# spthm/grace-devel

Hardware: AMD Instinct MI355X
Metric: Mrays/s SPH column-density trace, 10^7 particles (higher is better)
Workload: dtype f32

## Files before the change

### grace-devel_amd/csrc/trace.hip

```cpp
#include "kernel_tables.hpp"
#include "trace_kernel.hpp"
#include "trace_plan.hpp"

#include <cmath>

using namespace grace_hip;

namespace grace_hip {

static_assert(GRACE_SPH_KERNEL_TABLE_ROWS == GRACE_SPH_KERNEL_WENDLAND_C6 + 1, "one table per built-in kernel");
__device__ double g_sph_kernel_tables[GRACE_SPH_KERNEL_TABLE_ROWS][N_TABLE] = GRACE_SPH_KERNEL_TABLES_INIT;
static const double k_sph_kernel_tables[GRACE_SPH_KERNEL_TABLE_ROWS][N_TABLE] = GRACE_SPH_KERNEL_TABLES_INIT;

static grace_status trace_state_destroy(Context& c)
{
    if (!c.trace) return GRACE_OK;
    TraceState& ts = *c.trace;
    GRACE_TRY(plan_release(ts));
    GRACE_TRY(scene_release(ts));
    GRACE_TRY(rays_release(ts));
    if (ts.hits.chunk_counts) GRACE_TRY_HIP(hipFree(ts.hits.chunk_counts));
    if (ts.custom_table) GRACE_TRY_HIP(hipFree(ts.custom_table));
    if (ts.status) GRACE_TRY_HIP(hipFree(ts.status));
    if (ts.ev0) GRACE_TRY_HIP(hipEventDestroy(ts.ev0));
    if (ts.ev1) GRACE_TRY_HIP(hipEventDestroy(ts.ev1));
    delete c.trace;
    c.trace = nullptr;
    return GRACE_OK;
}

grace_status trace_state(TraceState** out)
{
    Context* c = nullptr;
    GRACE_TRY(current_context(&c));
    if (!c->trace) {
        void* tables = nullptr;
        GRACE_TRY_HIP(hipGetSymbolAddress(&tables, HIP_SYMBOL(g_sph_kernel_tables)));
        c->trace = new TraceState();
        c->trace->builtin_tables = static_cast<const double*>(tables);
        c->trace->kernel_table = c->trace->builtin_tables + GRACE_SPH_KERNEL_CUBIC * N_TABLE;
        g_trace_state_destroy = trace_state_destroy;
    }
    *out = c->trace;
    return GRACE_OK;
}

}

namespace {

struct LaunchPlan {
    int width = 64, n_packets = 0;
    int split = 1;
    bool dev_split = false;
    int hit_chunk_shift = GRANULE_SHIFT, hit_chunks = 0, hit_split = 1;
    size_t hit_packets = 0;
    bool hits_split = false;
    bool keep_chunks = false;
    bool reorder = false;
    bool lattice = false;
    int lat_split = 0;
    bool fast_b = false;
    int treelet = 0, treelet_axis = 0;
};

template <int MODE>
LaunchPlan plan_launch(const TraceState& ts, const bool keep_requested, const size_t n_rays, const size_t n_prims)
{
    LaunchPlan p;
    while ((((n_prims - 1) >> p.hit_chunk_shift) + 1) > size_t(MAX_HIT_CHUNKS)) ++p.hit_chunk_shift;
    p.hit_chunks = int(((n_prims - 1) >> p.hit_chunk_shift) + 1);
    p.hit_packets = ceil_div(n_rays, size_t(64));
    const bool split_hits = ts.width <= 0 && p.hit_packets < 4096 && p.hit_chunks >= 8 && ts.split != 1;
    p.hits_split = MODE == MODE_HITS && split_hits;
    p.keep_chunks = MODE == MODE_COUNT && keep_requested && split_hits;
    if (p.hits_split) {
        if (ts.split > 0) p.hit_split = ts.split;
        else while (p.hit_split < 8 && p.hit_packets * p.hit_split < 16384) p.hit_split *= 2;
    }
    if (ts.width > 0) p.width = ts.width;
    else if (ordered(MODE) && !p.hits_split)
        while (p.width > 16 && ceil_div(n_rays, size_t(p.width)) < 4096) p.width /= 2;
    else if (class_split(MODE) && ts.split <= 0)
        while (p.width > 16 && ceil_div(n_rays, size_t(p.width)) * SUM_CLASSES < 4096) p.width /= 2;
    p.n_packets = ceil_div(n_rays, size_t(p.width));
    p.reorder = ts.ray_reorder && n_rays > 64;
    if (class_split(MODE)) {
        const size_t wave_budget = f4_sums(MODE) ? 16385 : 16384;
        if (ts.split > 0) p.split = ts.split;
        else {
            while (p.split < SUM_CLASSES && size_t(p.n_packets) * p.split < wave_budget) p.split *= 2;
            if (f4_sums(MODE) && p.split > 1 && p.split < ts.lat_split && p.reorder && p.width == 64)
                p.split = ts.lat_split;
        }
    }
    if (p.hits_split) p.split = p.hit_split;
    p.dev_split = f4_class_split(MODE) && p.split > 1 && ts.split <= 0;
    p.lattice = has_lattice(MODE) && p.reorder;
    if (f4_class_split(MODE) && p.split == 1 && p.lattice && p.width == 64
        && ts.lat_split > 0 && ts.split <= 0)
        p.lat_split = ts.lat_split;
    p.fast_b = f4_sums(MODE) && !ts.exact_integrals;
    const int auto_treelet = (MODE == MODE_TRI) ? 512 : 8192, auto_treelet_axis = 32768;
#ifdef GRACE_PACKET_STATS
    p.treelet = ts.treelet < 0 ? auto_treelet : ts.treelet;
    p.treelet_axis = ts.treelet < 0 ? auto_treelet_axis : ts.treelet;
#else
    p.treelet = (MODE == MODE_STATS) ? 0 : (ts.treelet < 0 ? auto_treelet : ts.treelet);
    p.treelet_axis = (MODE == MODE_STATS) ? 0 : (ts.treelet < 0 ? auto_treelet_axis : ts.treelet);
#endif
    return p;
}

struct Nested { bool on = false; size_t* measure = nullptr; };

struct TraceBuffers {
    unsigned long long* sig = nullptr;
    float4* A = nullptr; float2* B = nullptr; double* T64 = nullptr; int2* node_prims = nullptr; float4* C = nullptr;
    float* partial = nullptr; double* partial_d = nullptr;
    int *chunk_counts = nullptr, *chunk_off = nullptr, *scratch_counts = nullptr;
    int4* wave_map = nullptr; int *n_wave_map = nullptr, *pk_first = nullptr, *pk_parts = nullptr;
    uint32_t *pk_prefix = nullptr, *pk_total = nullptr;
    uint32_t* ext = nullptr; uint32_t* keys = nullptr; uint32_t* perm = nullptr;
    bool plan_eligible = false;
    PlanKey plan_key;
};

template <int MODE>
grace_status use_records(TraceState& ts, TraceArgs& a, TraceBuffers& b, FrameGuard& frame, const LaunchPlan& p,
                         const size_t n_rays, const size_t n_prims, const size_t n_nodes, hipStream_t stream,
                         const Nested nested = Nested())
{
    enum CacheUse { USE_NONE, USE_FILL, USE_CHECK, USE_TRUST };
    auto decide = [&](const bool have, const bool pinned, const bool repeat) {
        if (have) return ts.cache_validation ? USE_CHECK : USE_TRUST;
        return (ts.cache_auto && repeat && !pinned) ? USE_FILL : USE_NONE;
    };
    CacheUse scene_use = USE_NONE, rays_use = USE_NONE;
    const SceneKey skey{primitive(MODE), a.spheres, a.nodes, a.leaves, n_prims, n_nodes};
    if (!fp64(MODE) && MODE != MODE_STATS && !nested.measure) {
        scene_use = decide(ts.scene.valid && ts.scene.key == skey, ts.scene.valid && ts.scene.pinned,
                           ts.scene.seen == skey);
        ts.scene.seen = skey;
        if (scene_use == USE_FILL && scene_cache_alloc(ts, skey) != GRACE_OK) scene_use = USE_NONE;
    }
    const RayKey rkey{a.rays, n_rays};
    if (p.reorder && !nested.on) {
        rays_use = decide(ts.rays.valid && ts.rays.key == rkey, ts.rays.valid && ts.rays.pinned,
                          ts.rays.seen == rkey);
        ts.rays.seen = rkey;
        if (rays_use == USE_FILL && rays_cache_alloc(ts, rkey) != GRACE_OK) rays_use = USE_NONE;
    }
    const bool scene_cached = scene_use != USE_NONE, rays_cached = rays_use != USE_NONE;
    auto held = [](const CacheUse u) { return u == USE_CHECK || u == USE_TRUST; };
    b.plan_eligible = ts.plan_on && f4_sums(MODE) && held(scene_use) && held(rays_use) && p.lat_split == 0;
    if (b.plan_eligible)
        b.plan_key = PlanKey{ PLAN_FORMAT, p.fast_b, group_shift(n_prims), p.width, p.reorder, n_rays, n_prims, ts.scene.gen, ts.rays.gen };
    PlanGate gate;
    const bool plan_steady = b.plan_eligible && ts.plan.valid && ts.plan.key == b.plan_key;
    if (plan_steady) {
        gate.ctl = ts.plan.ctl; gate.scene = ts.scene.ctl; gate.rays = ts.rays.ctl;
    }
    const bool scene_sig = scene_use == USE_FILL || scene_use == USE_CHECK;
    const bool rays_sig = rays_use == USE_FILL || rays_use == USE_CHECK, sig = scene_sig || rays_sig;
    auto carve = [&](char* const base) {
        size_t used = 0;
        auto take = [&](auto*& ptr, const size_t count) {
            using T = std::remove_reference_t<decltype(*ptr)>;
            ptr = base ? reinterpret_cast<T*>(base + used) : nullptr;
            used += Workspace::aligned(count * sizeof(T));
        };
        if (sig) take(b.sig, sig_partial_words());
        if (!scene_cached) {
            take(b.A, n_prims + 4);
            if (f4_integrals(MODE)) take(b.B, n_prims + 4);
            if (MODE == MODE_TRI) take(b.T64, 9 * (n_prims + 4));
            take(b.node_prims, n_nodes); take(b.C, cluster_record_count(n_prims));
        }
        if (f4_sums(MODE)) take(b.partial, n_rays * SUM_CLASSES * channels(MODE));
        if (double_sums(MODE)) take(b.partial_d, n_rays * SUM_CLASSES);
        if (p.hits_split) {
            take(b.chunk_counts, n_rays * size_t(p.hit_chunks)); take(b.chunk_off, n_rays * size_t(p.hit_chunks));
            take(b.scratch_counts, n_rays); take(b.wave_map, p.hit_packets * p.hit_split); take(b.n_wave_map, 16);
            take(b.pk_prefix, p.hit_packets * size_t(p.hit_chunks));
            take(b.pk_total, p.hit_packets + 16); take(b.pk_first, p.hit_packets + 16); take(b.pk_parts, p.hit_packets + 16);
        }
        if (p.reorder) { take(b.ext, 20); take(b.keys, n_rays); take(b.perm, n_rays); }
        return used;
    };
    const size_t own = carve(nullptr);
    const size_t need = own + (p.reorder ? sort_ws_bytes(n_rays, 4, 0) : 0);
    if (nested.measure) {
        *nested.measure = need + Workspace::aligned(sig_partial_words() * sizeof(*b.sig));
        return GRACE_OK;
    }
    if (nested.on) GRACE_REQUIRE(Workspace::room() >= need, "trace: the caller's frame is too small for a nested trace");
    else GRACE_TRY(frame.begin(need, stream));
    carve(Workspace::take<char>(own));
    if (sig) {
        SigRequest rq;
        if (scene_sig) {
            rq.prims = a.spheres; rq.prims_bytes = n_prims * (MODE == MODE_TRI ? 36 : 16);
            rq.nodes = a.nodes; rq.nodes_bytes = n_nodes * 64;
            rq.leaves = a.leaves; rq.leaves_bytes = (n_nodes + 1) * 16;
            rq.scene_ctl = ts.scene.ctl; rq.scene_force = scene_use == USE_FILL;
        }
        if (rays_sig) {
            rq.rays = a.rays; rq.rays_bytes = n_rays * 28;
            rq.rays_ctl = ts.rays.ctl; rq.rays_force = rays_use == USE_FILL; rq.rays_ext = ts.rays.ext;
        }
        GRACE_TRY(launch_signatures(rq, b.sig, stream));
    }
    if (scene_cached) {
        Scene& sc = ts.scene;
        if (scene_use != USE_TRUST) {
            GRACE_TRY(scene_fill(skey.kind, a.spheres, n_prims, a.nodes, n_nodes, a.leaves, sc.A, sc.B1, sc.B50,
                                 sc.T64, sc.node_prims, sc.C, stream, &sc.ctl->stale));
            sc.valid = true;
        }
        a.A = sc.A; a.T64 = sc.T64; a.node_prims = sc.node_prims; a.C = sc.C;
        a.B = f4_integrals(MODE) ? (p.fast_b ? sc.B50 : sc.B1) : nullptr;
    } else {
        GRACE_TRY(scene_fill(skey.kind, primitive(MODE) == PRIM_D4 ? static_cast<const void*>(a.spheres_d) : a.spheres,
                             n_prims, a.nodes, n_nodes, a.leaves, b.A, p.fast_b ? nullptr : b.B, p.fast_b ? b.B : nullptr,
                             b.T64, b.node_prims, b.C, stream));
        a.A = b.A; a.B = b.B; a.T64 = b.T64; a.node_prims = b.node_prims; a.C = b.C;
    }
    if (p.reorder) {
        const float4* scene_min = a.C + 2 * ((n_prims + 63) / 64);
        uint32_t* lat_flag = p.lattice ? b.ext + 13 : nullptr;
        int* split_dev = p.dev_split ? reinterpret_cast<int*>(b.ext + 12) : nullptr;
        const int split_flags = f4_sums(MODE) ? SPLIT_WIDE_BUDGET : 0;
        if (rays_cached) {
            RayOrder& ro = ts.rays;
            if (rays_use != USE_TRUST) {
                GRACE_TRY(ray_order(a.rays, n_rays, ro.ext, b.keys, ro.perm, nullptr, nullptr, 0, 0, nullptr,
                                    stream, &ro.ctl->stale));
                ro.valid = true;
            }
            int* plan_split_dev = b.plan_eligible && split_dev && !weighted(MODE)
                ? reinterpret_cast<int*>(b.ext + 16) : nullptr;
            if (lat_flag || split_dev || plan_steady)
                GRACE_TRY(launch_choose_variants(ro.ext, int(n_rays), scene_min, lat_flag, p.n_packets,
                                                 p.split | split_flags, split_dev, stream, plan_steady ? &gate : nullptr,
                                                 plan_split_dev));
            a.perm = ro.perm; a.plan_split_dev = plan_split_dev;
        } else {
            GRACE_TRY(ray_order(a.rays, n_rays, b.ext, b.keys, b.perm, scene_min, lat_flag, p.n_packets,
                                p.split | split_flags, split_dev, stream));
            a.perm = b.perm;
        }
        a.lat_dev = reinterpret_cast<const int*>(lat_flag); a.split_dev = split_dev;
    }
    return GRACE_OK;
}

template <int MODE, bool SPLIT, bool ALT = false>
void launch_walk(const int grid, const TraceArgs& args, hipStream_t stream)
{
    trace_kernel<MODE, SPLIT, ALT, false><<<grid, TRACE_BLOCK, 0, stream>>>(args);
    if constexpr (has_lattice(MODE))
        if (args.lat_dev) trace_kernel<MODE, SPLIT, ALT, true><<<grid, TRACE_BLOCK, 0, stream>>>(args);
}

template <int MODE>
grace_status dispatch(const TraceState& ts, const TraceArgs& a, const TraceBuffers& b, const LaunchPlan& p,
                      const int* kept, const size_t n_rays, hipStream_t stream)
{
    const int grid = ceil_div(size_t(p.n_packets) * p.split, TRACE_BLOCK / 64);
    const int* const plan_k_dev = a.plan_usable ? a.plan_split_dev : nullptr;
    auto combine = [&](const int k, const int* k_dev, const int* run_if) -> grace_status {
        const int g = ceil_div(n_rays * channels(MODE), 256);
        if constexpr (double_sums(MODE))
            combine_classes_kernel<double><<<g, 256, 0, stream>>>(a.partial_d, int(n_rays), k, k_dev, a.out_sums_d, run_if);
        else if constexpr (weighted(MODE))
            combine_channel_classes_kernel<<<g, 256, 0, stream>>>(a.partial, int(n_rays), channels(MODE), k, k_dev,
                                                                  a.out_sums, a.out_stride, run_if,
                                                                  a.plan_usable, plan_k_dev);
        else if constexpr (f4_sums(MODE))
            combine_classes_kernel<float><<<g, 256, 0, stream>>>(a.partial, int(n_rays), k, k_dev, a.out_sums, run_if,
                                                                 a.plan_usable, plan_k_dev);
        else return GRACE_OK;
        GRACE_CHECK_LAUNCH();
        return GRACE_OK;
    };
    if constexpr (class_split(MODE)) {
        auto walk = [&](auto alt_tag) -> grace_status {
            constexpr bool ALT = decltype(alt_tag)::value;
            if constexpr (has_lattice(MODE)) if (p.lat_split) {
                if (output(MODE) == OUT_COUNTS)
                    GRACE_TRY_HIP(hipMemsetAsync(a.out_counts, 0, n_rays * sizeof(int), stream));
                trace_kernel<MODE, false, ALT, false><<<grid, TRACE_BLOCK, 0, stream>>>(a);
                GRACE_CHECK_LAUNCH();
                TraceArgs a_lat = a;
                a_lat.split = p.lat_split; a_lat.split_dev = nullptr;
                trace_kernel<MODE, true, ALT, true><<<ceil_div(size_t(p.n_packets) * p.lat_split, TRACE_BLOCK / 64),
                                                      TRACE_BLOCK, 0, stream>>>(a_lat);
                GRACE_CHECK_LAUNCH();
                return combine(p.lat_split, nullptr, a.lat_dev);
            }
            if constexpr (f4_sums(MODE)) if (a.plan_usable) {
                GRACE_TRY(plan_record(ts, a, stream));
                const int grid_planned = a.plan_split_dev
                    ? ceil_div(size_t(p.n_packets) * planned_split(p.n_packets), TRACE_BLOCK / 64) : grid;
                GRACE_TRY(launch_planned(MODE, ALT, grid_planned, a, stream));
                if (p.split == 1) GRACE_TRY(combine(1, nullptr, reinterpret_cast<const int*>(a.plan_usable)));
            }
            if (p.split > 1) launch_walk<MODE, true, ALT>(grid, a, stream);
            else launch_walk<MODE, false, ALT>(grid, a, stream);
            return GRACE_OK;
        };
        if constexpr (f4_sums(MODE)) GRACE_TRY(p.fast_b ? walk(std::true_type()) : walk(std::false_type()));
        else GRACE_TRY(walk(std::false_type()));
    } else if constexpr (MODE == MODE_HITS) {
        if (p.hits_split) {
            const int* counts = kept;
            if (!kept) {
                TraceArgs c = a;
                c.chunk_counts = b.chunk_counts; c.out_counts = b.scratch_counts;
                GRACE_TRY_HIP(hipMemsetAsync(b.chunk_counts, 0, n_rays * size_t(p.hit_chunks) * 4, stream));
                GRACE_TRY_HIP(hipMemsetAsync(b.scratch_counts, 0, n_rays * 4, stream));
                launch_walk<MODE_COUNT, true>(grid, c, stream);
                GRACE_CHECK_LAUNCH();
                counts = b.chunk_counts;
            }
            hits_offsets_kernel<<<ceil_div(n_rays, 4), 256, 0, stream>>>(counts, a.offsets, int(n_rays),
                                                                         p.hit_chunks, b.chunk_off);
            GRACE_CHECK_LAUNCH();
            hits_plan_kernel<<<p.n_packets, MAX_HIT_CHUNKS, 0, stream>>>(counts, a.perm, int(n_rays),
                                                                         p.hit_chunks, b.pk_prefix, b.pk_total);
            GRACE_CHECK_LAUNCH();
            hits_assign_kernel<<<1, 1024, 0, stream>>>(b.pk_total, p.n_packets, p.n_packets * p.split, p.hit_chunks,
                                                       b.pk_first, b.pk_parts, b.n_wave_map,
                                                       ts.hits_stage_split ? 200000ull : 0ull);
            GRACE_CHECK_LAUNCH();
            hits_bounds_kernel<<<p.n_packets, 64, 0, stream>>>(b.pk_prefix, b.pk_total, b.pk_first, b.pk_parts,
                                                               p.hit_chunks, b.wave_map);
            GRACE_CHECK_LAUNCH();
            TraceArgs staged = a, direct = a;
            staged.stage_dev = direct.stage_dev = b.n_wave_map + 4;
            staged.stage_want = 1; direct.stage_want = 0;
            launch_walk<MODE, true, true>(grid, staged, stream);
            GRACE_CHECK_LAUNCH();
            launch_walk<MODE, true, false>(grid, direct, stream);
        } else if (p.n_packets >= 4096) {
            launch_walk<MODE, false, true>(grid, a, stream);
        } else {
            launch_walk<MODE, false, false>(grid, a, stream);
        }
    } else {
        launch_walk<MODE, false>(grid, a, stream);
    }
    GRACE_CHECK_LAUNCH();
    GRACE_TRY(stamps_report(MODE));
    if (p.split > 1) GRACE_TRY(combine(p.split, a.split_dev, nullptr));
    return GRACE_OK;
}

template <int MODE>
grace_status launch_trace(TraceArgs a, size_t n_rays, size_t n_spheres, size_t n_nodes,
                          hipStream_t stream, const Nested nested = Nested())
{
    GRACE_REQUIRE(a.rays && a.spheres && a.nodes && a.leaves && a.root, "trace: null pointer");
    GRACE_REQUIRE(n_rays < (size_t(1) << 31), "trace: bad ray count");
    GRACE_REQUIRE(n_nodes >= 1 && n_nodes < (size_t(1) << 30), "trace: bad node count");
    GRACE_REQUIRE(n_spheres > 0 && n_spheres < (size_t(1) << 31), "trace: bad primitive count");
    TraceState* ts_ptr = nullptr;
    GRACE_TRY(trace_state(&ts_ptr));
    TraceState& ts = *ts_ptr;
    GRACE_TRY(ensure_status(ts, stream));
    a.kernel_table = ts.kernel_table;
    const LaunchPlan p = plan_launch<MODE>(ts, a.keep_chunks, n_rays, n_spheres);
    const bool reuse_chunks = p.hits_split && ts.hits.valid && ts.hits.rays == a.rays
        && ts.hits.n_rays == n_rays && ts.hits.prims == static_cast<const void*>(a.spheres)
        && ts.hits.n_prims == n_spheres && ts.hits.n_chunks == p.hit_chunks;
    if (chunked(MODE)) ts.hits.valid = false;
    const size_t need = n_rays * size_t(p.hit_chunks);
    if (p.keep_chunks && ts.hits.capacity < need) {
        if (ts.hits.chunk_counts) { GRACE_TRY_HIP(hipDeviceSynchronize()); GRACE_TRY_HIP(hipFree(ts.hits.chunk_counts)); }
        ts.hits.chunk_counts = nullptr; ts.hits.capacity = 0;
        hipError_t e = hipMalloc(reinterpret_cast<void**>(&ts.hits.chunk_counts), need * sizeof(int));
        if (e != hipSuccess) return set_error(GRACE_OUT_OF_MEMORY, __FILE__, __LINE__, hipGetErrorString(e));
        ts.hits.capacity = need;
    }
    FrameGuard frame;
    TraceBuffers b;
    GRACE_TRY(use_records<MODE>(ts, a, b, frame, p, n_rays, n_spheres, n_nodes, stream, nested));
    if (nested.measure) return GRACE_OK;
    a.width = p.width; a.split = p.split; a.treelet = p.treelet; a.treelet_axis = p.treelet_axis;
    a.n_rays = int(n_rays); a.n_nodes = int(n_nodes); a.n_prims = int(n_spheres); a.status = ts.status;
    a.group_shift = group_shift(n_spheres); a.chunk_shift = p.hit_chunk_shift; a.n_chunks = p.hit_chunks;
    a.partial = b.partial; a.partial_d = b.partial_d;
    a.chunk_off = b.chunk_off; a.wave_map = b.wave_map; a.n_wave_map = b.n_wave_map;
    if (p.split > 1 && output(MODE) == OUT_COUNTS)
        GRACE_TRY_HIP(hipMemsetAsync(a.out_counts, 0, n_rays * sizeof(int), stream));
    if (p.keep_chunks && p.split > 1) {
        a.chunk_counts = ts.hits.chunk_counts;
        GRACE_TRY_HIP(hipMemsetAsync(ts.hits.chunk_counts, 0, n_rays * size_t(p.hit_chunks) * 4, stream));
        ts.hits.valid = true; ts.hits.rays = a.rays; ts.hits.n_rays = n_rays;
        ts.hits.prims = a.spheres; ts.hits.n_prims = n_spheres; ts.hits.n_chunks = p.hit_chunks;
    }
    ts.last_lat_dev = a.lat_dev; ts.last_lat_stream = stream;
    if constexpr (f4_sums(MODE)) {
        PacketPlan& pp = ts.plan;
        if (b.plan_eligible && !(pp.key == b.plan_key && (pp.valid || pp.dead)))
            GRACE_TRY(plan_fill(ts, b.plan_key, a, stream));
        ts.last_plan_ctl = nullptr;
        if (b.plan_eligible && pp.valid && pp.key == b.plan_key) {
            a.plan_entries = pp.entries; a.plan_spans = pp.spans; a.plan_counts = pp.counts;
            a.plan_usable = &pp.ctl->usable;
            ts.last_plan_ctl = pp.ctl; ts.last_plan_stream = stream;
        }
    }
    return timed(ts, stream, [&] {
        return dispatch<MODE>(ts, a, b, p, reuse_chunks ? ts.hits.chunk_counts : nullptr, n_rays, stream);
    });
}

TraceArgs trace_args(const void* d_rays, const void* d_prims, const int* d_nodes, const int* d_leaves,
                     const int* d_root)
{
    TraceArgs a = {};
    a.rays = static_cast<const float*>(d_rays);
    a.spheres = static_cast<const float4*>(d_prims);
    a.nodes = reinterpret_cast<const float4*>(d_nodes);
    a.leaves = reinterpret_cast<const int4*>(d_leaves);
    a.root = d_root;
    return a;
}

}

namespace grace_hip {
grace_status rays_invalidate_if_written(const void* d_written)
{
    Context* c = nullptr;
    GRACE_TRY(current_context(&c));
    if (!c->trace) return GRACE_OK;
    TraceState& ts = *c->trace;
    if (ts.cache_validation) return GRACE_OK;
    if (ts.rays.valid && d_written && d_written == static_cast<const void*>(ts.rays.key.rays)) return rays_release(ts);
    return GRACE_OK;
}

grace_status scene_invalidate_if_written(const void* d_written)
{
    Context* c = nullptr;
    GRACE_TRY(current_context(&c));
    if (!c->trace) return GRACE_OK;
    TraceState& ts = *c->trace;
    if (ts.cache_validation) return GRACE_OK;
    if (ts.scene.valid && d_written
        && (d_written == ts.scene.key.prims || d_written == ts.scene.key.nodes || d_written == ts.scene.key.leaves))
        return scene_release(ts);
    return GRACE_OK;
}

grace_status trace_nested_bytes(size_t n_rays, size_t n_spheres, size_t n_nodes, size_t* bytes)
{
    TraceArgs a = trace_args(bytes, bytes, reinterpret_cast<const int*>(bytes), reinterpret_cast<const int*>(bytes),
                             reinterpret_cast<const int*>(bytes));
    size_t counts = 0, hits = 0;
    GRACE_TRY(launch_trace<MODE_COUNT>(a, n_rays, n_spheres, n_nodes, nullptr, Nested{true, &counts}));
    GRACE_TRY(launch_trace<MODE_HITS>(a, n_rays, n_spheres, n_nodes, nullptr, Nested{true, &hits}));
    *bytes = counts > hits ? counts : hits;
    return GRACE_OK;
}

grace_status trace_hitcounts_nested(const void* d_rays, size_t n_rays, const float* d_spheres, size_t n_spheres,
                                    const int* d_nodes, size_t n_nodes, const int* d_leaves, const int* d_root,
                                    int* d_hit_counts, hipStream_t stream)
{
    TraceArgs a = trace_args(d_rays, d_spheres, d_nodes, d_leaves, d_root);
    a.out_counts = d_hit_counts;
    return launch_trace<MODE_COUNT>(a, n_rays, n_spheres, n_nodes, stream, Nested{true, nullptr});
}

grace_status trace_hits_nested(const void* d_rays, size_t n_rays, const float* d_spheres, size_t n_spheres,
                               const int* d_nodes, size_t n_nodes, const int* d_leaves, const int* d_root,
                               const int* d_ray_offsets, int* d_hit_indices, float* d_hit_integrals,
                               float* d_hit_distances, hipStream_t stream)
{
    TraceArgs a = trace_args(d_rays, d_spheres, d_nodes, d_leaves, d_root);
    a.offsets = d_ray_offsets;
    a.hit_idx = d_hit_indices;
    a.hit_integral = d_hit_integrals;
    a.hit_dist = d_hit_distances;
    return launch_trace<MODE_HITS>(a, n_rays, n_spheres, n_nodes, stream, Nested{true, nullptr});
}
}

extern "C" {

grace_status grace_trace_hitcounts_f4(const void* d_rays, size_t n_rays, const float* d_spheres,
                                      size_t n_spheres, const int* d_nodes, size_t n_nodes,
                                      const int* d_leaves, const int* d_root,
                                      int* d_hit_counts, grace_stream stream)
{
    if (n_rays == 0) return GRACE_OK;
    GRACE_REQUIRE(d_hit_counts, "trace_hitcounts: null output");
    TraceArgs a = trace_args(d_rays, d_spheres, d_nodes, d_leaves, d_root);
    a.out_counts = d_hit_counts;
    return launch_trace<MODE_COUNT>(a, n_rays, n_spheres, n_nodes, as_stream(stream));
}

grace_status grace_trace_hitcounts_keep_f4(const void* d_rays, size_t n_rays, const float* d_spheres,
                                           size_t n_spheres, const int* d_nodes, size_t n_nodes,
                                           const int* d_leaves, const int* d_root,
                                           int* d_hit_counts, grace_stream stream)
{
    if (n_rays == 0) return GRACE_OK;
    GRACE_REQUIRE(d_hit_counts, "trace_hitcounts: null output");
    TraceArgs a = trace_args(d_rays, d_spheres, d_nodes, d_leaves, d_root);
    a.out_counts = d_hit_counts;
    a.keep_chunks = true;
    return launch_trace<MODE_COUNT>(a, n_rays, n_spheres, n_nodes, as_stream(stream));
}

grace_status grace_trace_cumulative_f4(const void* d_rays, size_t n_rays, const float* d_spheres,
                                       size_t n_spheres, const int* d_nodes, size_t n_nodes,
                                       const int* d_leaves, const int* d_root,
                                       float* d_cumulated, grace_stream stream)
{
    if (n_rays == 0) return GRACE_OK;
    GRACE_REQUIRE(d_cumulated, "trace_cumulative: null output");
    TraceArgs a = trace_args(d_rays, d_spheres, d_nodes, d_leaves, d_root);
    a.out_sums = d_cumulated;
    return launch_trace<MODE_CUMULATIVE>(a, n_rays, n_spheres, n_nodes, as_stream(stream));
}

grace_status grace_trace_cumulative_weighted_f4(const void* d_rays, size_t n_rays, const float* d_spheres,
                                                size_t n_spheres, const int* d_nodes, size_t n_nodes,
                                                const int* d_leaves, const int* d_root,
                                                const float* d_weights, int n_channels, float* d_out,
                                                grace_stream stream)
{
    GRACE_REQUIRE(n_channels >= 1 && n_channels <= 64, "trace_cumulative_weighted: channels must be 1..64");
    if (n_rays == 0) return GRACE_OK;
    GRACE_REQUIRE(d_weights || n_spheres == 0, "trace_cumulative_weighted: null weights");
    GRACE_REQUIRE(d_out, "trace_cumulative_weighted: null output");
    GRACE_REQUIRE(n_rays * size_t(n_channels) < (size_t(1) << 31), "trace_cumulative_weighted: too many outputs");
    for (int g = 0; g < n_channels; g += MAX_LAUNCH_CHANNELS) {
        TraceArgs a = trace_args(d_rays, d_spheres, d_nodes, d_leaves, d_root);
        a.weights = d_weights + g;
        a.w_stride = n_channels;
        a.out_sums = d_out + g;
        a.out_stride = n_channels;
        const hipStream_t s = as_stream(stream);
        switch (n_channels - g < MAX_LAUNCH_CHANNELS ? n_channels - g : MAX_LAUNCH_CHANNELS) {
        case 1: GRACE_TRY(launch_trace<MODE_WCUM1>(a, n_rays, n_spheres, n_nodes, s)); break;
        case 2: GRACE_TRY(launch_trace<MODE_WCUM2>(a, n_rays, n_spheres, n_nodes, s)); break;
        case 3: GRACE_TRY(launch_trace<MODE_WCUM3>(a, n_rays, n_spheres, n_nodes, s)); break;
        default: GRACE_TRY(launch_trace<MODE_WCUM4>(a, n_rays, n_spheres, n_nodes, s)); break;
        }
    }
    return GRACE_OK;
}

grace_status grace_trace_hits_f4(const void* d_rays, size_t n_rays, const float* d_spheres,
                                 size_t n_spheres, const int* d_nodes, size_t n_nodes,
                                 const int* d_leaves, const int* d_root,
                                 const int* d_ray_offsets, int* d_hit_indices,
                                 float* d_hit_integrals, float* d_hit_distances,
                                 grace_stream stream)
{
    if (n_rays == 0) return GRACE_OK;
    GRACE_REQUIRE(d_ray_offsets && d_hit_indices && d_hit_integrals && d_hit_distances,
                  "trace_hits: null output");
    TraceArgs a = trace_args(d_rays, d_spheres, d_nodes, d_leaves, d_root);
// ... 71 lines not shown
    GRACE_REQUIRE(d_hit_counts, "trace_hitcounts (float4, double): null output");
    TraceArgs a = trace_args(d_rays, d_spheres, d_nodes, d_leaves, d_root);
    a.out_counts = d_hit_counts;
    return launch_trace<MODE_COUNT_F4D>(a, n_rays, n_spheres, n_nodes, as_stream(stream));
}

grace_status grace_trace_cumulative_f4_f64(const void* d_rays, size_t n_rays, const float* d_spheres,
                                           size_t n_spheres, const int* d_nodes, size_t n_nodes,
                                           const int* d_leaves, const int* d_root, double* d_sums,
                                           grace_stream stream)
{
    if (n_rays == 0) return GRACE_OK;
    GRACE_REQUIRE(d_sums, "trace_cumulative (float4, double): null output");
    TraceArgs a = trace_args(d_rays, d_spheres, d_nodes, d_leaves, d_root);
    a.out_sums_d = d_sums;
    return launch_trace<MODE_CUM_F4D>(a, n_rays, n_spheres, n_nodes, as_stream(stream));
}

grace_status grace_trace_hits_f4_f64(const void* d_rays, size_t n_rays, const float* d_spheres,
                                     size_t n_spheres, const int* d_nodes, size_t n_nodes,
                                     const int* d_leaves, const int* d_root, const int* d_ray_offsets,
                                     int* d_hit_indices, double* d_hit_integrals,
                                     double* d_hit_distances, grace_stream stream)
{
    if (n_rays == 0) return GRACE_OK;
    GRACE_REQUIRE(d_ray_offsets && d_hit_indices && d_hit_integrals && d_hit_distances,
                  "trace_hits (float4, double): null output");
    TraceArgs a = trace_args(d_rays, d_spheres, d_nodes, d_leaves, d_root);
    a.offsets = d_ray_offsets;
    a.hit_idx = d_hit_indices;
    a.hit_integral_d = d_hit_integrals;
    a.hit_dist_d = d_hit_distances;
    return launch_trace<MODE_HITS_F4D>(a, n_rays, n_spheres, n_nodes, as_stream(stream));
}

grace_status grace_trace_stats_f4(const void* d_rays, size_t n_rays, const float* d_spheres,
                                  size_t n_spheres, const int* d_nodes, size_t n_nodes,
                                  const int* d_leaves, const int* d_root,
                                  uint32_t* d_stats4, grace_stream stream)
{
    if (n_rays == 0) return GRACE_OK;
    GRACE_REQUIRE(d_stats4, "trace_stats: null output");
    TraceArgs a = trace_args(d_rays, d_spheres, d_nodes, d_leaves, d_root);
    a.stats = d_stats4;
    return launch_trace<MODE_STATS>(a, n_rays, n_spheres, n_nodes, as_stream(stream));
}

grace_status grace_hit_integrals_f32(const float* d_b2, const float* d_h, size_t n, float* d_out,
                                     grace_stream stream)
{
    GRACE_REQUIRE(n == 0 || (d_b2 && d_h && d_out), "hit_integrals: null pointer");
    if (n == 0) return GRACE_OK;
    TraceState* ts = nullptr;
    GRACE_TRY(trace_state(&ts));
    hit_integrals_kernel<<<stream_grid(n, 256), 256, 0, as_stream(stream)>>>(d_b2, d_h, n, d_out,
                                                                             ts->kernel_table);
    GRACE_CHECK_LAUNCH();
    return GRACE_OK;
}

grace_status grace_sph_kernel_table(int kind, double* h_out51)
{
    GRACE_REQUIRE(kind >= GRACE_SPH_KERNEL_CUBIC && kind <= GRACE_SPH_KERNEL_WENDLAND_C6,
                  "sph_kernel_table: kind must be a built-in GRACE_SPH_KERNEL_* (0..5)");
    GRACE_REQUIRE(h_out51, "sph_kernel_table: null output");
    for (int i = 0; i < N_TABLE; ++i) h_out51[i] = k_sph_kernel_tables[kind][i];
    return GRACE_OK;
}

#define GRACE_TRACE_STATE()                                                                      \
    TraceState* ts_ptr_ = nullptr;                                                               \
    GRACE_TRY(trace_state(&ts_ptr_));                                                            \
    TraceState& ts = *ts_ptr_

grace_status grace_trace_prepare_f4(const float* d_spheres, size_t n_spheres, const int* d_nodes,
                                    size_t n_nodes, const int* d_leaves, grace_stream stream)
{
    GRACE_TRACE_STATE();
    return scene_prepare(ts, PRIM_F4, d_spheres, n_spheres, d_nodes, n_nodes, d_leaves, as_stream(stream));
}

grace_status grace_trace_prepare_tri(const float* d_tris, size_t n_tris, const int* d_nodes,
                                     size_t n_nodes, const int* d_leaves, grace_stream stream)
{
    GRACE_TRACE_STATE();
    return scene_prepare(ts, PRIM_TRI, d_tris, n_tris, d_nodes, n_nodes, d_leaves, as_stream(stream));
}

grace_status grace_trace_prepare_rays(const void* d_rays, size_t n_rays, grace_stream stream)
{
    GRACE_TRACE_STATE();
    return rays_prepare(ts, static_cast<const float*>(d_rays), n_rays, as_stream(stream));
}

grace_status grace_trace_release_rays(void)
{
    GRACE_TRACE_STATE();
    GRACE_TRY(plan_release(ts));
    return rays_release(ts);
}

grace_status grace_trace_release(void)
{
    GRACE_TRACE_STATE();
    if (ts.hits.chunk_counts) {
        GRACE_TRY_HIP(hipDeviceSynchronize());
        GRACE_TRY_HIP(hipFree(ts.hits.chunk_counts));
    }
    ts.hits = HitsCache();
    GRACE_TRY(plan_release(ts));
    return scene_release(ts);
}

grace_status grace_trace_enable_timing(int enabled)
{
    GRACE_TRACE_STATE();
    ts.timing = enabled != 0;
    ts.ev_valid = false;
    return GRACE_OK;
}

grace_status grace_trace_last_kernel_ms(float* h_ms)
{
    GRACE_REQUIRE(h_ms, "null output");
    GRACE_TRACE_STATE();
    GRACE_REQUIRE(ts.timing && ts.ev_valid, "no timed traversal launch recorded");
    GRACE_TRY_HIP(hipEventSynchronize(ts.ev1));
    GRACE_TRY_HIP(hipEventElapsedTime(h_ms, ts.ev0, ts.ev1));
    return GRACE_OK;
}

grace_status grace_trace_last_lattice(int* h_lattice)
{
    GRACE_REQUIRE(h_lattice, "null output");
    *h_lattice = 0;
    GRACE_TRACE_STATE();
    if (ts.last_lat_dev) {
        GRACE_TRY_HIP(hipStreamSynchronize(ts.last_lat_stream));
        GRACE_TRY_HIP(hipMemcpy(h_lattice, ts.last_lat_dev, sizeof(int), hipMemcpyDeviceToHost));
    }
    return GRACE_OK;
}

grace_status grace_trace_last_plan_used(int* h_used)
{
    GRACE_REQUIRE(h_used, "null output");
    *h_used = 0;
    GRACE_TRACE_STATE();
    if (ts.last_plan_ctl) {
        PlanCtl h = {};
        GRACE_TRY_HIP(hipStreamSynchronize(ts.last_plan_stream));
        GRACE_TRY_HIP(hipMemcpy(&h, ts.last_plan_ctl, sizeof(h), hipMemcpyDeviceToHost));
        *h_used = h.usable != 0u ? 1 : 0;
    }
    return GRACE_OK;
}

grace_status grace_trace_plan_stats(unsigned long long* h_stats)
{
    GRACE_REQUIRE(h_stats, "null output");
    for (int k = 0; k < 7; ++k) h_stats[k] = 0;
    GRACE_TRACE_STATE();
    if (ts.last_plan_ctl) {
        PlanCtl h = {};
        GRACE_TRY_HIP(hipStreamSynchronize(ts.last_plan_stream));
        GRACE_TRY_HIP(hipMemcpy(&h, ts.last_plan_ctl, sizeof(h), hipMemcpyDeviceToHost));
        if (h.usable != 0u) {
            for (int k = 0; k < 6; ++k) h_stats[k] = h.stats[k];
            h_stats[6] = h.largest_round;
        }
    }
    return GRACE_OK;
}

grace_status grace_trace_set_plan(int on)
{
    GRACE_TRACE_STATE();
    ts.plan_on = on != 0;
    if (!ts.plan_on) GRACE_TRY(plan_release(ts));
    return GRACE_OK;
}

grace_status grace_trace_set_plan_budget(size_t bytes)
{
    GRACE_TRACE_STATE();
    ts.plan_budget = bytes;
    GRACE_TRY(plan_release(ts));
    return GRACE_OK;
}

grace_status grace_trace_plan_bytes(size_t* h_bytes)
{
    GRACE_REQUIRE(h_bytes, "null output");
    GRACE_TRACE_STATE();
    const PacketPlan& pp = ts.plan;
    *h_bytes = pp.valid ? (pp.n_entries + 4) * sizeof(uint4) + pp.n_lists * (sizeof(int) + sizeof(int2)) + sizeof(PlanCtl) : 0;
    return GRACE_OK;
}

grace_status grace_trace_set_packet_split(int waves_per_packet)
{
    GRACE_REQUIRE(waves_per_packet == -1 || waves_per_packet == 1 || waves_per_packet == 2
                      || waves_per_packet == 4 || waves_per_packet == 8,
                  "packet split must be 1, 2, 4, 8 or -1 (automatic)");
    GRACE_TRACE_STATE();
    ts.split = waves_per_packet;
    return GRACE_OK;
}

grace_status grace_trace_set_packet_width(int rays_per_packet)
{
    GRACE_REQUIRE(rays_per_packet == -1 || rays_per_packet == 16 || rays_per_packet == 32
                      || rays_per_packet == 64,
                  "packet width must be 16, 32, 64 or -1 (automatic)");
    GRACE_TRACE_STATE();
    ts.width = rays_per_packet;
    return GRACE_OK;
}

grace_status grace_trace_set_exact_integrals(int enabled)
{
    GRACE_TRACE_STATE();
    ts.exact_integrals = enabled != 0;
    return GRACE_OK;
}

grace_status grace_trace_set_sph_kernel(int kind)
{
    GRACE_REQUIRE(kind >= GRACE_SPH_KERNEL_CUBIC && kind <= GRACE_SPH_KERNEL_WENDLAND_C6,
                  "set_sph_kernel: kind must be a built-in GRACE_SPH_KERNEL_* (0..5); a custom table is "
                  "set with grace_trace_set_sph_kernel_table");
    GRACE_TRACE_STATE();
    ts.sph_kernel = kind;
    ts.kernel_table = ts.builtin_tables + kind * N_TABLE;
    return GRACE_OK;
}

grace_status grace_trace_set_sph_kernel_table(const double* h_table, int n)
{
    GRACE_REQUIRE(h_table && n == N_TABLE, "set_sph_kernel_table: the table must hold 51 values");
    for (int i = 0; i < N_TABLE; ++i)
        GRACE_REQUIRE(std::isfinite(h_table[i]) && h_table[i] >= 0.0,
                      "set_sph_kernel_table: every value must be finite and >= 0");
    GRACE_REQUIRE(h_table[N_TABLE - 1] == 0.0, "set_sph_kernel_table: the last value (b = H) must be 0");
    GRACE_TRACE_STATE();
    GRACE_TRY_HIP(hipDeviceSynchronize());
    if (!ts.custom_table)
        GRACE_TRY_HIP(hipMalloc(reinterpret_cast<void**>(&ts.custom_table), N_TABLE * sizeof(double)));
    GRACE_TRY_HIP(hipMemcpy(ts.custom_table, h_table, N_TABLE * sizeof(double), hipMemcpyHostToDevice));
    for (int i = 0; i < N_TABLE; ++i) ts.custom_host[i] = h_table[i];
    ts.sph_kernel = GRACE_SPH_KERNEL_CUSTOM;
    ts.kernel_table = ts.custom_table;
    return GRACE_OK;
}

grace_status grace_trace_get_sph_kernel(int* h_kind, double* h_table51)
{
    GRACE_TRACE_STATE();
    if (h_kind) *h_kind = ts.sph_kernel;
    if (h_table51) {
        const double* t = ts.sph_kernel == GRACE_SPH_KERNEL_CUSTOM ? ts.custom_host
                                                                   : k_sph_kernel_tables[ts.sph_kernel];
        for (int i = 0; i < N_TABLE; ++i) h_table51[i] = t[i];
    }
    return GRACE_OK;
}

grace_status grace_trace_set_treelet_size(int max_primitives)
{
    GRACE_REQUIRE(max_primitives >= -1, "treelet size must be >= 0 (or -1 for automatic)");
    GRACE_TRACE_STATE();
    ts.treelet = max_primitives;
    return GRACE_OK;
}

grace_status grace_trace_set_ray_reorder(int enabled)
{
    GRACE_TRACE_STATE();
    ts.ray_reorder = enabled != 0;
    return GRACE_OK;
}

grace_status grace_trace_set_cache_validation(int enabled)
{
    GRACE_TRACE_STATE();
    ts.cache_validation = enabled != 0;
    return GRACE_OK;
}

grace_status grace_trace_set_cache_auto(int enabled)
{
    GRACE_TRACE_STATE();
    ts.cache_auto = enabled != 0;
    if (!ts.cache_auto) {
        if ((ts.scene.valid && !ts.scene.pinned) || (ts.rays.valid && !ts.rays.pinned)) GRACE_TRY(plan_release(ts));
        if (ts.scene.valid && !ts.scene.pinned) GRACE_TRY(scene_release(ts));
        if (ts.rays.valid && !ts.rays.pinned) GRACE_TRY(rays_release(ts));
        ts.scene.seen = SceneKey();
        ts.rays.seen = RayKey();
    }
    return GRACE_OK;
}

grace_status grace_trace_set_lattice_split(int waves_per_packet)
{
    GRACE_REQUIRE(waves_per_packet == 0 || waves_per_packet == 2 || waves_per_packet == 4
                      || waves_per_packet == 8,
                  "lattice split must be 0 (one wave per packet), 2, 4 or 8");
    GRACE_TRACE_STATE();
    ts.lat_split = waves_per_packet;
    return GRACE_OK;
}

grace_status grace_trace_set_hits_staging(int enabled)
{
    GRACE_TRACE_STATE();
    ts.hits_stage_split = enabled != 0;
    return GRACE_OK;
}

grace_status grace_trace_status(grace_stream stream)
{
    GRACE_TRACE_STATE();
    if (!ts.status) return GRACE_OK;
// ... 17 lines not shown
```

### grace-devel_amd/csrc/trace_cache.hip

```cpp
#include "trace_state.hpp"

#include <cstdint>

using namespace grace_hip;

namespace {

constexpr int SIG_BLOCK = 256;
constexpr int SIG_GRID = 1024;
constexpr int SIG_GROUPS = 2;

struct SigArgs {
    const uint32_t* base[4];
    size_t words[4];
    size_t chunk0[4];
    int group[4];
    int aligned[4];
    int n_arrays;
};

__device__ __forceinline__ unsigned long long mix64(unsigned long long v)
{
    v ^= v >> 32;
    v *= 0xD6E8FEB86659FD93ull;
    v ^= v >> 29;
    return v;
}

__global__ __launch_bounds__(SIG_BLOCK) void signature_kernel(const SigArgs a,
                                                              unsigned long long* __restrict__ partial)
{
    unsigned long long sx[SIG_GROUPS] = { 0ull, 0ull }, sy[SIG_GROUPS] = { 0ull, 0ull };
    const size_t t0 = blockIdx.x * size_t(blockDim.x) + threadIdx.x, stride = size_t(gridDim.x) * blockDim.x;
    for (int k = 0; k < a.n_arrays; ++k) {
        const size_t n_chunks = (a.words[k] + 3) / 4;
        const uint32_t* w = a.base[k];
        unsigned long long ax = 0ull, ay = 0ull;
        for (size_t c = t0; c < n_chunks; c += stride) {
            uint4 q;
            if (a.aligned[k] && 4 * c + 4 <= a.words[k]) {
                q = reinterpret_cast<const uint4*>(w)[c];
            } else {
                q.x = 4 * c + 0 < a.words[k] ? w[4 * c + 0] : 0u;
                q.y = 4 * c + 1 < a.words[k] ? w[4 * c + 1] : 0u;
                q.z = 4 * c + 2 < a.words[k] ? w[4 * c + 2] : 0u;
                q.w = 4 * c + 3 < a.words[k] ? w[4 * c + 3] : 0u;
            }
            const unsigned long long i = a.chunk0[k] + c;
            const unsigned long long lo = (unsigned long long)q.x | ((unsigned long long)q.y << 32);
            const unsigned long long hi = (unsigned long long)q.z | ((unsigned long long)q.w << 32);
            const unsigned long long x = mix64(lo ^ (i * 0x9E3779B97F4A7C15ull));
            const unsigned long long y = mix64((hi + ((x << 31) | (x >> 33))) ^ (i * 0xC2B2AE3D27D4EB4Full));
            ax += x;
            ay += y;
        }
        sx[a.group[k]] += ax;
        sy[a.group[k]] += ay;
    }
    __shared__ unsigned long long s_red[SIG_BLOCK / 64][2 * SIG_GROUPS];
    const int lane = threadIdx.x & 63, wave = threadIdx.x >> 6;
#pragma unroll
    for (int g = 0; g < SIG_GROUPS; ++g) {
#pragma unroll
        for (int off = 32; off > 0; off >>= 1) {
            sx[g] += __shfl_xor(sx[g], off);
            sy[g] += __shfl_xor(sy[g], off);
        }
        if (lane == 0) { s_red[wave][2 * g] = sx[g]; s_red[wave][2 * g + 1] = sy[g]; }
    }
    __syncthreads();
    if (threadIdx.x < 2 * SIG_GROUPS) {
        unsigned long long v = 0ull;
        for (int w = 0; w < SIG_BLOCK / 64; ++w) v += s_red[w][threadIdx.x];
        partial[size_t(blockIdx.x) * 2 * SIG_GROUPS + threadIdx.x] = v;
    }
}

struct CheckArgs {
    CacheCtl* ctl[SIG_GROUPS];
    int force[SIG_GROUPS];
    unsigned long long salt[SIG_GROUPS];
    uint32_t* rays_ext;
};

__global__ __launch_bounds__(SIG_BLOCK) void signature_check_kernel(const unsigned long long* __restrict__ partial,
                                                                    const CheckArgs a)
{
    __shared__ unsigned long long s_red[SIG_BLOCK / 64][2 * SIG_GROUPS];
    unsigned long long v[2 * SIG_GROUPS] = { 0ull, 0ull, 0ull, 0ull };
    for (int b = threadIdx.x; b < SIG_GRID; b += blockDim.x)
#pragma unroll
        for (int k = 0; k < 2 * SIG_GROUPS; ++k) v[k] += partial[size_t(b) * 2 * SIG_GROUPS + k];
    const int lane = threadIdx.x & 63, wave = threadIdx.x >> 6;
#pragma unroll
    for (int k = 0; k < 2 * SIG_GROUPS; ++k) {
#pragma unroll
        for (int off = 32; off > 0; off >>= 1) v[k] += __shfl_xor(v[k], off);
        if (lane == 0) s_red[wave][k] = v[k];
    }
    __syncthreads();
    if (threadIdx.x < SIG_GROUPS) {
        const int g = threadIdx.x;
        CacheCtl* ctl = a.ctl[g];
        if (ctl) {
            unsigned long long x = a.salt[g], y = ~a.salt[g];
            for (int w = 0; w < SIG_BLOCK / 64; ++w) { x += s_red[w][2 * g]; y += s_red[w][2 * g + 1]; }
            const bool stale = a.force[g] || ctl->sig[0] != x || ctl->sig[1] != y;
            ctl->sig[0] = x;
            ctl->sig[1] = y;
            ctl->stale = stale ? 1u : 0u;
            if (g == 1 && stale && a.rays_ext) {
                for (int k = 0; k < 16; ++k) a.rays_ext[k] = k < 6 ? 0xFFFFFFFFu : 0u;
            }
        }
    }
}

}

namespace grace_hip {

size_t sig_partial_words() { return size_t(SIG_GRID) * 2 * SIG_GROUPS; }

grace_status launch_signatures(const SigRequest& rq, unsigned long long* partial, hipStream_t stream)
{
    SigArgs a = {};
    CheckArgs c = {};
    size_t next_chunk[SIG_GROUPS] = { 0, 0 };
    auto add = [&](const void* p, size_t bytes, int group) {
        if (!p || bytes == 0) return;
        const int k = a.n_arrays++;
        a.base[k] = static_cast<const uint32_t*>(p);
        a.words[k] = bytes / 4;
        a.group[k] = group;
        a.aligned[k] = (reinterpret_cast<uintptr_t>(p) & 15u) == 0 ? 1 : 0;
        a.chunk0[k] = next_chunk[group];
        next_chunk[group] += (a.words[k] + 3) / 4;
        c.salt[group] = c.salt[group] * 0x100000001B3ull + bytes;
    };
    if (rq.scene_ctl) {
        add(rq.prims, rq.prims_bytes, 0);
        add(rq.nodes, rq.nodes_bytes, 0);
        add(rq.leaves, rq.leaves_bytes, 0);
        c.ctl[0] = rq.scene_ctl;
        c.force[0] = rq.scene_force ? 1 : 0;
    }
    if (rq.rays_ctl) {
        add(rq.rays, rq.rays_bytes, 1);
        c.ctl[1] = rq.rays_ctl;
        c.force[1] = rq.rays_force ? 1 : 0;
        c.rays_ext = rq.rays_ext;
    }
    if (!c.ctl[0] && !c.ctl[1]) return GRACE_OK;
    signature_kernel<<<SIG_GRID, SIG_BLOCK, 0, stream>>>(a, partial);
    GRACE_CHECK_LAUNCH();
    signature_check_kernel<<<1, SIG_BLOCK, 0, stream>>>(partial, c);
    GRACE_CHECK_LAUNCH();
    return GRACE_OK;
}

}
```

### grace-devel_amd/csrc/trace_coherence.hip

```cpp
#include "trace_state.hpp"

using namespace grace_hip;

namespace {

__device__ __forceinline__ uint32_t f2ord_u(float f)
{
    const uint32_t u = __float_as_uint(f);
    return (u & 0x80000000u) ? ~u : (u | 0x80000000u);
}

__device__ __forceinline__ float ord2f_u(uint32_t u)
{
    return __uint_as_float((u & 0x80000000u) ? (u & 0x7fffffffu) : ~u);
}

__global__ void ray_ext_init_kernel(uint32_t* __restrict__ ext16)
{
    if (threadIdx.x < 16) ext16[threadIdx.x] = threadIdx.x < 6 ? 0xFFFFFFFFu : 0u;
}

__global__ __launch_bounds__(1024) void ray_extents_kernel(const float* __restrict__ rays, int n,
                                                          uint32_t* __restrict__ ext12,
                                                          const uint32_t* __restrict__ run_if)
// ... 3 lines not shown
    float len_hi = -INFINITY;
#pragma unroll
    for (int k = 0; k < 6; ++k) { lo[k] = INFINITY; hi[k] = -INFINITY; }
    for (int i = blockIdx.x * blockDim.x + threadIdx.x; i < n; i += gridDim.x * blockDim.x) {
        const float* r = rays + 7 * size_t(i);
#pragma unroll
        for (int k = 0; k < 6; ++k) {
            const float v = r[k];
            lo[k] = fminf(lo[k], v);
            hi[k] = fmaxf(hi[k], v);
        }
        len_hi = fmaxf(len_hi, r[6]);
    }
#pragma unroll
    for (int off = 32; off > 0; off >>= 1) len_hi = fmaxf(len_hi, __shfl_xor(len_hi, off));
#pragma unroll
    for (int k = 0; k < 6; ++k) {
#pragma unroll
        for (int off = 32; off > 0; off >>= 1) {
            lo[k] = fminf(lo[k], __shfl_xor(lo[k], off));
            hi[k] = fmaxf(hi[k], __shfl_xor(hi[k], off));
        }
    }
    __shared__ float s_lo[16][6], s_hi[16][6], s_len[16];
    const int wave = threadIdx.x >> 6;
    if ((threadIdx.x & 63) == 0) {
#pragma unroll
        for (int k = 0; k < 6; ++k) { s_lo[wave][k] = lo[k]; s_hi[wave][k] = hi[k]; }
        s_len[wave] = len_hi;
    }
    __syncthreads();
    const int n_waves = int(blockDim.x >> 6);
    if (threadIdx.x < 6) {
        const int k = threadIdx.x;
        float l = s_lo[0][k], h = s_hi[0][k];
        for (int w = 1; w < n_waves; ++w) { l = fminf(l, s_lo[w][k]); h = fmaxf(h, s_hi[w][k]); }
        atomicMin(&ext12[k], f2ord_u(l));
        atomicMax(&ext12[6 + k], f2ord_u(h));
    } else if (threadIdx.x == 6) {
        float l = s_len[0];
        for (int w = 1; w < n_waves; ++w) l = fmaxf(l, s_len[w]);
        if (l > -INFINITY) atomicMax(&ext12[15], f2ord_u(l));
    }
}

__device__ int choose_split(const uint32_t* __restrict__ ext12, int n_packets, int launched_arg, bool lattice)
{
    const bool one_direction = ext12[0] == ext12[6] && ext12[1] == ext12[7] && ext12[2] == ext12[8];
    const int launched = launched_arg & 0xFF;
    const int budget = (launched_arg & SPLIT_WIDE_BUDGET) ? 32768 : 16384;
    int k = launched;
    if (one_direction && !lattice) {
        k = 1;
        while (k < launched && n_packets * k < 8192) k *= 2;
        if (k < launched && n_packets >= 6144 && n_packets * k * 2 <= budget) k *= 2;
    } else if (!lattice) {
        k = 1;
        while (k < launched && n_packets * k < 16384) k *= 2;
    }
    return k;
}

__device__ __forceinline__ uint32_t hilbert2d_15(uint32_t x, uint32_t y)
{
    uint32_t d = 0;
    for (uint32_t s = 1u << 14; s > 0; s >>= 1) {
        const uint32_t rx = (x & s) ? 1u : 0u, ry = (y & s) ? 1u : 0u;
        d = (d << 2) | ((3u * rx) ^ ry);
        if (ry == 0) {
            if (rx) { x = 32767u - x; y = 32767u - y; }
            const uint32_t t = x; x = y; y = t;
        }
    }
    return d;
}

__global__ __launch_bounds__(256) void ray_lattice_kernel(const float* __restrict__ rays, int n,
                                                          const uint32_t* __restrict__ ext12,
                                                          uint32_t* __restrict__ flag,
                                                          const uint32_t* __restrict__ run_if)
{
    if (run_if && *run_if == 0u) return;
    int dims[2] = { 0, 0 }, nvar = 0;
    float lo[2] = { 0.f, 0.f }, span[2] = { 0.f, 0.f };
    for (int k = 5; k >= 0; --k) {
        const float l = ord2f_u(ext12[k]), sp = ord2f_u(ext12[6 + k]) - l;
        if (sp > 0.f && sp < INFINITY) {
            if (nvar < 2) { dims[nvar] = k; lo[nvar] = l; span[nvar] = sp; }
            ++nvar;
        }
    }
    bool fit = nvar == 2 && n >= 64 && (n & (n - 1)) == 0;
    float m1 = 0.f, m2 = 0.f;
    if (fit) {
        int log_n = 0;
        while ((1 << log_n) < n) ++log_n;
        fit = false;
        const float ratio = span[0] / span[1];
        for (int a = 3; a <= log_n - 3; ++a) {
            const float c1 = float((1 << a) - 1), c2 = float((1 << (log_n - a)) - 1);
            if (fabsf(c1 / c2 - ratio) <= 1e-3f * ratio) { fit = true; m1 = c1; m2 = c2; break; }
        }
    }
    if (!fit) {
        if (blockIdx.x == 0 && threadIdx.x == 0) atomicOr(flag, 1u);
        return;
    }
    const float s1 = m1 / span[0], s2 = m2 / span[1];
    bool off = false;
    for (int i = blockIdx.x * blockDim.x + threadIdx.x; i < n; i += gridDim.x * blockDim.x) {
        const float* r = rays + 7 * size_t(i);
        const float u1 = (r[dims[0]] - lo[0]) * s1, u2 = (r[dims[1]] - lo[1]) * s2;
        off = off || !(fabsf(u1 - rintf(u1)) <= 0.01f) || !(fabsf(u2 - rintf(u2)) <= 0.01f);
    }
    if (__builtin_amdgcn_ballot_w64(off) != 0ull && (threadIdx.x & 63) == 0) atomicOr(flag, 1u);
}

__device__ void choose_variants(const uint32_t* __restrict__ ext12, int n, const float4* __restrict__ scene_min,
                                uint32_t* __restrict__ lat_flag, int split_packets, int split_launched,
                                int* __restrict__ split_dev)
{
    if (lat_flag) {
        int n_dir = 0;
        bool one_dir = true;
        float e1 = 0.f, e2 = 0.f;
        for (int k = 0; k < 3; ++k) {
            const float dl = ord2f_u(ext12[k]), dh = ord2f_u(ext12[6 + k]);
            one_dir = one_dir && dl == dh;
            n_dir += dl != 0.f ? 1 : 0;
            const float e = ord2f_u(ext12[9 + k]) - ord2f_u(ext12[3 + k]);
            if (e > e1) { e2 = e1; e1 = e; } else if (e > e2) e2 = e;
        }
        const float spacing2 = e1 * e2 / float(n);
        const float r2_min = scene_min->x;
        bool lat = one_dir && n_dir == 1 && spacing2 > 0.f && r2_min < 2.0f * spacing2;
        if (!lat && e1 == 0.f && ext12[15] != 0u) {
            const float len = ord2f_u(ext12[15]);
            if (len > 0.f && len < INFINITY) lat = r2_min < 2.0f * (12.566371f * len * len / float(n));
        }
        *lat_flag = lat ? 1u : 0u;
    }
    if (split_dev)
        *split_dev = choose_split(ext12, split_packets, split_launched, lat_flag ? *lat_flag != 0u : false);
}

__global__ void choose_variants_kernel(const uint32_t* __restrict__ ext12, int n, const float4* __restrict__ scene_min,
                                       uint32_t* __restrict__ lat_flag, int split_packets, int split_launched,
                                       int* __restrict__ split_dev, const PlanGate gate,
                                       int* __restrict__ plan_split_dev)
{
    if (lat_flag || split_dev)
        choose_variants(ext12, n, scene_min, lat_flag, split_packets, split_launched, split_dev);
    if (plan_split_dev) *plan_split_dev = planned_split(split_packets);
    if (gate.ctl) {
        PlanCtl& pc = *gate.ctl;
        const bool stale = pc.sig[0] != gate.scene->sig[0] || pc.sig[1] != gate.scene->sig[1]
            || pc.sig[2] != gate.rays->sig[0] || pc.sig[3] != gate.rays->sig[1];
        pc.record = stale ? 1u : 0u;
        if (stale) {
            pc.unusable = 0u; pc.usable = 1u;
            pc.sig[0] = gate.scene->sig[0]; pc.sig[1] = gate.scene->sig[1];
            pc.sig[2] = gate.rays->sig[0]; pc.sig[3] = gate.rays->sig[1];
            for (int k = 0; k < 6; ++k) pc.stats[k] = 0ull;
            pc.largest_round = 0u;
        }
    }
}

__global__ __launch_bounds__(256) void ray_keys_kernel(const float* __restrict__ rays, int n,
                                                       const uint32_t* __restrict__ ext12,
                                                       uint32_t* __restrict__ keys,
                                                       const float4* __restrict__ scene_min,
                                                       uint32_t* __restrict__ lat_flag,
                                                       int split_packets, int split_launched,
                                                       int* __restrict__ split_dev,
                                                       const uint32_t* __restrict__ not_grid,
                                                       const uint32_t* __restrict__ run_if)
{
    if (run_if && *run_if == 0u) return;
    const bool z_order_2d = not_grid && *not_grid == 0u;
    if (blockIdx.x == 0 && threadIdx.x == 0)
        choose_variants(ext12, n, scene_min, lat_flag, split_packets, split_launched, split_dev);
    float lo[6], scale[6], span[6];
    int nvar = 0;
    float span_d = 0.f, span_o = 0.f;
#pragma unroll
    for (int k = 0; k < 6; ++k) {
        lo[k] = ord2f_u(ext12[k]);
        span[k] = ord2f_u(ext12[6 + k]) - lo[k];
        const bool varies = span[k] > 0.f && span[k] < INFINITY;
        if (varies) { if (k < 3) span_d = fmaxf(span_d, span[k]); else span_o = fmaxf(span_o, span[k]); }
    }
#pragma unroll
    for (int k = 0; k < 6; ++k) {
        const bool varies = span[k] > 0.f && span[k] < INFINITY;
        scale[k] = varies ? 1.0f / (k < 3 ? span_d : span_o) : 0.f;
        nvar += varies ? 1 : 0;
    }
    const int bits = nvar ? min(15, 30 / nvar) : 0;
    const float qmax = float((1 << bits) - 1);
    const bool pencil = scale[3] == 0.f && scale[4] == 0.f && scale[5] == 0.f && nvar > 0;
    for (int i = blockIdx.x * blockDim.x + threadIdx.x; i < n; i += gridDim.x * blockDim.x) {
        const float* r = rays + 7 * size_t(i);
        if (pencil) {
            const float l1 = fabsf(r[0]) + fabsf(r[1]) + fabsf(r[2]);
            float u = r[0] / l1, v = r[1] / l1;
            if (r[2] < 0.f) {
                const float fu = (1.f - fabsf(v)) * (u >= 0.f ? 1.f : -1.f);
                const float fv = (1.f - fabsf(u)) * (v >= 0.f ? 1.f : -1.f);
                u = fu; v = fv;
            }
            const uint32_t qu = uint32_t(fminf(32767.f, fmaxf(0.f, (u * 0.5f + 0.5f) * 32767.f + 0.5f)));
            const uint32_t qv = uint32_t(fminf(32767.f, fmaxf(0.f, (v * 0.5f + 0.5f) * 32767.f + 0.5f)));
            keys[i] = hilbert2d_15(qu, qv);
            continue;
        }
        uint32_t q[6];
#pragma unroll
        for (int k = 0; k < 6; ++k) q[k] = uint32_t(fminf(qmax, (r[k] - lo[k]) * scale[k] * qmax + 0.5f));
#ifndef GRACE_MORTON2D
        if (nvar == 2 && !z_order_2d) {
            uint32_t xy[2] = {0, 0};
            int m = 0;
#pragma unroll
            for (int k = 5; k >= 0; --k)
                if (scale[k] > 0.f) { if (m < 2) xy[m] = q[k]; ++m; }
            keys[i] = hilbert2d_15(xy[1], xy[0]);
            continue;
        }
#endif
        uint32_t key = 0;
        for (int b = bits - 1; b >= 0; --b) {
#pragma unroll
            for (int k = 5; k >= 0; --k)
                if (scale[k] > 0.f) key = (key << 1) | ((q[k] >> b) & 1u);
        }
        keys[i] = key << (30 - bits * nvar);
    }
}

}

namespace grace_hip {

grace_status launch_choose_variants(const uint32_t* ext12, int n, const float4* scene_min, uint32_t* lat_flag,
                                    int split_packets, int split_launched, int* split_dev, hipStream_t stream,
                                    const PlanGate* gate, int* plan_split_dev)
{
    choose_variants_kernel<<<1, 1, 0, stream>>>(ext12, n, scene_min, lat_flag, split_packets, split_launched,
                                                split_dev, gate ? *gate : PlanGate(), plan_split_dev);
    GRACE_CHECK_LAUNCH();
    return GRACE_OK;
}

static grace_status rays_free_buffers(RayOrder& ro)
{
    if (ro.perm || ro.ext || ro.ctl) GRACE_TRY_HIP(hipDeviceSynchronize());
    if (ro.perm) GRACE_TRY_HIP(hipFree(ro.perm));
    if (ro.ext) GRACE_TRY_HIP(hipFree(ro.ext));
    if (ro.ctl) GRACE_TRY_HIP(hipFree(ro.ctl));
    ro.perm = nullptr; ro.ext = nullptr; ro.ctl = nullptr;
    ro.valid = false;
    ro.pinned = false;
    return GRACE_OK;
}

grace_status rays_release(TraceState& ts)
{
    GRACE_TRY(rays_free_buffers(ts.rays));
    ts.rays = RayOrder();
    return GRACE_OK;
}

grace_status rays_cache_alloc(TraceState& ts, const RayKey& key)
{
    RayOrder& ro = ts.rays;
    GRACE_TRY(rays_free_buffers(ro));
    if (hipMalloc(reinterpret_cast<void**>(&ro.perm), key.n * 4) != hipSuccess
        || hipMalloc(reinterpret_cast<void**>(&ro.ext), 64) != hipSuccess
        || hipMalloc(reinterpret_cast<void**>(&ro.ctl), sizeof(CacheCtl)) != hipSuccess) {
        (void)hipGetLastError();
        (void)rays_free_buffers(ro);
        return set_error(GRACE_OUT_OF_MEMORY, __FILE__, __LINE__, "ray order cache: out of device memory");
    }
    ro.key = key;
    ro.gen = ++ts.cache_gen;
    return GRACE_OK;
}

grace_status ray_order(const float* d_rays, size_t n_rays, uint32_t* ext, uint32_t* keys, uint32_t* perm,
                       const float4* scene_min, uint32_t* lat_flag, int n_packets, int split, int* split_dev,
                       hipStream_t stream, const uint32_t* run_if)
{
    if (!run_if) {
        ray_ext_init_kernel<<<1, 64, 0, stream>>>(ext);
        GRACE_CHECK_LAUNCH();
    }
    const int grid_small = stream_grid(n_rays, 256, 4) < 1024 ? stream_grid(n_rays, 256, 4) : 1024;
    const int grid_ext = stream_grid(n_rays, 1024, 4) < 128 ? stream_grid(n_rays, 1024, 4) : 128;
    ray_extents_kernel<<<grid_ext, 1024, 0, stream>>>(d_rays, int(n_rays), ext, run_if);
    GRACE_CHECK_LAUNCH();
    ray_lattice_kernel<<<grid_small, 256, 0, stream>>>(d_rays, int(n_rays), ext, ext + 14, run_if);
    GRACE_CHECK_LAUNCH();
    ray_keys_kernel<<<stream_grid(n_rays, 256), 256, 0, stream>>>(d_rays, int(n_rays), ext, keys, scene_min,
                                                                 lat_flag, n_packets, split, split_dev, ext + 14,
                                                                 run_if);
    GRACE_CHECK_LAUNCH();
// ... 41 lines not shown
```

### grace-devel_amd/csrc/trace_kernel.hpp

```cpp
#pragma once

#include "trace_diag.hpp"
#include "trace_packet.hpp"
#include "trace_state.hpp"

#include <type_traits>

namespace {

using namespace grace_hip;

__device__ __forceinline__ bool any_lane(bool p) { return __builtin_amdgcn_ballot_w64(p) != 0ull; }

__device__ __forceinline__ int imin(int a, int b) { return a < b ? a : b; }
__device__ __forceinline__ int imax(int a, int b) { return a > b ? a : b; }

__device__ __forceinline__ void aabbs_hit(const float ix, const float iy, const float iz,
                                          const float ox, const float oy, const float oz,
                                          const float len, const float4 L, const float4 R,
                                          const float4 Z, bool& hit_l, bool& hit_r)
{
    const float bx_L = (L.x - ox) * ix, tx_L = (L.y - ox) * ix;
    const float by_L = (L.z - oy) * iy, ty_L = (L.w - oy) * iy;
    const float bz_L = (Z.x - oz) * iz, tz_L = (Z.y - oz) * iz;
    const float bx_R = (R.x - ox) * ix, tx_R = (R.y - ox) * ix;
    const float by_R = (R.z - oy) * iy, ty_R = (R.w - oy) * iy;
    const float bz_R = (Z.z - oz) * iz, tz_R = (Z.w - oz) * iz;

    auto entry = [](const float t) { return t != t ? -INFINITY : t; };
    auto exit_ = [](const float t) { return t != t ? INFINITY : t; };
    const int zero = __float_as_int(0.0f), ilen = __float_as_int(len);
    const int tmin_L = imax(imax(__float_as_int(fminf(entry(bx_L), entry(tx_L))), __float_as_int(fminf(entry(by_L), entry(ty_L)))),
                            imax(imin(__float_as_int(entry(bz_L)), __float_as_int(entry(tz_L))), zero));
    const int tmax_L = imin(imin(__float_as_int(fmaxf(exit_(bx_L), exit_(tx_L))), __float_as_int(fmaxf(exit_(by_L), exit_(ty_L)))),
                            imin(imax(__float_as_int(exit_(bz_L)), __float_as_int(exit_(tz_L))), ilen));
    const int tmin_R = imax(imax(__float_as_int(fminf(entry(bx_R), entry(tx_R))), __float_as_int(fminf(entry(by_R), entry(ty_R)))),
                            imax(imin(__float_as_int(entry(bz_R)), __float_as_int(entry(tz_R))), zero));
    const int tmax_R = imin(imin(__float_as_int(fmaxf(exit_(bx_R), exit_(tx_R))), __float_as_int(fmaxf(exit_(by_R), exit_(ty_R)))),
                            imin(imax(__float_as_int(exit_(bz_R)), __float_as_int(exit_(tz_R))), ilen));
    hit_r = __int_as_float(tmax_R) >= __int_as_float(tmin_R);
    hit_l = __int_as_float(tmax_L) >= __int_as_float(tmin_L);
}

__device__ __forceinline__ float sqrt_rn_normal(const float x)
{
    const float y = __builtin_amdgcn_sqrtf(x);
    const float ym = __int_as_float(__float_as_int(y) - 1);
    const float yp = __int_as_float(__float_as_int(y) + 1);
    const float rm = __builtin_fmaf(-ym, y, x);
    const float rp = __builtin_fmaf(-yp, y, x);
    float r = (0.0f >= rm) ? ym : y;
    r = (0.0f < rp) ? yp : r;
    return r;
}

__device__ __forceinline__ float hit_integral(const float b2, const float ir, const float ir2,
                                              const double2* lut)
{
    const bool tiny = b2 < 1.2621774e-29f && b2 > 0.0f;
    const float root = __builtin_amdgcn_ballot_w64(tiny) ? __builtin_sqrtf(b2) : sqrt_rn_normal(b2);
    const float b = (N_TABLE - 1) * (root * ir);
    int x_idx = static_cast<int>(b);
    float t32 = b - static_cast<float>(x_idx);
    if (__builtin_amdgcn_ballot_w64(x_idx >= N_TABLE - 1)) {
        t32 = x_idx >= N_TABLE - 1 ? 1.0f : t32;
        x_idx = x_idx >= N_TABLE - 1 ? N_TABLE - 2 : x_idx;
    }
    const double2 y = lut[x_idx];
    float integral = static_cast<float>(__builtin_fma(static_cast<double>(t32), y.y, y.x));
    integral *= ir2;
    return integral;
}

__device__ __forceinline__ float hit_integral_fast(const float b2, const float ir50,
                                                   const float2* lutf)
{
    const float b = __builtin_amdgcn_sqrtf(b2) * ir50;
    const float2 y = lutf[static_cast<int>(b)];
    return __builtin_fmaf(y.y, b, y.x);
}

__device__ __forceinline__ bool tri_intersect(const double ddx, const double ddy, const double ddz,
                                              const float ox, const float oy, const float oz,
                                              const double* __restrict__ tri, float* t_out)
{
    const double vx = tri[0], vy = tri[1], vz = tri[2];
    const double e1x = tri[3], e1y = tri[4], e1z = tri[5];
    const double e2x = tri[6], e2y = tri[7], e2z = tri[8];
    const float Px = float(ddy * e2z - ddz * e2y);
    const float Py = float(ddz * e2x - ddx * e2z);
    const float Pz = float(ddx * e2y - ddy * e2x);
    const float det = float((e1x * double(Px) + e1y * double(Py)) + e1z * double(Pz));
    bool reject = det < 1E-14f;
    const float inv_det = 1.0f / det;
    const float OVx = ox - float(vx), OVy = oy - float(vy), OVz = oz - float(vz);
    const double dOVx = OVx, dOVy = OVy, dOVz = OVz;
    const float u = float(((dOVx * double(Px) + dOVy * double(Py)) + dOVz * double(Pz)) * double(inv_det));
    reject = reject || (u < 0.f || u > 1.f);
    const float Qx = float(dOVy * e1z - dOVz * e1y);
    const float Qy = float(dOVz * e1x - dOVx * e1z);
    const float Qz = float(dOVx * e1y - dOVy * e1x);
    const float v = float(((ddx * double(Qx) + ddy * double(Qy)) + ddz * double(Qz)) * double(inv_det));
    reject = reject || (v < 0.f || u + v > 1.f);
    *t_out = float(((e2x * double(Qx) + e2y * double(Qy)) + e2z * double(Qz)) * double(inv_det));
    return !reject;
}

__global__ __launch_bounds__(256) void hit_integrals_kernel(const float* __restrict__ b2,
                                                            const float* __restrict__ h, size_t n,
                                                            float* __restrict__ out,
                                                            const double* __restrict__ table)
{
    __shared__ double2 s_lut[N_TABLE];
    if (threadIdx.x < N_TABLE) {
        const double y0 = table[threadIdx.x];
        const double y1 = threadIdx.x + 1 < N_TABLE ? table[threadIdx.x + 1] : y0;
        s_lut[threadIdx.x] = make_double2(y0, y1 - y0);
    }
    __syncthreads();
    for (size_t i = blockIdx.x * size_t(blockDim.x) + threadIdx.x; i < n;
         i += size_t(gridDim.x) * blockDim.x) {
        const float ir = 1.f / h[i];
        out[i] = hit_integral(b2[i], ir, ir * ir, s_lut);
    }
}

__device__ __forceinline__ bool beam_may_hit(const float4 s, const Beam& bm,
                                             const float margin = 3.814697265625e-06f )
{
    float p2_lo = 0.f, p2_hi = 0.f, t_lo = 0.f, t_hi = 0.f;
    const float c[3] = { s.x, s.y, s.z };
#pragma unroll
    for (int k = 0; k < 3; ++k) {
        const float plo = c[k] - bm.ohi[k], phi = c[k] - bm.olo[k];
        const float a2 = plo * plo, b2 = phi * phi;
        p2_hi += fmaxf(a2, b2);
        p2_lo += (plo <= 0.f && phi >= 0.f) ? 0.f : fminf(a2, b2);
        const float q0 = plo * bm.dlo[k], q1 = plo * bm.dhi[k];
        const float q2 = phi * bm.dlo[k], q3 = phi * bm.dhi[k];
        t_lo += fminf(fminf(q0, q1), fminf(q2, q3));
        t_hi += fmaxf(fmaxf(q0, q1), fmaxf(q2, q3));
    }
    const float t2_hi = fmaxf(t_lo * t_lo, t_hi * t_hi);
    const float b2_lo = p2_lo - t2_hi - margin * p2_hi;
    return !(b2_lo >= s.w);
}

struct Pencil {
    float ox, oy, oz;
    float ax, ay, az;
    float sin_t, cos_t;
    float nx[4], ny[4], nz[4];
};

__device__ __forceinline__ bool pencil_may_hit(const float4 s, const Pencil& pc)
{
    const float vx = s.x - pc.ox, vy = s.y - pc.oy, vz = s.z - pc.oz;
    const float d2 = __builtin_fmaf(vx, vx, __builtin_fmaf(vy, vy, vz * vz));
    const float va = __builtin_fmaf(vx, pc.ax, __builtin_fmaf(vy, pc.ay, vz * pc.az));
    const float inv = __builtin_amdgcn_rsqf(d2);
    const float sin_a = fminf(1.0f, __builtin_amdgcn_sqrtf(s.w) * inv * 1.00001f);
    const float cos_a = __builtin_amdgcn_sqrtf(fmaxf(0.0f, __builtin_fmaf(-sin_a, sin_a, 1.0f)));
    const float cos_limit = __builtin_fmaf(pc.cos_t, cos_a, -pc.sin_t * sin_a) - 1e-5f;
    const float h = __builtin_amdgcn_sqrtf(s.w) * 1.00001f + 1e-6f * __builtin_amdgcn_sqrtf(d2);
    float out = -1.0f;
#pragma unroll
    for (int k = 0; k < 4; ++k)
        out = fmaxf(out, __builtin_fmaf(vx, pc.nx[k], __builtin_fmaf(vy, pc.ny[k], vz * pc.nz[k])) - h);
    return !(d2 > s.w * 1.00001f) || (!(va * inv < cos_limit) && !(out > 0.0f));
}

template <int AX, bool FUSED = false>
__device__ __forceinline__ bool axis_beam_may_hit(const float4 s, const Beam& bm)
{
    constexpr int D1 = AX == 0 ? 1 : 0, D2 = AX == 2 ? 1 : 2;
    const float s1 = AX == 0 ? s.y : s.x;
    const float s2 = AX == 2 ? s.y : s.z;
    const float q1 = s1 - __builtin_amdgcn_fmed3f(s1, bm.olo[D1], bm.ohi[D1]);
    const float q2 = s2 - __builtin_amdgcn_fmed3f(s2, bm.olo[D2], bm.ohi[D2]);
    const float b2_lo = FUSED ? __builtin_fmaf(q1, q1, q2 * q2) : q1 * q1 + q2 * q2;
    return !(b2_lo >= s.w);
}

__device__ __forceinline__ float4 cluster_sphere(const float4 blo, const float4 bhi)
{
    const float cx = 0.5f * (blo.x + bhi.x), cy = 0.5f * (blo.y + bhi.y), cz = 0.5f * (blo.z + bhi.z);
    const float ex = bhi.x - cx, ey = bhi.y - cy, ez = bhi.z - cz;
    const float fx = cx - blo.x, fy = cy - blo.y, fz = cz - blo.z;
    const float rx = fmaxf(ex, fx), ry = fmaxf(ey, fy), rz = fmaxf(ez, fz);
    return make_float4(cx, cy, cz, (rx * rx + ry * ry + rz * rz) * 1.001f);
}

template <int AX>
__device__ __forceinline__ bool cluster_may_hit(const float4 blo, const float4 bhi, const Beam& bm,
                                                const Pencil* pc)
{
    if constexpr (AX >= 0) {
        constexpr int D1 = AX == 0 ? 1 : 0, D2 = AX == 2 ? 1 : 2;
        const float lo1 = AX == 0 ? blo.y : blo.x, hi1 = AX == 0 ? bhi.y : bhi.x;
        const float lo2 = AX == 2 ? blo.y : blo.z, hi2 = AX == 2 ? bhi.y : bhi.z;
        return !(lo1 > bm.ohi[D1]) && !(hi1 < bm.olo[D1]) && !(lo2 > bm.ohi[D2]) && !(hi2 < bm.olo[D2]);
    } else if constexpr (AX == -2) {
        const float lx = blo.x - pc->ox, ly = blo.y - pc->oy, lz = blo.z - pc->oz;
        const float hx = bhi.x - pc->ox, hy = bhi.y - pc->oy, hz = bhi.z - pc->oz;
        const float scale = fmaxf(fmaxf(fmaxf(fabsf(lx), fabsf(hx)), fmaxf(fabsf(ly), fabsf(hy))),
                                  fmaxf(fabsf(lz), fabsf(hz)));
        const float slack = 1e-5f * scale;
        float worst = -1.0f;
#pragma unroll
        for (int k = 0; k < 4; ++k) {
            const float m = fminf(pc->nx[k] * lx, pc->nx[k] * hx) + fminf(pc->ny[k] * ly, pc->ny[k] * hy)
                + fminf(pc->nz[k] * lz, pc->nz[k] * hz);
            worst = fmaxf(worst, m);
        }
        const float front = fmaxf(pc->ax * lx, pc->ax * hx) + fmaxf(pc->ay * ly, pc->ay * hy)
            + fmaxf(pc->az * lz, pc->az * hz);
        return !(worst > slack) && !(front < -slack) && pencil_may_hit(cluster_sphere(blo, bhi), *pc);
    } else {
        return beam_may_hit(cluster_sphere(blo, bhi), bm, 1.52587890625e-05f );
    }
}

typedef uint32_t plan_u32x4 __attribute__((ext_vector_type(4)));
typedef int plan_i32x2 __attribute__((ext_vector_type(2)));
template <typename T>
__device__ __forceinline__ const __attribute__((address_space(4))) T* plan_const(const void* p)
{
    return (const __attribute__((address_space(4))) T*)(uintptr_t)p;
}

template <int N>
struct WeightedB {
    float x, y;
    float w[N + 1];
    __device__ WeightedB(const float2 b) : x(b.x), y(b.y), w{} {}
};

template <int MODE, bool SPLIT, bool ALT = false, bool LAT = false, bool PLANNED = false>
__global__ __launch_bounds__(TRACE_BLOCK, !f4_class_split(MODE) ? 1
                                          : weighted(MODE) ? (channels(MODE) == 1 ? 6 : 7 - channels(MODE))
                                          : (SPLIT ? 8 : 6))
void trace_kernel(const TraceArgs a)
{
    static_assert(!ALT || f4_integrals(MODE), "no alternative path for this mode");
    static_assert(!LAT || has_lattice(MODE), "no lattice cull for this mode");
    static_assert(!PLANNED || (SPLIT && !LAT && f4_sums(MODE)), "planned: class-split column densities only");
    if constexpr (PLANNED) {
        if (*plan_const<uint32_t>(a.plan_usable) == 0u) return;
    } else if (has_lattice(MODE)) {
        if (a.plan_usable && *a.plan_usable != 0u) return;
        if (a.lat_dev ? (*a.lat_dev != 0) != LAT : LAT) return;
        if (a.stage_dev && *a.stage_dev != a.stage_want) return;
    }
    constexpr bool FAST = ALT && f4_sums(MODE);
    constexpr bool WEIGHTED = weighted(MODE);
    constexpr int NW = channels(MODE), WP = WEIGHTED ? (NW + 1) / 2 : 0;
    using BRec = std::conditional_t<WEIGHTED, WeightedB<NW>, float2>;
    __shared__ double2 s_lut[FAST ? 1 : N_TABLE];
    constexpr int LUTF_N = 256;
    __shared__ float2 s_lutf[FAST ? LUTF_N : 1];
    constexpr bool D4 = primitive(MODE) == PRIM_D4, F4D = primitive(MODE) == PRIM_F4D;
    constexpr bool LDS_TILE = primitive(MODE) == PRIM_F4;
    __shared__ __align__(16) float2 s_tile[LDS_TILE ? TRACE_BLOCK / 64 : 1][LDS_TILE ? 3 + WP : 1][LDS_TILE ? 66 : 1];
    __shared__ double s_tile_d[D4 ? TRACE_BLOCK / 64 : 1][D4 ? 64 : 1][D4 ? 6 : 1];
    __shared__ float4 s_tile_f[F4D ? TRACE_BLOCK / 64 : 1][F4D ? 64 : 1][F4D ? 2 : 1];
    const int lane = threadIdx.x & 63;
    static_assert(!SPLIT || class_split(MODE) || MODE == MODE_HITS, "triangle and stats walks do not split");
    constexpr bool RANGE_SPLIT = SPLIT && MODE == MODE_HITS;
    const int split_ordinary = !SPLIT ? 1 : (!RANGE_SPLIT && a.split_dev) ? *a.split_dev : a.split;
    int split_planned = 0;
    if constexpr (PLANNED)
        if (a.plan_split_dev) split_planned = *plan_const<int>(a.plan_split_dev);
    const int split = PLANNED && split_planned > 0 ? split_planned : split_ordinary;
    const int n_packets = (a.n_rays + a.width - 1) / a.width;
    const int nb = (n_packets * split + TRACE_BLOCK / 64 - 1) / (TRACE_BLOCK / 64);
    const int q = nb >> 3, r8 = nb & 7, xcd = blockIdx.x & 7, slot = blockIdx.x >> 3;
    if (slot >= q + (xcd < r8 ? 1 : 0)) return;
    const int vblock = (xcd < r8 ? xcd * (q + 1) : r8 * (q + 1) + (xcd - r8) * q) + slot;
    const int wave_id = __builtin_amdgcn_readfirstlane(vblock * (TRACE_BLOCK / 64)
                                                       + (threadIdx.x >> 6));
    if (integrates(MODE)) {
        if (FAST) {
            static_assert(TRACE_BLOCK >= 256, "one table entry per thread");
            float2 e = make_float2(0.f, 0.f);
            if (threadIdx.x < N_TABLE - 1) {
                const double y0 = a.kernel_table[threadIdx.x], dy = a.kernel_table[threadIdx.x + 1] - y0;
                e = make_float2(float(y0 - double(threadIdx.x) * dy), float(dy));
            }
            if (threadIdx.x < LUTF_N) s_lutf[threadIdx.x] = e;
        } else if (threadIdx.x < N_TABLE) {
            const int i0 = threadIdx.x;
            const double y0 = a.kernel_table[i0];
            const double y1 = i0 + 1 < N_TABLE ? a.kernel_table[i0 + 1] : y0;
            s_lut[threadIdx.x] = make_double2(y0, y1 - y0);
        }
        __syncthreads();
    }
    int packet = wave_id / split, part = wave_id - packet * split;
    int prim_lo = 0, prim_hi = 0x7fffffff;
    if (RANGE_SPLIT) {
        if (wave_id >= *a.n_wave_map) return;
        const int4 wm = a.wave_map[wave_id];
        packet = wm.x; part = 0;
        prim_lo = wm.y << a.chunk_shift;
        prim_hi = wm.z << a.chunk_shift;
        if (prim_lo >= prim_hi) return;
    }
    const int first_ray = packet * a.width;
    if (first_ray >= a.n_rays) return;
    const int classes_per_part = SUM_CLASSES / split;
    const int own_lo = part * classes_per_part, own_hi = own_lo + classes_per_part;
    auto owns_granule = [&](const int g) {
        if (RANGE_SPLIT) { const int p = g << GRANULE_SHIFT; return p >= prim_lo && p < prim_hi; }
        const int c = g & (SUM_CLASSES - 1);
        return c >= own_lo && c < own_hi;
    };
    auto foreign_range = [&](const int first, const int count) {
        if (RANGE_SPLIT) return first + count <= prim_lo || first >= prim_hi;
        const int g0 = first >> GRANULE_SHIFT, g1 = (first + count - 1) >> GRANULE_SHIFT;
        return g1 - g0 <= 1 && !owns_granule(g0) && !owns_granule(g1);
    };
    const PacketRay ray = load_packet_ray(a, first_ray, lane);
    const bool valid = ray.valid;
    const int ray_index = ray.index;
    const float dx = ray.dx, dy = ray.dy, dz = ray.dz;
    const float ox = ray.ox, oy = ray.oy, oz = ray.oz;
    const float len = ray.len;
    const float ix = 1.f / dx, iy = 1.f / dy, iz = 1.f / dz;
    const Beam beam = packet_beam(ray);
    int axis = -1;
    if (!ordered(MODE)) axis = packet_axis(dx, dy, dz);
    __shared__ Pencil s_pencil[TRACE_BLOCK / 64];
    Pencil pencil;
    bool is_pencil = false;
    if (!PLANNED && axis < 0 && MODE != MODE_STATS && beam.olo[0] == beam.ohi[0] && beam.olo[1] == beam.ohi[1]
        && beam.olo[2] == beam.ohi[2]) {
        float sx = dx, sy = dy, sz = dz;
#pragma unroll
        for (int off = 32; off > 0; off >>= 1) {
            sx += __shfl_xor(sx, off); sy += __shfl_xor(sy, off); sz += __shfl_xor(sz, off);
        }
        const float inv = 1.0f / sqrtf(sx * sx + sy * sy + sz * sz);
        const float ax = sx * inv, ay = sy * inv, az = sz * inv;
        const float cx = ay * dz - az * dy, cy = az * dx - ax * dz, cz = ax * dy - ay * dx;
        const float sin_t = wave_max(sqrtf(cx * cx + cy * cy + cz * cz)) + 2e-6f;
        const float cos_min = wave_min(ax * dx + ay * dy + az * dz);
        if (cos_min > 0.5f && sin_t < 0.8660254f) {
            is_pencil = true;
            pencil.ox = beam.olo[0]; pencil.oy = beam.olo[1]; pencil.oz = beam.olo[2];
            pencil.ax = ax; pencil.ay = ay; pencil.az = az;
            pencil.sin_t = sin_t;
            pencil.cos_t = sqrtf(1.0f - sin_t * sin_t);
            float ux, uy, uz;
            if (fabsf(ax) <= fabsf(ay) && fabsf(ax) <= fabsf(az)) { ux = 0.f; uy = -az; uz = ay; }
            else if (fabsf(ay) <= fabsf(az)) { ux = az; uy = 0.f; uz = -ax; }
            else { ux = -ay; uy = ax; uz = 0.f; }
            const float un = 1.0f / sqrtf(ux * ux + uy * uy + uz * uz);
            ux *= un; uy *= un; uz *= un;
            const float vx = ay * uz - az * uy, vy = az * ux - ax * uz, vz = ax * uy - ay * ux;
            const float da_ = ax * dx + ay * dy + az * dz;
            const float tu = (ux * dx + uy * dy + uz * dz) / da_, tv = (vx * dx + vy * dy + vz * dz) / da_;
            const float m = 4e-6f;
            const float tu_lo = wave_min(tu) - m, tu_hi = wave_max(tu) + m;
            const float tv_lo = wave_min(tv) - m, tv_hi = wave_max(tv) + m;
            auto plane = [&](int k, float cu, float cv, float ca) {
                float px = cu * ux + cv * vx + ca * ax, py = cu * uy + cv * vy + ca * ay,
                      pz = cu * uz + cv * vz + ca * az;
                const float pn = 1.0f / sqrtf(px * px + py * py + pz * pz);
                pencil.nx[k] = px * pn; pencil.ny[k] = py * pn; pencil.nz[k] = pz * pn;
            };
            plane(0, 1.f, 0.f, -tu_hi);
            plane(1, -1.f, 0.f, tu_lo);
            plane(2, 0.f, 1.f, -tv_hi);
            plane(3, 0.f, -1.f, tv_lo);
            if (lane == 0) s_pencil[threadIdx.x >> 6] = pencil;
        }
    }
    const AxisRay ar = axis_ray(axis, ray);
    const float oa = ar.oa, da = ar.da, noda = ar.noda, o1 = ar.o1, o2 = ar.o2;
    float noda_lo = 0.f, noda_hi = 0.f, len_lo = 0.f, da0 = 0.f;
    bool same_sense = false;
    if (axis >= 0) axis_extremes(ar, len, noda_lo, noda_hi, len_lo, da0, same_sense);
    const float fat_r2 = FAST && axis >= 0 ? fat_radius2(axis, beam) : INFINITY;
    const int treelet = axis >= 0 ? a.treelet_axis : a.treelet;
    constexpr bool LATTICE = LAT;
    __shared__ float s_lat[LATTICE ? TRACE_BLOCK / 64 : 1][2][8];
    __shared__ float s_lat_r2[LATTICE ? TRACE_BLOCK / 64 : 1];
    if (LATTICE && lane == 0) s_lat_r2[threadIdx.x >> 6] = 0.f;
    if (LATTICE && axis >= 0) {
        bool ok;
        float cell2;
        build_origin_lattice(o1, o2, lane, s_lat, ok, cell2);
        if (lane == 0) s_lat_r2[threadIdx.x >> 6] = ok ? cell2 : 0.f;
    }

    int count = 0;
    constexpr bool CHUNKED = SPLIT && chunked(MODE);
    int cur_chunk = -1;
    int count_at_chunk = 0;
    float sum = 0.f;
    float wsum[NW] = {};
    constexpr bool CLASSES_F = f4_sums(MODE), CLASSES_D = double_sums(MODE);
    constexpr bool CLASSES = output(MODE) == OUT_SUMS || WEIGHTED;
    __shared__ float s_class[CLASSES_F ? TRACE_BLOCK / 64 : 1][CLASSES_F ? SUM_CLASSES * NW : 1][CLASSES_F ? 64 : 1];
    __shared__ double s_class_d[CLASSES_D ? TRACE_BLOCK / 64 : 1][CLASSES_D ? SUM_CLASSES : 1][CLASSES_D ? 64 : 1];
    const int wv_acc = threadIdx.x >> 6;
    if (CLASSES_F) {
#pragma unroll
        for (int c = 0; c < SUM_CLASSES * NW; ++c) s_class[wv_acc][c][lane] = 0.f;
    }
    if (CLASSES_D) {
#pragma unroll
        for (int c = 0; c < SUM_CLASSES; ++c) s_class_d[wv_acc][c][lane] = 0.0;
    }
    double sum_d = 0.0;
    int cur_granule = -1;
    int cur_granule_end = 0;
    bool cur_owned = true;
    auto enter_granule = [&](const int prim) {
        if (cur_granule >= 0) {
            if constexpr (WEIGHTED) {
#pragma unroll
                for (int c = 0; c < NW; ++c) s_class[wv_acc][(cur_granule & (SUM_CLASSES - 1)) * NW + c][lane] = wsum[c];
            } else {
            if (CLASSES_D) s_class_d[wv_acc][cur_granule & (SUM_CLASSES - 1)][lane] = sum_d;
            else s_class[wv_acc][cur_granule & (SUM_CLASSES - 1)][lane] = sum;
            }
        }
        cur_granule = prim >> GRANULE_SHIFT;
// ... 861 lines not shown
```

### grace-devel_amd/csrc/trace_planned.hip

```cpp
#include "trace_kernel.hpp"

#include <vector>

using namespace grace_hip;

namespace {

struct PlanRef {
    uint4* entries;
    const int2* spans;
    int* counts;
    PlanCtl* ctl;
    int force;
};

template <bool FUSED>
__global__ __launch_bounds__(TRACE_BLOCK) void plan_record_kernel(const TraceArgs a, const PlanRef pl)
{
    __shared__ float s_lat[TRACE_BLOCK / 64][2][8];
    if (pl.spans && !pl.force && pl.ctl->record == 0u) return;
    const int lane = threadIdx.x & 63, wv = threadIdx.x >> 6;
    const int n_packets = (a.n_rays + a.width - 1) / a.width;
    const int packet = blockIdx.x * (TRACE_BLOCK / 64) + wv;
    if (packet >= n_packets) return;
// ... 33 lines not shown
            const bool g_may = box_may_hit(group_boxes[2 * size_t(gj)], group_boxes[2 * size_t(gj) + 1], true);
            const int n_g = min(64, n_groups - g0);
            unsigned long long gmask = __builtin_amdgcn_ballot_w64(g_may) & (n_g >= 64 ? ~0ull : ((1ull << n_g) - 1ull));
            while (gmask != 0ull) {
                const int g = g0 + __builtin_ctzll(gmask);
                gmask &= gmask - 1ull;
                const int r_lo = g << a.group_shift;
                const int r_hi = r_lo + min(1 << a.group_shift, covered - r_lo);
                const int c_first = r_lo >> 6, c_last = (r_hi - 1) >> 6;
                for (int cg = c_first; cg <= c_last; cg += 64) {
                    const int cj = min(cg + lane, c_last);
                    const bool c_may = box_may_hit(a.C[2 * size_t(cj)], a.C[2 * size_t(cj) + 1], false);
                    const int n_c = min(64, c_last - cg + 1);
                    unsigned long long cmask = __builtin_amdgcn_ballot_w64(c_may)
                        & (n_c >= 64 ? ~0ull : ((1ull << n_c) - 1ull));
                    while (cmask != 0ull) {
                        const int c = cg + __builtin_ctzll(cmask);
                        cmask &= cmask - 1ull;
                        const int pbase = c << 6;
                        const int pj = min(max(pbase + lane, r_lo), r_hi - 1);
                        const float4 mine = a.A[pj];
                        const int lo_bit = max(r_lo - pbase, 0), hi_bit = min(r_hi - pbase, 64);
                        const unsigned long long m_mask =
                            (hi_bit >= 64 ? ~0ull : ((1ull << hi_bit) - 1ull)) & (~0ull << lo_bit);
                        const float s1 = axis == 0 ? mine.y : mine.x;
                        const float s2 = axis == 2 ? mine.y : mine.z;
                        const float sa = axis == 0 ? mine.x : axis == 1 ? mine.y : mine.z;
                        const float q1 = s1 - __builtin_amdgcn_fmed3f(s1, lo1, hi1);
                        const float q2 = s2 - __builtin_amdgcn_fmed3f(s2, lo2, hi2);
                        const float b2_lo = FUSED ? __builtin_fmaf(q1, q1, q2 * q2) : q1 * q1 + q2 * q2;
                        bool keep = !(b2_lo >= mine.w);
                        unsigned long long rest = __builtin_amdgcn_ballot_w64(keep) & m_mask;
                        keep = __builtin_amdgcn_inverse_ballot_w64(rest);
                        if (rest != 0ull && __builtin_amdgcn_ballot_w64(keep && mine.w < lat_r2) != 0ull) {
                            float p1 = INFINITY, p2 = INFINITY;
                            for (int k = 0; k < 8; ++k) {
                                p1 = fminf(p1, fabsf(s1 - s_lat[wv][0][k]));
                                p2 = fminf(p2, fabsf(s2 - s_lat[wv][1][k]));
                            }
                            const float nan_if_nan = (s1 + s2) * 0.0f;
                            const float l2 = (FUSED ? __builtin_fmaf(p1, p1, p2 * p2) : p1 * p1 + p2 * p2) + nan_if_nan;
                            keep = keep && !(l2 >= mine.w);
                            rest = __builtin_amdgcn_ballot_w64(keep);
                        }
                        if (rest == 0ull) continue;
                        const unsigned long long inside =
                            __builtin_amdgcn_ballot_w64(__builtin_fmaf(sa, da0, noda_lo) >= 0.0f)
                            & __builtin_amdgcn_ballot_w64(__builtin_fmaf(sa, da0, noda_hi) < len_lo);
                        const bool lean = same_sense && (rest & ~inside) == 0ull;
                        const bool fat = FUSED && (rest & ~__builtin_amdgcn_ballot_w64(mine.w >= fat_r2)) == 0ull;
                        const int cls = (c >> (GRANULE_SHIFT - 6)) & (SUM_CLASSES - 1);
                        const int n = __builtin_amdgcn_readlane(cnt, cls);
                        const int bits = (lean ? 1 : 0) | (fat ? 2 : 0);
                        const int n_surv = __builtin_popcountll(rest);
                        const int open_n = __builtin_amdgcn_readlane(round_n, cls);
                        const int open_bits = __builtin_amdgcn_readlane(round_bits, cls);
                        const bool close_cap = n > 0 && open_n + n_surv > 64;
                        const bool close_flag = n > 0 && !close_cap && open_bits != bits;
                        const bool close = close_cap || close_flag;
                        if (pl.spans) {
                            const int2 span = pl.spans[packet * SUM_CLASSES + cls];
                            if (n < span.y) {
                                if (lane == 0) {
                                    if (close) pl.entries[size_t(span.x) + n - 1].w = uint32_t(open_bits) | PLAN_ROUND_END;
                                    pl.entries[size_t(span.x) + n] =
                                        make_uint4(uint32_t(c), uint32_t(rest), uint32_t(rest >> 32), uint32_t(bits));
                                }
                            } else {
                                failed = true;
                            }
                        }
                        if (lane == cls) {
                            if (close) {
                                t_rounds += 1; t_full += open_n == 64 ? 1 : 0;
                                t_cap += close_cap ? 1 : 0; t_flag += close_flag ? 1 : 0;
                                t_max = max(t_max, open_n);
                                round_n = 0;
                            }
                            round_n += n_surv; round_bits = bits;
                            t_surv += n_surv;
                            cnt += 1;
                        }
                    }
                }
            }
        }
    }
    if (failed) {
        cnt = 0;
        if (lane == 0) { pl.ctl->unusable = 1u; pl.ctl->usable = 0u; }
    }
    if (lane < SUM_CLASSES) pl.counts[packet * SUM_CLASSES + lane] = cnt;
    if (pl.spans && !failed) {
        for (int cls = 0; cls < SUM_CLASSES; ++cls) {
            const int n = __builtin_amdgcn_readlane(cnt, cls);
            const int open_bits = __builtin_amdgcn_readlane(round_bits, cls);
            if (n > 0 && lane == 0)
                pl.entries[size_t(pl.spans[packet * SUM_CLASSES + cls].x) + n - 1].w = uint32_t(open_bits) | PLAN_ROUND_END;
        }
        if (lane < SUM_CLASSES && cnt > 0) {
            t_rounds += 1; t_full += round_n == 64 ? 1 : 0;
            t_max = max(t_max, round_n);
        }
        if (lane >= SUM_CLASSES) cnt = 0;
        int tally[6] = { cnt, t_surv, t_rounds, t_full, t_cap, t_flag };
#pragma unroll
        for (int off = 1; off < SUM_CLASSES; off <<= 1) {
#pragma unroll
            for (int k = 0; k < 6; ++k) tally[k] += __shfl_xor(tally[k], off);
            t_max = max(t_max, __shfl_xor(t_max, off));
        }
        if (lane == 0) {
#pragma unroll
            for (int k = 0; k < 6; ++k)
                if (tally[k]) atomicAdd(&pl.ctl->stats[k], (unsigned long long)tally[k]);
            atomicMax(&pl.ctl->largest_round, uint32_t(t_max));
        }
    }
}

grace_status launch_record(const bool fast, const TraceArgs& a, const PlanRef& pl, hipStream_t stream)
{
    const int n_packets = (a.n_rays + a.width - 1) / a.width;
    const int grid = ceil_div(size_t(n_packets), size_t(TRACE_BLOCK / 64));
    if (fast) plan_record_kernel<true><<<grid, TRACE_BLOCK, 0, stream>>>(a, pl);
    else plan_record_kernel<false><<<grid, TRACE_BLOCK, 0, stream>>>(a, pl);
    GRACE_CHECK_LAUNCH();
    return GRACE_OK;
}

grace_status plan_free_buffers(PacketPlan& pp)
{
    void* bufs[] = { pp.entries, pp.spans, pp.counts, pp.ctl };
    bool any = false;
    for (void* b : bufs) any = any || b;
    if (any) GRACE_TRY_HIP(hipDeviceSynchronize());
    for (void* b : bufs)
        if (b) GRACE_TRY_HIP(hipFree(b));
    pp.entries = nullptr; pp.spans = nullptr; pp.counts = nullptr; pp.ctl = nullptr;
    pp.valid = false;
    pp.n_lists = pp.n_entries = pp.recorded = 0;
    return GRACE_OK;
}

}

namespace grace_hip {

grace_status plan_release(TraceState& ts)
{
    GRACE_TRY(plan_free_buffers(ts.plan));
    ts.plan = PacketPlan();
    ts.last_plan_ctl = nullptr;
    return GRACE_OK;
}

grace_status plan_fill(TraceState& ts, const PlanKey& key, const TraceArgs& a, hipStream_t stream)
{
    PacketPlan& pp = ts.plan;
    GRACE_TRY(plan_free_buffers(pp));
    ts.last_plan_ctl = nullptr;
    pp.key = key;
    pp.dead = true;
    const int n_packets = (a.n_rays + a.width - 1) / a.width;
    const size_t n_lists = size_t(n_packets) * SUM_CLASSES;
    auto alloc = [&](auto*& ptr, const size_t bytes) {
        if (hipMalloc(reinterpret_cast<void**>(&ptr), bytes) == hipSuccess) return true;
        (void)hipGetLastError();
        ptr = nullptr;
        return false;
    };
    if (n_lists * (sizeof(int) + sizeof(int2)) > ts.plan_budget) return GRACE_OK;
    if (!alloc(pp.counts, n_lists * sizeof(int)) || !alloc(pp.spans, n_lists * sizeof(int2))
        || !alloc(pp.ctl, sizeof(PlanCtl)))
        return plan_free_buffers(pp);
    GRACE_TRY_HIP(hipMemsetAsync(pp.ctl, 0, sizeof(PlanCtl), stream));
    GRACE_TRY(launch_record(key.fast, a, PlanRef{ nullptr, nullptr, pp.counts, pp.ctl, 1 }, stream));
    std::vector<int> counts(n_lists);
    PlanCtl seen = {};
    GRACE_TRY_HIP(hipMemcpyAsync(counts.data(), pp.counts, n_lists * sizeof(int), hipMemcpyDeviceToHost, stream));
    GRACE_TRY_HIP(hipMemcpyAsync(&seen, pp.ctl, sizeof(seen), hipMemcpyDeviceToHost, stream));
    GRACE_TRY_HIP(hipStreamSynchronize(stream));
    if (seen.unusable) return plan_free_buffers(pp);
    std::vector<int2> spans(n_lists);
    size_t total = 0, used = 0;
    for (size_t l = 0; l < n_lists; ++l) {
        const size_t room = size_t(counts[l]) + size_t(counts[l]) / 8 + 2;
        spans[l] = make_int2(int(total), int(room));
        total += room;
        used += size_t(counts[l]);
        if (total >= (size_t(1) << 31)) return plan_free_buffers(pp);
    }
    const size_t bytes = (total + 4) * sizeof(uint4) + n_lists * (sizeof(int) + sizeof(int2));
    if (bytes > ts.plan_budget || !alloc(pp.entries, (total + 4) * sizeof(uint4))) return plan_free_buffers(pp);
    GRACE_TRY_HIP(hipMemcpy(pp.spans, spans.data(), n_lists * sizeof(int2), hipMemcpyHostToDevice));
    GRACE_TRY_HIP(hipMemsetAsync(pp.entries + total, 0, 4 * sizeof(uint4), stream));
    pp.n_lists = n_lists; pp.n_entries = total; pp.recorded = used;
    GRACE_TRY_HIP(hipMemsetD32Async(reinterpret_cast<hipDeviceptr_t>(&pp.ctl->usable), 1, 1, stream));
    GRACE_TRY_HIP(hipMemcpyAsync(&pp.ctl->sig[0], ts.scene.ctl->sig, 16, hipMemcpyDeviceToDevice, stream));
    GRACE_TRY_HIP(hipMemcpyAsync(&pp.ctl->sig[2], ts.rays.ctl->sig, 16, hipMemcpyDeviceToDevice, stream));
    GRACE_TRY(launch_record(key.fast, a, PlanRef{ pp.entries, pp.spans, pp.counts, pp.ctl, 1 }, stream));
    pp.valid = true;
    pp.dead = false;
    return GRACE_OK;
}

grace_status plan_record(const TraceState& ts, const TraceArgs& a, hipStream_t stream)
{
    const PacketPlan& pp = ts.plan;
    return launch_record(pp.key.fast, a, PlanRef{ pp.entries, pp.spans, pp.counts, pp.ctl, 0 }, stream);
}

grace_status launch_planned(const int mode, const bool fast, const int grid, const TraceArgs& a, hipStream_t stream)
{
    auto go = [&](auto mode_tag) {
        constexpr int MODE = decltype(mode_tag)::value;
        if (fast) trace_kernel<MODE, true, true, false, true><<<grid, TRACE_BLOCK, 0, stream>>>(a);
        else trace_kernel<MODE, true, false, false, true><<<grid, TRACE_BLOCK, 0, stream>>>(a);
    };
    switch (mode) {
    case MODE_CUMULATIVE: go(std::integral_constant<int, MODE_CUMULATIVE>()); break;
    case MODE_WCUM1: go(std::integral_constant<int, MODE_WCUM1>()); break;
    case MODE_WCUM2: go(std::integral_constant<int, MODE_WCUM2>()); break;
    case MODE_WCUM3: go(std::integral_constant<int, MODE_WCUM3>()); break;
    case MODE_WCUM4: go(std::integral_constant<int, MODE_WCUM4>()); break;
    default: return set_error(GRACE_INVALID_ARGUMENT, __FILE__, __LINE__, "no planned kernel for this mode");
    }
    GRACE_CHECK_LAUNCH();
    return GRACE_OK;
}

}
```

### grace-devel_amd/csrc/trace_state.hpp

```cpp
#pragma once

#include "common.hpp"

namespace grace_hip {

constexpr int TRACE_BLOCK = 256;
constexpr int N_TABLE = 51;
constexpr int SPLIT_WIDE_BUDGET = 0x100;

inline int group_shift(size_t n_prims)
{
    int s = 12;
    while (((n_prims + (size_t(1) << s) - 1) >> s) > 4096) ++s;
    return s;
}
inline size_t group_count(size_t n_prims)
{
    const int s = group_shift(n_prims);
    return (n_prims + (size_t(1) << s) - 1) >> s;
}
inline size_t cluster_record_count(size_t n_prims)
{
    return 2 * ((n_prims + 63) / 64) + 1 + 2 * group_count(n_prims);
}
constexpr int MAX_HIT_CHUNKS = 256;
constexpr int SUM_CLASSES = 8;
constexpr int GRANULE_SHIFT = 10;


enum { MODE_COUNT = 0, MODE_CUMULATIVE = 1, MODE_HITS = 2, MODE_STATS = 3, MODE_TRI = 4,
       MODE_COUNT_D4 = 5, MODE_CUM_D4 = 6, MODE_HITS_D4 = 7,
       MODE_COUNT_F4D = 8, MODE_CUM_F4D = 9, MODE_HITS_F4D = 10,
       MODE_WCUM1 = 11, MODE_WCUM2 = 12, MODE_WCUM3 = 13, MODE_WCUM4 = 14 };

enum Primitive { PRIM_F4 = 0,
                 PRIM_TRI = 1,
                 PRIM_D4 = 2,
                 PRIM_F4D = 3 };
enum Output { OUT_COUNTS, OUT_SUMS, OUT_HITS, OUT_STATS, OUT_CLOSEST,
              OUT_WSUMS };

struct ModeParts { Primitive prim; Output out; int channels = 1; };
constexpr ModeParts mode_parts(const int mode)
{
    switch (mode) {
    case MODE_COUNT:      return { PRIM_F4, OUT_COUNTS };
    case MODE_CUMULATIVE: return { PRIM_F4, OUT_SUMS };
    case MODE_HITS:       return { PRIM_F4, OUT_HITS };
    case MODE_STATS:      return { PRIM_F4, OUT_STATS };
    case MODE_TRI:        return { PRIM_TRI, OUT_CLOSEST };
    case MODE_COUNT_D4:   return { PRIM_D4, OUT_COUNTS };
    case MODE_CUM_D4:     return { PRIM_D4, OUT_SUMS };
    case MODE_HITS_D4:    return { PRIM_D4, OUT_HITS };
    case MODE_COUNT_F4D:  return { PRIM_F4D, OUT_COUNTS };
    case MODE_CUM_F4D:    return { PRIM_F4D, OUT_SUMS };
    case MODE_HITS_F4D:   return { PRIM_F4D, OUT_HITS };
    case MODE_WCUM1:      return { PRIM_F4, OUT_WSUMS, 1 };
    case MODE_WCUM2:      return { PRIM_F4, OUT_WSUMS, 2 };
    case MODE_WCUM3:      return { PRIM_F4, OUT_WSUMS, 3 };
    case MODE_WCUM4:      return { PRIM_F4, OUT_WSUMS, 4 };
    }
    __builtin_unreachable();
}
constexpr Primitive primitive(const int mode) { return mode_parts(mode).prim; }
constexpr Output output(const int mode) { return mode_parts(mode).out; }
constexpr int channels(const int mode) { return mode_parts(mode).channels; }
constexpr int MAX_LAUNCH_CHANNELS = 4;
constexpr bool weighted(const int mode) { return output(mode) == OUT_WSUMS; }

constexpr bool fp64(const int mode) { return primitive(mode) == PRIM_D4 || primitive(mode) == PRIM_F4D; }
constexpr bool class_split(const int mode)
{
    return output(mode) == OUT_COUNTS || output(mode) == OUT_SUMS || output(mode) == OUT_WSUMS;
}
constexpr bool f4_class_split(const int mode) { return class_split(mode) && primitive(mode) == PRIM_F4; }
constexpr bool f4_sums(const int mode)
{
    return primitive(mode) == PRIM_F4 && (output(mode) == OUT_SUMS || output(mode) == OUT_WSUMS);
}
constexpr bool double_sums(const int mode) { return output(mode) == OUT_SUMS && fp64(mode); }
constexpr bool ordered(const int mode) { return output(mode) == OUT_HITS || output(mode) == OUT_CLOSEST; }
constexpr bool integrates(const int mode)
{
    return output(mode) == OUT_SUMS || output(mode) == OUT_WSUMS || output(mode) == OUT_HITS;
}
constexpr bool f4_integrals(const int mode) { return integrates(mode) && primitive(mode) == PRIM_F4; }
constexpr bool has_lattice(const int mode) { return primitive(mode) == PRIM_F4 && output(mode) != OUT_STATS; }
constexpr bool chunked(const int mode)
{
    return primitive(mode) == PRIM_F4 && (output(mode) == OUT_COUNTS || output(mode) == OUT_HITS);
}

struct TraceArgs {
    const float* rays;
    const uint32_t* perm;
    int n_rays;
    const float4* spheres;
    const int2* node_prims;
    int treelet;
    int treelet_axis;
    const float4* A;
    const float2* B;
    int group_shift;
    const float4* C;
    const double* T64;
    const double* spheres_d;
    double* out_sums_d;
    double* hit_integral_d;
    double* hit_dist_d;
    int split;
    int n_prims;
    float* partial;
    double* partial_d;
    const int* split_dev;
    const int* lat_dev;
    const int* stage_dev;
    int stage_want;
    int* chunk_counts;
    const int* chunk_off;
    const int4* wave_map;
    const int* n_wave_map;
    bool keep_chunks;
    int chunk_shift, n_chunks;
    int width;
    const float4* nodes;
    int n_nodes;
    const int4* leaves;
    const int* root;
    int* out_counts;
    float* out_sums;
    const int* offsets;
    int* hit_idx;
    float* hit_integral;
    float* hit_dist;
    uint32_t* stats;
    int* status;
    const float* weights;
    int w_stride;
    int out_stride;
    const double* kernel_table;
    const uint4* plan_entries;
    const int2* plan_spans;
    const int* plan_counts;
    const uint32_t* plan_usable;
    const int* plan_split_dev;
};


struct CacheCtl {
    unsigned long long sig[2];
    uint32_t stale;
    uint32_t pad;
};

struct SceneKey {
    Primitive kind = PRIM_F4;
    const void* prims = nullptr; const void* nodes = nullptr; const void* leaves = nullptr;
    size_t n_prims = 0, n_nodes = 0;
    bool operator==(const SceneKey& o) const
    {
        return kind == o.kind && prims == o.prims && nodes == o.nodes && leaves == o.leaves
            && n_prims == o.n_prims && n_nodes == o.n_nodes;
    }
};

struct Scene {
    bool valid = false;
    SceneKey key;
    SceneKey seen;
    float4* A = nullptr; float2* B1 = nullptr; float2* B50 = nullptr; double* T64 = nullptr;
    int2* node_prims = nullptr; float4* C = nullptr;
    CacheCtl* ctl = nullptr;
    bool pinned = false;
    unsigned long long gen = 0;
};

struct RayKey {
    const float* rays = nullptr;
    size_t n = 0;
    bool operator==(const RayKey& o) const { return rays == o.rays && n == o.n; }
};

struct RayOrder {
    bool valid = false;
    RayKey key, seen;
    uint32_t* perm = nullptr;
    uint32_t* ext = nullptr;
    CacheCtl* ctl = nullptr;
    bool pinned = false;
    unsigned long long gen = 0;
};

struct PlanCtl {
    uint32_t record;
    uint32_t unusable;
    uint32_t usable;
    uint32_t largest_round;
    unsigned long long sig[4];
    unsigned long long stats[6];
};
constexpr uint32_t PLAN_ROUND_END = 4u;
constexpr int PLAN_FORMAT = 2;

struct PlanKey {
    int format = PLAN_FORMAT;
    bool fast = false;
    int group_shift = 0, width = 0;
    bool reorder = false;
    size_t n_rays = 0, n_prims = 0;
    unsigned long long scene_gen = 0, rays_gen = 0;
    bool operator==(const PlanKey& o) const
    {
        return format == o.format && fast == o.fast && group_shift == o.group_shift && width == o.width && reorder == o.reorder
            && n_rays == o.n_rays && n_prims == o.n_prims && scene_gen == o.scene_gen && rays_gen == o.rays_gen;
    }
};

struct PacketPlan {
    bool valid = false;
    bool dead = false;
    PlanKey key;
    uint4* entries = nullptr;
    int2* spans = nullptr;
    int* counts = nullptr;
    PlanCtl* ctl = nullptr;
    size_t n_lists = 0, n_entries = 0;
    size_t recorded = 0;
};

struct PlanGate {
    const CacheCtl* scene = nullptr;
    const CacheCtl* rays = nullptr;
    PlanCtl* ctl = nullptr;
};

__host__ __device__ inline int planned_split(const int n_packets)
{
    return n_packets <= 8192 ? SUM_CLASSES : SUM_CLASSES / 2;
}

struct HitsCache {
    int* chunk_counts = nullptr;
    size_t capacity = 0;
    bool valid = false;
    const void* rays = nullptr; const void* prims = nullptr;
    size_t n_rays = 0, n_prims = 0;
    int n_chunks = 0;
};

struct TraceState {
    int* status = nullptr;
    const int* last_lat_dev = nullptr;
    hipStream_t last_lat_stream = nullptr;
    bool timing = false;
    hipEvent_t ev0 = nullptr, ev1 = nullptr;
    bool ev_valid = false;
    bool ray_reorder = true;
    int treelet = -1;
    int split = -1;
    int lat_split = 4;
    int width = -1;
    bool exact_integrals = false;
    bool hits_stage_split = true;
    bool cache_validation = true;
    bool cache_auto = true;
    int sph_kernel = 0;
    const double* builtin_tables = nullptr;
    const double* kernel_table = nullptr;
    double* custom_table = nullptr;
    double custom_host[N_TABLE] = {};
    bool plan_on = true;
    size_t plan_budget = size_t(512) << 20;
    Scene scene;
    RayOrder rays;
    HitsCache hits;
    unsigned long long cache_gen = 0;
    PacketPlan plan;
    const PlanCtl* last_plan_ctl = nullptr;
    hipStream_t last_plan_stream = nullptr;
};

grace_status trace_state(TraceState** out);

inline grace_status ensure_status(TraceState& ts, hipStream_t stream)
{
    if (!ts.status) {
        GRACE_TRY_HIP(hipMalloc(reinterpret_cast<void**>(&ts.status), sizeof(int)));
        GRACE_TRY_HIP(hipMemsetAsync(ts.status, 0, sizeof(int), stream));
    }
    return GRACE_OK;
}

template <typename Launches>
grace_status timed(TraceState& ts, hipStream_t stream, Launches launches)
{
    if (ts.timing) {
        if (!ts.ev0) { GRACE_TRY_HIP(hipEventCreate(&ts.ev0)); GRACE_TRY_HIP(hipEventCreate(&ts.ev1)); }
        GRACE_TRY_HIP(hipEventRecord(ts.ev0, stream));
    }
    GRACE_TRY(launches());
    if (ts.timing) {
        GRACE_TRY_HIP(hipEventRecord(ts.ev1, stream));
        ts.ev_valid = true;
    }
    return GRACE_OK;
}

size_t sig_partial_words();
struct SigRequest {
    const void* prims = nullptr; size_t prims_bytes = 0;
    const void* nodes = nullptr; size_t nodes_bytes = 0;
    const void* leaves = nullptr; size_t leaves_bytes = 0;
    CacheCtl* scene_ctl = nullptr; bool scene_force = false;
    const void* rays = nullptr; size_t rays_bytes = 0;
    CacheCtl* rays_ctl = nullptr; bool rays_force = false;
    uint32_t* rays_ext = nullptr;
};
grace_status launch_signatures(const SigRequest& rq, unsigned long long* partial, hipStream_t stream);

grace_status scene_release(TraceState& ts);
grace_status scene_cache_alloc(TraceState& ts, const SceneKey& key);
grace_status scene_fill(Primitive kind, const void* prims, size_t n_prims, const float4* nodes,
                        size_t n_nodes, const int4* leaves, float4* A, float2* B1, float2* B50,
                        double* T64, int2* node_prims, float4* C, hipStream_t stream,
                        const uint32_t* run_if = nullptr);
grace_status scene_prepare(TraceState& ts, Primitive kind, const void* prims, size_t n_prims,
                           const int* d_nodes, size_t n_nodes, const int* d_leaves, hipStream_t stream);

grace_status rays_release(TraceState& ts);
grace_status rays_cache_alloc(TraceState& ts, const RayKey& key);
grace_status ray_order(const float* d_rays, size_t n_rays, uint32_t* ext, uint32_t* keys, uint32_t* perm,
                       const float4* scene_min, uint32_t* lat_flag, int n_packets, int split, int* split_dev,
                       hipStream_t stream, const uint32_t* run_if = nullptr);
grace_status rays_prepare(TraceState& ts, const float* d_rays, size_t n_rays, hipStream_t stream);
grace_status launch_choose_variants(const uint32_t* ext12, int n, const float4* scene_min, uint32_t* lat_flag,
                                    int split_packets, int split_launched, int* split_dev, hipStream_t stream,
                                    const PlanGate* gate = nullptr, int* plan_split_dev = nullptr);

grace_status plan_release(TraceState& ts);
grace_status plan_fill(TraceState& ts, const PlanKey& key, const TraceArgs& a, hipStream_t stream);
grace_status plan_record(const TraceState& ts, const TraceArgs& a, hipStream_t stream);
grace_status launch_planned(int mode, bool fast, int grid, const TraceArgs& a, hipStream_t stream);

}
```

### grace-devel_amd/grace_hip/__init__.py

```python
import collections
import ctypes as C
import os

import numpy as np
import torch

_HERE = os.path.dirname(os.path.abspath(__file__))
LIB_PATH = os.path.join(os.path.dirname(_HERE), "lib", "libgrace_hip.so")

if not os.path.exists(LIB_PATH):
    raise ImportError(
        "libgrace_hip.so is not built (%s). Run __graft_entry__.build() or "
        "`make -C grace-devel_amd`. There is no CPU fallback." % LIB_PATH)

_lib = C.CDLL(LIB_PATH)
_lib.grace_last_error.restype = C.c_char_p
_lib.grace_version.restype = C.c_int

GRACE_OK = 0
GRACE_INVALID_ARGUMENT = 1
GRACE_HIP_ERROR = 2
GRACE_OUT_OF_MEMORY = 3
GRACE_STACK_OVERFLOW = 4

# ... 165 lines not shown
def ALBVH_sph(spheres, deltas, tree):
    n = len(spheres)
    assert tree.leaves.shape[0] >= n and len(deltas) == n + 1
    n_leaves = C.c_size_t(0)
    fn = {torch.float32: _lib.grace_albvh_build_f4, torch.float64: _lib.grace_albvh_build_f4_f64,
          torch.int32: _lib.grace_albvh_build_f4_u32,
          torch.int64: _lib.grace_albvh_build_f4_u64}.get(deltas.dtype)
    if fn is None:
        raise ValueError("deltas must be float32/float64 or 32/64-bit XOR deltas")
    _check(fn(_ptr(_spheres(spheres)), C.c_size_t(n), _ptr(deltas), C.c_int(tree.max_per_leaf),
              _ptr(tree.nodes), _ptr(tree.leaves), _ptr(tree.root_index), C.byref(n_leaves),
              _stream()))
    tree.leaves = tree.leaves[: n_leaves.value]
    tree.nodes = tree.nodes[: n_leaves.value - 1]
    return tree


PRIM_SPHERE_F4, PRIM_TRIANGLE, PRIM_SPHERE_D4, PRIM_BOX = 0, 1, 2, 3
COMP_LESS, COMP_GREATER = 0, 1
_DELTA_CODES = {torch.float32: 0, torch.float64: 1, torch.int32: 2, torch.int64: 3}


def build_ALBVH(tree, prims, deltas, prim_kind=PRIM_SPHERE_F4, delta_comp=COMP_LESS):
    n = len(prims)
    assert tree.leaves.shape[0] >= n and len(deltas) == n + 1
    if deltas.dtype not in _DELTA_CODES:
        raise ValueError("deltas must be float32/float64 or 32/64-bit XOR deltas")
    n_leaves = C.c_size_t(0)
    _check(_lib.grace_albvh_build_ex(C.c_int(prim_kind), _ptr(prims), C.c_size_t(n),
                                     C.c_int(_DELTA_CODES[deltas.dtype]), _ptr(deltas), C.c_int(delta_comp),
                                     C.c_int(tree.max_per_leaf), _ptr(tree.nodes), _ptr(tree.leaves),
                                     _ptr(tree.root_index), C.byref(n_leaves), _stream()))
    tree.leaves = tree.leaves[: n_leaves.value]
    tree.nodes = tree.nodes[: n_leaves.value - 1]
    return tree


def min_max_components(data, n_comp, first=0):
    code = {torch.float32: 0, torch.float64: 1, torch.int32: 2}[data.dtype]
    assert data.dim() == 2 and data.is_contiguous() and first + n_comp <= data.shape[1]
    npdt = {0: np.float32, 1: np.float64, 2: np.int32}[code]
    lo = np.zeros(n_comp, npdt); hi = np.zeros(n_comp, npdt)
    elem = data.element_size()
    _check(_lib.grace_minmax_components(C.c_void_p(data.data_ptr() + first * elem), C.c_size_t(len(data)),
                                        C.c_int(code), C.c_int(n_comp), C.c_size_t(data.shape[1] * elem),
                                        lo.ctypes.data_as(C.c_void_p), hi.ctypes.data_as(C.c_void_p), _stream()))
    return lo, hi


def build_tree(spheres, tree, low=None, high=None, want_perm=False):
    deltas = torch.empty(len(spheres) + 1, dtype=torch.float32, device=spheres.device)
    keys = torch.empty(len(spheres), dtype=torch.int32, device=spheres.device)
    morton_keys_sph(spheres, keys, low, high)
    perm = sort_by_key(keys, spheres, 0, 30, want_perm=want_perm)
    euclidean_deltas_sph(spheres, deltas)
    ALBVH_sph(spheres, deltas, tree)
    return (tree, perm) if want_perm else tree


def _check_rays(rays):
    _rays(rays)
    if len(rays) % 32 != 0:
        raise ValueError("Number of rays must be a multiple of the warp size (32).")


def _trace_args(rays, spheres, tree):
    return (_ptr(rays), C.c_size_t(len(rays)), _ptr(_spheres(spheres)), C.c_size_t(len(spheres)),
            _ptr(tree.nodes), C.c_size_t(tree.n_nodes), _ptr(tree.leaves), _ptr(tree.root_index))


def hit_integrals(b2, h):
    out = torch.empty_like(b2)
    _check(_lib.grace_hit_integrals_f32(_ptr(b2), _ptr(h), C.c_size_t(len(b2)), _ptr(out), _stream()))
    return out


def enable_kernel_timing(enabled=True):
    _check(_lib.grace_trace_enable_timing(C.c_int(1 if enabled else 0)))


def last_kernel_ms():
    ms = C.c_float(0)
    _check(_lib.grace_trace_last_kernel_ms(C.byref(ms)))
    return ms.value


def last_lattice():
    v = C.c_int(0)
    _check(_lib.grace_trace_last_lattice(C.byref(v)))
    return v.value


def set_packet_split(k):
    _check(_lib.grace_trace_set_packet_split(C.c_int(int(k))))


def set_packet_width(w):
    _check(_lib.grace_trace_set_packet_width(C.c_int(int(w))))


def set_exact_integrals(enabled):
    _check(_lib.grace_trace_set_exact_integrals(C.c_int(1 if enabled else 0)))


SPH_KERNELS = ("cubic", "quartic", "quintic", "wendland_c2", "wendland_c4", "wendland_c6")
SPH_KERNEL_CUSTOM = -1


def _kernel_kind(name):
    if name not in SPH_KERNELS:
        raise ValueError("unknown SPH kernel %r (one of %s)" % (name, ", ".join(SPH_KERNELS)))
    return SPH_KERNELS.index(name)


def sph_kernel_table(name):
    out = (C.c_double * N_TABLE)()
    _check(_lib.grace_sph_kernel_table(C.c_int(_kernel_kind(name)), out))
    return np.array(out, np.float64)


def set_sph_kernel(kernel):
    if isinstance(kernel, str):
        _check(_lib.grace_trace_set_sph_kernel(C.c_int(_kernel_kind(kernel))))
        return
    t = np.asarray(kernel)
    if t.dtype.kind not in "fiu" or t.ndim != 1:
        raise ValueError("an SPH kernel table must be a 1-D array of 51 numbers")
    t = np.ascontiguousarray(t, dtype=np.float64)
    _check(_lib.grace_trace_set_sph_kernel_table(t.ctypes.data_as(C.POINTER(C.c_double)), C.c_int(len(t))))


def sph_kernel():
    kind = C.c_int(0)
    out = (C.c_double * N_TABLE)()
    _check(_lib.grace_trace_get_sph_kernel(C.byref(kind), out))
    name = "custom" if kind.value == SPH_KERNEL_CUSTOM else SPH_KERNELS[kind.value]
    return name, np.array(out, np.float64)


def set_cache_validation(enabled):
    _check(_lib.grace_trace_set_cache_validation(C.c_int(1 if enabled else 0)))


def set_cache_auto(enabled):
    _check(_lib.grace_trace_set_cache_auto(C.c_int(1 if enabled else 0)))


def set_plan(enabled):
    _check(_lib.grace_trace_set_plan(C.c_int(1 if enabled else 0)))


def set_plan_budget(n_bytes):
    _check(_lib.grace_trace_set_plan_budget(C.c_size_t(int(n_bytes))))


def plan_bytes():
    v = C.c_size_t(0)
    _check(_lib.grace_trace_plan_bytes(C.byref(v)))
    return v.value


def last_plan_used():
    v = C.c_int(0)
    _check(_lib.grace_trace_last_plan_used(C.byref(v)))
    return v.value


PlanStats = collections.namedtuple(
    "PlanStats", "entries survivors rounds full_rounds closed_by_capacity closed_by_flags largest_round")


def plan_stats():
    v = (C.c_ulonglong * 7)()
    _check(_lib.grace_trace_plan_stats(v))
    return PlanStats(*[int(x) for x in v])


def set_lattice_split(k):
    _check(_lib.grace_trace_set_lattice_split(C.c_int(k)))


def set_hits_staging(enabled):
    _check(_lib.grace_trace_set_hits_staging(C.c_int(1 if enabled else 0)))


class Context:

    def __init__(self):
        self._h = C.c_void_p(0)
        _check(_lib.grace_context_create(C.byref(self._h)))

    def make_current(self):
        _check(_lib.grace_context_set_current(self._h))

    @staticmethod
    def reset_current():
        _check(_lib.grace_context_set_current(C.c_void_p(0)))

    def destroy(self):
        if self._h:
            _check(_lib.grace_context_destroy(self._h))
            self._h = C.c_void_p(0)

    def __enter__(self):
        self.make_current()
        return self

    def __exit__(self, *exc):
        Context.reset_current()
        self.destroy()
        return False


def set_treelet_size(n):
    _check(_lib.grace_trace_set_treelet_size(C.c_int(int(n))))


def set_ray_reorder(enabled):
    _check(_lib.grace_trace_set_ray_reorder(C.c_int(1 if enabled else 0)))


def trace_status():
    _check(_lib.grace_trace_status(_stream()))


_prepared = {}


def trace_prepare(spheres, tree):
    _check(_lib.grace_trace_prepare_f4(_ptr(_spheres(spheres)), C.c_size_t(len(spheres)),
                                       _ptr(tree.nodes), C.c_size_t(tree.n_nodes),
                                       _ptr(tree.leaves), _stream()))
    _prepared["scene"] = (spheres, tree.nodes, tree.leaves)


def trace_prepare_tri(tris, tree):
    _check(_lib.grace_trace_prepare_tri(_ptr(_tris(tris)), C.c_size_t(len(tris)),
                                        _ptr(tree.nodes), C.c_size_t(tree.n_nodes),
                                        _ptr(tree.leaves), _stream()))
    _prepared["scene"] = (tris, tree.nodes, tree.leaves)


def trace_prepare_rays(rays):
    _check(_lib.grace_trace_prepare_rays(_ptr(_rays(rays)), C.c_size_t(len(rays)), _stream()))
    _prepared["rays"] = rays


def trace_release_rays():
    _check(_lib.grace_trace_release_rays())
    _prepared.pop("rays", None)


def trace_release():
    _check(_lib.grace_trace_release())
    _prepared.pop("scene", None)


def _trace_hitcounts_keep(rays, spheres, tree, hit_counts, real=torch.float32):
    _check_rays(rays)
    fn = _lib.grace_trace_hitcounts_f4_f64 if real == torch.float64 else _lib.grace_trace_hitcounts_keep_f4
    _check(fn(*_trace_args(rays, spheres, tree), _ptr(hit_counts), _stream()))
    return hit_counts


def _real_of(real):
    assert real in (torch.float32, torch.float64), "real: torch.float32 or torch.float64"
    return real


def trace_hitcounts_f4_f64(rays, spheres, tree, hit_counts, check=False):
    _check_rays(rays)
    assert hit_counts.dtype == torch.int32 and len(hit_counts) == len(rays)
    _check(_lib.grace_trace_hitcounts_f4_f64(*_trace_args(rays, spheres, tree), _ptr(hit_counts), _stream()))
    if check:
        trace_status()
    return hit_counts


def trace_hitcounts_sph(rays, spheres, tree, hit_counts, check=False):
    _check_rays(rays)
    assert hit_counts.dtype == torch.int32 and len(hit_counts) == len(rays)
    _check(_lib.grace_trace_hitcounts_f4(*_trace_args(rays, spheres, tree), _ptr(hit_counts),
                                         _stream()))
    if check:
        trace_status()
    return hit_counts


def trace_cumulative_sph(rays, spheres, tree, cumulated, check=False):
    _check_rays(rays)
    assert cumulated.dtype in (torch.float32, torch.float64) and len(cumulated) == len(rays)
    fn = _lib.grace_trace_cumulative_f4_f64 if cumulated.dtype == torch.float64 else _lib.grace_trace_cumulative_f4
    _check(fn(*_trace_args(rays, spheres, tree), _ptr(cumulated), _stream()))
    if check:
        trace_status()
    return cumulated


def trace_cumulative_weighted_sph(rays, spheres, tree, weights, out=None, check=False):
    _check_rays(rays)
    if weights.dtype != torch.float32:
        raise ValueError("weights must be float32")
    if weights.dim() not in (1, 2) or weights.shape[0] != len(spheres):
        raise ValueError("weights must have shape [n_spheres] or [n_spheres, C]")
    n_ch = 1 if weights.dim() == 1 else weights.shape[1]
    if not 1 <= n_ch <= 64:
# ... 734 lines not shown
```

### include/grace_hip.h

```cpp
#ifndef GRACE_HIP_H
#define GRACE_HIP_H

#include <stddef.h>
#include <stdint.h>

#ifdef __cplusplus
extern "C" {
#endif

typedef enum grace_status {
    GRACE_OK = 0,
    GRACE_INVALID_ARGUMENT = 1,
    GRACE_HIP_ERROR = 2,
    GRACE_OUT_OF_MEMORY = 3,
    GRACE_STACK_OVERFLOW = 4
} grace_status;

typedef void* grace_stream;

int grace_version(void);
const char* grace_last_error(void);

grace_status grace_device_malloc(void** d_ptr, size_t bytes);
grace_status grace_device_free(void* d_ptr);
// ... 64 lines not shown
} grace_sort_stats;
grace_status grace_sort_last_stats(grace_sort_stats* h_stats);

grace_status grace_deltas_euclid_f4(const float* d_spheres, size_t n, float* d_deltas,
                                    grace_stream stream);
grace_status grace_deltas_area_f4(const float* d_spheres, size_t n, float* d_deltas,
                                  grace_stream stream);
grace_status grace_deltas_xor_u32(const uint32_t* d_keys, size_t n, uint32_t* d_deltas,
                                  grace_stream stream);
grace_status grace_deltas_xor_u64(const uint64_t* d_keys, size_t n, uint64_t* d_deltas,
                                  grace_stream stream);

grace_status grace_albvh_build_f4(const float* d_spheres, size_t n, const float* d_deltas,
                                  int max_per_leaf, int* d_nodes, int* d_leaves, int* d_root,
                                  size_t* h_n_leaves, grace_stream stream);
grace_status grace_albvh_build_f4_u32(const float* d_spheres, size_t n, const uint32_t* d_deltas,
                                      int max_per_leaf, int* d_nodes, int* d_leaves,
                                      int* d_root, size_t* h_n_leaves, grace_stream stream);

grace_status grace_centroid_bounds_tri(const float* d_tris, size_t n, float* h_bot, float* h_top,
                                       grace_stream stream);
grace_status grace_morton_keys30_tri(const float* d_tris, size_t n, const float* h_bot,
                                     const float* h_top, uint32_t* d_keys, grace_stream stream);
grace_status grace_albvh_build_tri_u32(const float* d_tris, size_t n, const uint32_t* d_deltas,
                                       int max_per_leaf, int* d_nodes, int* d_leaves, int* d_root,
                                       size_t* h_n_leaves, grace_stream stream);

enum { GRACE_PRIM_SPHERE_F4 = 0, GRACE_PRIM_TRIANGLE = 1, GRACE_PRIM_SPHERE_D4 = 2, GRACE_PRIM_BOX = 3 };
enum { GRACE_DELTA_F32 = 0, GRACE_DELTA_F64 = 1, GRACE_DELTA_U32 = 2, GRACE_DELTA_U64 = 3 };
enum { GRACE_COMP_LESS = 0, GRACE_COMP_GREATER = 1 };
grace_status grace_albvh_build_ex(int prim_kind, const void* d_prims, size_t n, int delta_type,
                                  const void* d_deltas, int delta_comp, int max_per_leaf,
                                  int* d_nodes, int* d_leaves, int* d_root, size_t* h_n_leaves,
                                  grace_stream stream);

grace_status grace_albvh_enable_timing(int enabled);
grace_status grace_albvh_last_phase_ms(float* h_leaves_ms, float* h_nodes_ms);
grace_status grace_trace_closest_tri(const void* d_rays, size_t n_rays, const float* d_tris,
                                     size_t n_tris, const int* d_nodes, size_t n_nodes,
                                     const int* d_leaves, const int* d_root, int* d_closest,
                                     grace_stream stream);

grace_status grace_trace_hitcounts_f4(const void* d_rays, size_t n_rays, const float* d_spheres,
                                      size_t n_spheres, const int* d_nodes, size_t n_nodes,
                                      const int* d_leaves, const int* d_root,
                                      int* d_hit_counts, grace_stream stream);
grace_status grace_trace_hitcounts_keep_f4(const void* d_rays, size_t n_rays, const float* d_spheres,
                                           size_t n_spheres, const int* d_nodes, size_t n_nodes,
                                           const int* d_leaves, const int* d_root,
                                           int* d_hit_counts, grace_stream stream);
grace_status grace_trace_cumulative_f4(const void* d_rays, size_t n_rays, const float* d_spheres,
                                       size_t n_spheres, const int* d_nodes, size_t n_nodes,
                                       const int* d_leaves, const int* d_root,
                                       float* d_cumulated, grace_stream stream);
grace_status grace_trace_cumulative_weighted_f4(const void* d_rays, size_t n_rays, const float* d_spheres,
                                                size_t n_spheres, const int* d_nodes, size_t n_nodes,
                                                const int* d_leaves, const int* d_root,
                                                const float* d_weights, int n_channels, float* d_out,
                                                grace_stream stream);
grace_status grace_trace_emission_absorption_f4(const void* d_rays, size_t n_rays, const float* d_spheres,
                                                size_t n_spheres, const int* d_nodes, size_t n_nodes,
                                                const int* d_leaves, const int* d_root,
                                                const float* d_emission, int n_channels,
                                                const float* d_absorption, float* d_out, float* d_tau,
                                                grace_stream stream);
grace_status grace_trace_absorption_deposit_f4(const void* d_rays, size_t n_rays, const float* d_spheres,
                                               size_t n_spheres, const int* d_nodes, size_t n_nodes,
                                               const int* d_leaves, const int* d_root,
                                               const float* d_luminosity, const float* d_absorption,
                                               int n_channels, double* d_deposit, float* d_transmitted,
                                               double* d_quantum, grace_stream stream);
typedef struct grace_spectrum_grid {
    double v0;
    double dv;
    int    n_bins;
    int    periodic;
    double hubble;
} grace_spectrum_grid;
grace_status grace_trace_spectra_f4(const void* d_rays, size_t n_rays, const float* d_spheres,
                                    size_t n_spheres, const int* d_nodes, size_t n_nodes,
                                    const int* d_leaves, const int* d_root,
                                    const float* d_amount, const float* d_width, const float* d_velocity,
                                    int n_channels, const grace_spectrum_grid* grid, float* d_tau,
                                    float* d_column, grace_stream stream);
grace_status grace_trace_set_ordered_budget(size_t bytes);
grace_status grace_trace_ordered_limits(int* wave_max_hits, int* block_max_hits);
typedef struct grace_ordered_stats {
    unsigned long long batches;
    unsigned long long total_hits;
    unsigned long long rays_wave, rays_block, rays_global;
    unsigned long long budget_bytes, frame_bytes;
    float ms_count, ms_trace, ms_composite;
} grace_ordered_stats;
grace_status grace_trace_ordered_enable_stats(int enabled);
grace_status grace_trace_ordered_last_stats(grace_ordered_stats* h_stats);
grace_status grace_trace_hits_f4(const void* d_rays, size_t n_rays, const float* d_spheres,
                                 size_t n_spheres, const int* d_nodes, size_t n_nodes,
                                 const int* d_leaves, const int* d_root,
                                 const int* d_ray_offsets, int* d_hit_indices,
                                 float* d_hit_integrals, float* d_hit_distances,
                                 grace_stream stream);
grace_status grace_trace_stats_f4(const void* d_rays, size_t n_rays, const float* d_spheres,
                                  size_t n_spheres, const int* d_nodes, size_t n_nodes,
                                  const int* d_leaves, const int* d_root,
                                  uint32_t* d_stats4, grace_stream stream);

grace_status grace_hit_integrals_f32(const float* d_b2, const float* d_h, size_t n, float* d_out,
                                     grace_stream stream);

grace_status grace_trace_set_ray_reorder(int enabled);

grace_status grace_trace_enable_timing(int enabled);
grace_status grace_trace_last_kernel_ms(float* h_ms);

grace_status grace_trace_last_lattice(int* h_lattice);

grace_status grace_trace_set_packet_split(int waves_per_packet);

grace_status grace_trace_set_packet_width(int rays_per_packet);

grace_status grace_trace_set_exact_integrals(int enabled);

#define GRACE_SPH_KERNEL_CUSTOM      (-1)
#define GRACE_SPH_KERNEL_CUBIC       0
#define GRACE_SPH_KERNEL_QUARTIC     1
#define GRACE_SPH_KERNEL_QUINTIC     2
#define GRACE_SPH_KERNEL_WENDLAND_C2 3
#define GRACE_SPH_KERNEL_WENDLAND_C4 4
#define GRACE_SPH_KERNEL_WENDLAND_C6 5
grace_status grace_trace_set_sph_kernel(int kind);
grace_status grace_trace_set_sph_kernel_table(const double* h_table, int n);
grace_status grace_trace_get_sph_kernel(int* h_kind, double* h_table51);
grace_status grace_sph_kernel_table(int kind, double* h_out51);

grace_status grace_trace_set_treelet_size(int max_primitives);

grace_status grace_trace_set_lattice_split(int waves_per_packet);
grace_status grace_trace_set_hits_staging(int enabled);

grace_status grace_trace_prepare_f4(const float* d_spheres, size_t n_spheres, const int* d_nodes,
                                    size_t n_nodes, const int* d_leaves, grace_stream stream);
grace_status grace_trace_prepare_tri(const float* d_tris, size_t n_tris, const int* d_nodes,
                                     size_t n_nodes, const int* d_leaves, grace_stream stream);
grace_status grace_trace_release(void);
grace_status grace_trace_prepare_rays(const void* d_rays, size_t n_rays, grace_stream stream);
grace_status grace_trace_release_rays(void);
grace_status grace_trace_set_cache_validation(int enabled);
grace_status grace_trace_set_cache_auto(int enabled);

grace_status grace_trace_set_plan(int on);
grace_status grace_trace_set_plan_budget(size_t bytes);
grace_status grace_trace_plan_bytes(size_t* h_bytes);
grace_status grace_trace_last_plan_used(int* h_used);
grace_status grace_trace_plan_stats(unsigned long long* h_stats );

grace_status grace_trace_status(grace_stream stream);

grace_status grace_scan_exclusive_i32(const int* d_in, size_t n, int* d_out, long long* h_total,
                                      grace_stream stream);
grace_status grace_segscan_exclusive_f32(const int* d_segment_offsets, size_t n_segments,
                                         const float* d_data, size_t n, float* d_results,
                                         grace_stream stream);
grace_status grace_segscan_exclusive_f64(const int* d_segment_offsets, size_t n_segments,
                                         const double* d_data, size_t n, double* d_results,
                                         grace_stream stream);
grace_status grace_add_iota_i32(int* d_values, size_t n, grace_stream stream);
grace_status grace_fill_u32(void* d_values, size_t n, uint32_t bits, grace_stream stream);
grace_status grace_multiply_by_weights_f32(const float* d_unweighted, size_t n,
                                           const float* d_weights, const uint32_t* d_weight_map,
                                           float* d_weighted, grace_stream stream);
grace_status grace_multiply_by_weights_f64(const double* d_unweighted, size_t n,
                                           const double* d_weights, const uint32_t* d_weight_map,
                                           double* d_weighted, grace_stream stream);

grace_status grace_sort_by_distance_f32(float* d_distances, const int* d_ray_offsets,
                                        size_t n_rays, size_t n_hits, int* d_hit_indices,
                                        float* d_hit_data, grace_stream stream);

grace_status grace_sort_by_distance_f64(double* d_distances, const int* d_ray_offsets,
                                        size_t n_rays, size_t n_hits, int* d_hit_indices,
                                        double* d_hit_data, grace_stream stream);

grace_status grace_rays_orthogonal_z(int n_side, const float* h_mins4, const float* h_maxs4,
                                     void* d_rays, float* h_area, grace_stream stream);
grace_status grace_rays_pinhole(int res_x, int res_y, const float* h_camera, const float* h_look_at,
                                const float* h_view_up, float fovy, float length, void* d_rays,
                                grace_stream stream);
grace_status grace_rays_healpix(int nside, float ox, float oy, float oz, float length,
                                void* d_rays, grace_stream stream);
grace_status grace_rays_isotropic(size_t n_rays, float ox, float oy, float oz, float length,
                                  uint64_t seed, void* d_rays, grace_stream stream);

grace_status grace_rays_isotropic_octant(size_t n_rays, float ox, float oy, float oz, float length,
                                         int octant, uint64_t seed, void* d_rays,
                                         grace_stream stream);
grace_status grace_rays_one_to_many(size_t n_rays, float ox, float oy, float oz,
                                    const void* d_points, int is_double, int elems_per_point,
                                    int sort_type, const float* h_bot, const float* h_top,
                                    void* d_rays, grace_stream stream);
grace_status grace_rays_plane_parallel_random(int width, int height, const float* h_base,
                                              const float* h_w, const float* h_h, float length,
                                              uint64_t seed, void* d_rays, grace_stream stream);
grace_status grace_rays_orthographic_projection(int res_x, int res_y, const float* h_camera,
                                                const float* h_look_at, const float* h_view_up,
                                                float vertical_extent, float length,
                                                void* d_rays, grace_stream stream);

grace_status grace_deltas_euclid_d4(const double* d_spheres, size_t n, float* d_deltas,
                                    grace_stream stream);
grace_status grace_deltas_euclid_d4_f64(const double* d_spheres, size_t n, double* d_deltas,
                                        grace_stream stream);
grace_status grace_deltas_area_d4(const double* d_spheres, size_t n, float* d_deltas,
                                  grace_stream stream);
grace_status grace_deltas_area_d4_f64(const double* d_spheres, size_t n, double* d_deltas,
                                      grace_stream stream);
grace_status grace_albvh_build_f4_u64(const float* d_spheres, size_t n, const uint64_t* d_deltas,
                                      int max_per_leaf, int* d_nodes, int* d_leaves, int* d_root,
                                      size_t* h_n_leaves, grace_stream stream);
grace_status grace_albvh_build_f4_f64(const float* d_spheres, size_t n, const double* d_deltas,
                                      int max_per_leaf, int* d_nodes, int* d_leaves, int* d_root,
                                      size_t* h_n_leaves, grace_stream stream);
grace_status grace_albvh_build_d4_f64(const double* d_spheres, size_t n, const double* d_deltas,
                                      int max_per_leaf, int* d_nodes, int* d_leaves, int* d_root,
                                      size_t* h_n_leaves, grace_stream stream);
grace_status grace_albvh_build_d4_u32(const double* d_spheres, size_t n, const uint32_t* d_deltas,
                                      int max_per_leaf, int* d_nodes, int* d_leaves, int* d_root,
                                      size_t* h_n_leaves, grace_stream stream);
grace_status grace_albvh_build_d4_u64(const double* d_spheres, size_t n, const uint64_t* d_deltas,
                                      int max_per_leaf, int* d_nodes, int* d_leaves, int* d_root,
                                      size_t* h_n_leaves, grace_stream stream);
grace_status grace_albvh_build_d4(const double* d_spheres, size_t n, const float* d_deltas,
                                  int max_per_leaf, int* d_nodes, int* d_leaves, int* d_root,
                                  size_t* h_n_leaves, grace_stream stream);
grace_status grace_trace_hitcounts_d4(const void* d_rays, size_t n_rays, const double* d_spheres,
                                      size_t n_spheres, const int* d_nodes, size_t n_nodes,
                                      const int* d_leaves, const int* d_root, int* d_hit_counts,
                                      grace_stream stream);
grace_status grace_trace_cumulative_d4(const void* d_rays, size_t n_rays, const double* d_spheres,
                                       size_t n_spheres, const int* d_nodes, size_t n_nodes,
                                       const int* d_leaves, const int* d_root, double* d_sums,
                                       grace_stream stream);
grace_status grace_trace_hits_d4(const void* d_rays, size_t n_rays, const double* d_spheres,
                                 size_t n_spheres, const int* d_nodes, size_t n_nodes,
                                 const int* d_leaves, const int* d_root, const int* d_ray_offsets,
                                 int* d_hit_indices, double* d_hit_integrals,
                                 double* d_hit_distances, grace_stream stream);
grace_status grace_trace_status_d4(grace_stream stream);

grace_status grace_trace_hitcounts_f4_f64(const void* d_rays, size_t n_rays, const float* d_spheres,
                                          size_t n_spheres, const int* d_nodes, size_t n_nodes,
                                          const int* d_leaves, const int* d_root, int* d_hit_counts,
                                          grace_stream stream);
grace_status grace_trace_cumulative_f4_f64(const void* d_rays, size_t n_rays, const float* d_spheres,
                                           size_t n_spheres, const int* d_nodes, size_t n_nodes,
                                           const int* d_leaves, const int* d_root, double* d_sums,
                                           grace_stream stream);
grace_status grace_trace_hits_f4_f64(const void* d_rays, size_t n_rays, const float* d_spheres,
                                     size_t n_spheres, const int* d_nodes, size_t n_nodes,
                                     const int* d_leaves, const int* d_root, const int* d_ray_offsets,
                                     int* d_hit_indices, double* d_hit_integrals,
                                     double* d_hit_distances, grace_stream stream);

grace_status grace_interpolate_points_f4(const float* d_points, size_t n_points, int elems_per_point,
                                         const float* d_spheres, size_t n_spheres, const int* d_nodes,
                                         size_t n_nodes, const int* d_leaves, const int* d_root,
                                         const float* d_weights, int n_channels,
                                         float* d_out, int* d_counts, grace_stream stream);
grace_status grace_interpolate_grid_f4(const float* h_origin3, const float* h_uvw9, const int* h_dims3,
                                       const float* d_spheres, size_t n_spheres, const int* d_nodes,
                                       size_t n_nodes, const int* d_leaves, const int* d_root,
                                       const float* d_weights, int n_channels,
                                       float* d_out, int* d_counts, grace_stream stream);
grace_status grace_interpolate_enable_stats(int enabled);
grace_status grace_interpolate_last_stats(unsigned long long* h_survivor_tests);

grace_status grace_nearest_neighbours_f4(const float* d_points, size_t n_points, int elems_per_point,
                                         const float* d_spheres, size_t n_spheres, const int* d_nodes,
                                         size_t n_nodes, const int* d_leaves, const int* d_root,
                                         int k, int* d_indices, float* d_d2, grace_stream stream);
grace_status grace_smoothing_lengths_f4(const float* d_spheres, size_t n_spheres, const int* d_nodes,
                                        size_t n_nodes, const int* d_leaves, const int* d_root,
                                        int k, float eta, float* d_h, grace_stream stream);
grace_status grace_neighbours_enable_stats(int enabled);
grace_status grace_neighbours_last_stats(unsigned long long* h_candidate_tests, unsigned long long* h_packets,
                                         unsigned long long* h_insertion_steps);

grace_status grace_range_counts_f4(const float* d_points, size_t n_points, int elems_per_point,
                                   const float* d_radii, float radius,
                                   const float* d_spheres, size_t n_spheres, const int* d_nodes,
                                   size_t n_nodes, const int* d_leaves, const int* d_root,
                                   const float* d_weights, int n_channels,
                                   int* d_counts, float* d_sums, grace_stream stream);
grace_status grace_range_neighbours_f4(const float* d_points, size_t n_points, int elems_per_point,
                                       const float* d_radii, float radius,
                                       const float* d_spheres, size_t n_spheres, const int* d_nodes,
                                       size_t n_nodes, const int* d_leaves, const int* d_root,
                                       const int* d_offsets, int* d_indices, float* d_d2,
                                       grace_stream stream);

grace_status grace_fof_labels_f4(const float* d_spheres, size_t n_spheres, const int* d_nodes,
                                 size_t n_nodes, const int* d_leaves, const int* d_root,
                                 float linking_length, int* d_labels, grace_stream stream);
grace_status grace_fof_groups(const int* d_labels, size_t n, int min_members, int* d_group_of,
                              int* d_sizes, int* d_n_groups, grace_stream stream);
grace_status grace_fof_members(const int* d_group_of, size_t n, const int* d_sizes, size_t n_groups,
                               int* d_offsets, int* d_members, grace_stream stream);
// ... 39 lines not shown
```

Baseline: 554.0.

## Fuse cache signature validation into the planned trace kernel speculatively

When the plan, scene and ray caches are all held and validated, the separate signature and check kernels are folded into extra workgroups of the planned trace launch. The last signature block uses a ticket atomic to run the check and set a flag. Trace and combine kernels then gate on that flag instead of the plan usable bit. This removes separate validation launches and their serialization on repeated calls, at the cost of added workgroups, cross-workgroup fences and a more intricate correctness path.

```diff
diff --git a/grace-devel_amd/csrc/trace.hip b/grace-devel_amd/csrc/trace.hip
--- a/grace-devel_amd/csrc/trace.hip
+++ b/grace-devel_amd/csrc/trace.hip
@@ -124,12 +124,14 @@
     uint32_t* ext = nullptr; uint32_t* keys = nullptr; uint32_t* perm = nullptr;
     bool plan_eligible = false;
     PlanKey plan_key;
+    bool speculative = false;
+    int spec_k = 0;
 };
 
-template <int MODE>
+template <int MODE, typename SpecLaunch>
 grace_status use_records(TraceState& ts, TraceArgs& a, TraceBuffers& b, FrameGuard& frame, const LaunchPlan& p,
                          const size_t n_rays, const size_t n_prims, const size_t n_nodes, hipStream_t stream,
-                         const Nested nested = Nested())
+                         const Nested nested, SpecLaunch spec_launch)
 {
     enum CacheUse { USE_NONE, USE_FILL, USE_CHECK, USE_TRUST };
     auto decide = [&](const bool have, const bool pinned, const bool repeat) {
@@ -160,6 +162,11 @@
     const bool plan_steady = b.plan_eligible && ts.plan.valid && ts.plan.key == b.plan_key;
     if (plan_steady) {
         gate.ctl = ts.plan.ctl; gate.scene = ts.scene.ctl; gate.rays = ts.rays.ctl;
+        const bool k_planned = p.dev_split && !weighted(MODE);
+        b.speculative = ts.spec_sig_blocks > 0 && scene_use == USE_CHECK && rays_use == USE_CHECK
+            && (k_planned || !p.dev_split);
+        b.spec_k = k_planned ? planned_split(p.n_packets) : p.split;
+        gate.decided = b.speculative;
     }
     const bool scene_sig = scene_use == USE_FILL || scene_use == USE_CHECK;
     const bool rays_sig = rays_use == USE_FILL || rays_use == USE_CHECK, sig = scene_sig || rays_sig;
@@ -185,7 +192,7 @@
             take(b.pk_prefix, p.hit_packets * size_t(p.hit_chunks));
             take(b.pk_total, p.hit_packets + 16); take(b.pk_first, p.hit_packets + 16); take(b.pk_parts, p.hit_packets + 16);
         }
-        if (p.reorder) { take(b.ext, 20); take(b.keys, n_rays); take(b.perm, n_rays); }
+        if (p.reorder) { take(b.ext, 24); take(b.keys, n_rays); take(b.perm, n_rays); }
         return used;
     };
     const size_t own = carve(nullptr);
@@ -197,6 +204,24 @@
     if (nested.on) GRACE_REQUIRE(Workspace::room() >= need, "trace: the caller's frame is too small for a nested trace");
     else GRACE_TRY(frame.begin(need, stream));
     carve(Workspace::take<char>(own));
+    if (scene_cached) {
+        Scene& sc = ts.scene;
+        a.A = sc.A; a.T64 = sc.T64; a.node_prims = sc.node_prims; a.C = sc.C;
+        a.B = f4_integrals(MODE) ? (p.fast_b ? sc.B50 : sc.B1) : nullptr;
+    } else {
+        a.A = b.A; a.B = b.B; a.T64 = b.T64; a.node_prims = b.node_prims; a.C = b.C;
+    }
+    uint32_t* lat_flag = nullptr;
+    int *split_dev = nullptr, *plan_split_dev = nullptr;
+    if (p.reorder) {
+        lat_flag = p.lattice ? b.ext + 13 : nullptr;
+        split_dev = p.dev_split ? reinterpret_cast<int*>(b.ext + 12) : nullptr;
+        if (rays_cached && b.plan_eligible && split_dev && !weighted(MODE))
+            plan_split_dev = reinterpret_cast<int*>(b.ext + 16);
+        a.perm = rays_cached ? ts.rays.perm : b.perm;
+        a.plan_split_dev = plan_split_dev;
+        a.lat_dev = reinterpret_cast<const int*>(lat_flag); a.split_dev = split_dev;
+    }
     if (sig) {
         SigRequest rq;
         if (scene_sig) {
@@ -209,7 +234,8 @@
             rq.rays = a.rays; rq.rays_bytes = n_rays * 28;
             rq.rays_ctl = ts.rays.ctl; rq.rays_force = rays_use == USE_FILL; rq.rays_ext = ts.rays.ext;
         }
-        GRACE_TRY(launch_signatures(rq, b.sig, stream));
+        if (b.speculative) GRACE_TRY(spec_launch(rq));
+        else GRACE_TRY(launch_signatures(rq, b.sig, stream));
     }
     if (scene_cached) {
         Scene& sc = ts.scene;
@@ -218,18 +244,13 @@
                                  sc.T64, sc.node_prims, sc.C, stream, &sc.ctl->stale));
             sc.valid = true;
         }
-        a.A = sc.A; a.T64 = sc.T64; a.node_prims = sc.node_prims; a.C = sc.C;
-        a.B = f4_integrals(MODE) ? (p.fast_b ? sc.B50 : sc.B1) : nullptr;
     } else {
         GRACE_TRY(scene_fill(skey.kind, primitive(MODE) == PRIM_D4 ? static_cast<const void*>(a.spheres_d) : a.spheres,
                              n_prims, a.nodes, n_nodes, a.leaves, b.A, p.fast_b ? nullptr : b.B, p.fast_b ? b.B : nullptr,
                              b.T64, b.node_prims, b.C, stream));
-        a.A = b.A; a.B = b.B; a.T64 = b.T64; a.node_prims = b.node_prims; a.C = b.C;
     }
     if (p.reorder) {
         const float4* scene_min = a.C + 2 * ((n_prims + 63) / 64);
-        uint32_t* lat_flag = p.lattice ? b.ext + 13 : nullptr;
-        int* split_dev = p.dev_split ? reinterpret_cast<int*>(b.ext + 12) : nullptr;
         const int split_flags = f4_sums(MODE) ? SPLIT_WIDE_BUDGET : 0;
         if (rays_cached) {
             RayOrder& ro = ts.rays;
@@ -238,19 +259,14 @@
                                     stream, &ro.ctl->stale));
                 ro.valid = true;
             }
-            int* plan_split_dev = b.plan_eligible && split_dev && !weighted(MODE)
-                ? reinterpret_cast<int*>(b.ext + 16) : nullptr;
             if (lat_flag || split_dev || plan_steady)
                 GRACE_TRY(launch_choose_variants(ro.ext, int(n_rays), scene_min, lat_flag, p.n_packets,
                                                  p.split | split_flags, split_dev, stream, plan_steady ? &gate : nullptr,
                                                  plan_split_dev));
-            a.perm = ro.perm; a.plan_split_dev = plan_split_dev;
         } else {
             GRACE_TRY(ray_order(a.rays, n_rays, b.ext, b.keys, b.perm, scene_min, lat_flag, p.n_packets,
                                 p.split | split_flags, split_dev, stream));
-            a.perm = b.perm;
-        }
-        a.lat_dev = reinterpret_cast<const int*>(lat_flag); a.split_dev = split_dev;
+        }
     }
     return GRACE_OK;
 }
@@ -268,6 +284,8 @@
                       const int* kept, const size_t n_rays, hipStream_t stream)
 {
     const int grid = ceil_div(size_t(p.n_packets) * p.split, TRACE_BLOCK / 64);
+    TraceArgs o = a;
+    if (b.speculative) o.plan_usable = a.spec.flags + 1;
     const int* const plan_k_dev = a.plan_usable ? a.plan_split_dev : nullptr;
     auto combine = [&](const int k, const int* k_dev, const int* run_if) -> grace_status {
         const int g = ceil_div(n_rays * channels(MODE), 256);
@@ -276,10 +294,10 @@
         else if constexpr (weighted(MODE))
             combine_channel_classes_kernel<<<g, 256, 0, stream>>>(a.partial, int(n_rays), channels(MODE), k, k_dev,
                                                                   a.out_sums, a.out_stride, run_if,
-                                                                  a.plan_usable, plan_k_dev);
+                                                                  o.plan_usable, plan_k_dev);
         else if constexpr (f4_sums(MODE))
             combine_classes_kernel<float><<<g, 256, 0, stream>>>(a.partial, int(n_rays), k, k_dev, a.out_sums, run_if,
-                                                                 a.plan_usable, plan_k_dev);
+                                                                 o.plan_usable, plan_k_dev);
         else return GRACE_OK;
         GRACE_CHECK_LAUNCH();
         return GRACE_OK;
@@ -303,11 +321,13 @@
                 GRACE_TRY(plan_record(ts, a, stream));
                 const int grid_planned = a.plan_split_dev
                     ? ceil_div(size_t(p.n_packets) * planned_split(p.n_packets), TRACE_BLOCK / 64) : grid;
-                GRACE_TRY(launch_planned(MODE, ALT, grid_planned, a, stream));
-                if (p.split == 1) GRACE_TRY(combine(1, nullptr, reinterpret_cast<const int*>(a.plan_usable)));
+                TraceArgs again = a;
+                again.spec.sig_blocks = 0;
+                GRACE_TRY(launch_planned(MODE, ALT, grid_planned, again, stream));
+                if (p.split == 1) GRACE_TRY(combine(1, nullptr, reinterpret_cast<const int*>(o.plan_usable)));
             }
-            if (p.split > 1) launch_walk<MODE, true, ALT>(grid, a, stream);
-            else launch_walk<MODE, false, ALT>(grid, a, stream);
+            if (p.split > 1) launch_walk<MODE, true, ALT>(grid, o, stream);
+            else launch_walk<MODE, false, ALT>(grid, o, stream);
             return GRACE_OK;
         };
         if constexpr (f4_sums(MODE)) GRACE_TRY(p.fast_b ? walk(std::true_type()) : walk(std::false_type()));
@@ -385,13 +405,35 @@
     }
     FrameGuard frame;
     TraceBuffers b;
-    GRACE_TRY(use_records<MODE>(ts, a, b, frame, p, n_rays, n_spheres, n_nodes, stream, nested));
+    auto set_sizes = [&] {
+        a.width = p.width; a.split = p.split; a.treelet = p.treelet; a.treelet_axis = p.treelet_axis;
+        a.n_rays = int(n_rays); a.n_nodes = int(n_nodes); a.n_prims = int(n_spheres); a.status = ts.status;
+        a.group_shift = group_shift(n_spheres); a.chunk_shift = p.hit_chunk_shift; a.n_chunks = p.hit_chunks;
+        a.partial = b.partial; a.partial_d = b.partial_d;
+        a.chunk_off = b.chunk_off; a.wave_map = b.wave_map; a.n_wave_map = b.n_wave_map;
+    };
+    auto use_plan = [&] {
+        const PacketPlan& pp = ts.plan;
+        a.plan_entries = pp.entries; a.plan_spans = pp.spans; a.plan_counts = pp.counts;
+        a.plan_usable = &pp.ctl->usable;
+    };
+    auto spec_launch = [&](const SigRequest& rq) -> grace_status {
+        if constexpr (f4_sums(MODE)) {
+            set_sizes();
+            use_plan();
+            SpecArgs& s = a.spec;
+            sig_build(rq, s.sig, s.check);
+            s.sig_blocks = ts.spec_sig_blocks; s.split = b.spec_k;
+            s.partial = b.sig; s.plan_ctl = ts.plan.ctl; s.flags = b.ext + 17;
+            GRACE_TRY(timed_begin(ts, stream));
+            const int grid = ceil_div(size_t(p.n_packets) * b.spec_k, TRACE_BLOCK / 64) + s.sig_blocks;
+            return launch_planned(MODE, p.fast_b, grid, a, stream);
+        }
+        return GRACE_OK;
+    };
+    GRACE_TRY(use_records<MODE>(ts, a, b, frame, p, n_rays, n_spheres, n_nodes, stream, nested, spec_launch));
     if (nested.measure) return GRACE_OK;
-    a.width = p.width; a.split = p.split; a.treelet = p.treelet; a.treelet_axis = p.treelet_axis;
-    a.n_rays = int(n_rays); a.n_nodes = int(n_nodes); a.n_prims = int(n_spheres); a.status = ts.status;
-    a.group_shift = group_shift(n_spheres); a.chunk_shift = p.hit_chunk_shift; a.n_chunks = p.hit_chunks;
-    a.partial = b.partial; a.partial_d = b.partial_d;
-    a.chunk_off = b.chunk_off; a.wave_map = b.wave_map; a.n_wave_map = b.n_wave_map;
+    set_sizes();
     if (p.split > 1 && output(MODE) == OUT_COUNTS)
         GRACE_TRY_HIP(hipMemsetAsync(a.out_counts, 0, n_rays * sizeof(int), stream));
     if (p.keep_chunks && p.split > 1) {
@@ -401,20 +443,22 @@
         ts.hits.prims = a.spheres; ts.hits.n_prims = n_spheres; ts.hits.n_chunks = p.hit_chunks;
     }
     ts.last_lat_dev = a.lat_dev; ts.last_lat_stream = stream;
+    ts.last_plan_flag = nullptr;
     if constexpr (f4_sums(MODE)) {
         PacketPlan& pp = ts.plan;
         if (b.plan_eligible && !(pp.key == b.plan_key && (pp.valid || pp.dead)))
             GRACE_TRY(plan_fill(ts, b.plan_key, a, stream));
         ts.last_plan_ctl = nullptr;
+        ts.last_plan_flag = nullptr;
         if (b.plan_eligible && pp.valid && pp.key == b.plan_key) {
-            a.plan_entries = pp.entries; a.plan_spans = pp.spans; a.plan_counts = pp.counts;
-            a.plan_usable = &pp.ctl->usable;
+            use_plan();
             ts.last_plan_ctl = pp.ctl; ts.last_plan_stream = stream;
-        }
-    }
-    return timed(ts, stream, [&] {
-        return dispatch<MODE>(ts, a, b, p, reuse_chunks ? ts.hits.chunk_counts : nullptr, n_rays, stream);
-    });
+            if (b.speculative) ts.last_plan_flag = a.spec.flags + 1;
+        }
+    }
+    if (!b.speculative) GRACE_TRY(timed_begin(ts, stream));
+    GRACE_TRY(dispatch<MODE>(ts, a, b, p, reuse_chunks ? ts.hits.chunk_counts : nullptr, n_rays, stream));
+    return timed_end(ts, stream);
 }
 
 TraceArgs trace_args(const void* d_rays, const void* d_prims, const int* d_nodes, const int* d_leaves,
@@ -792,6 +836,11 @@
         GRACE_TRY_HIP(hipStreamSynchronize(ts.last_plan_stream));
         GRACE_TRY_HIP(hipMemcpy(&h, ts.last_plan_ctl, sizeof(h), hipMemcpyDeviceToHost));
         *h_used = h.usable != 0u ? 1 : 0;
+        if (ts.last_plan_flag) {
+            uint32_t ran = 0u;
+            GRACE_TRY_HIP(hipMemcpy(&ran, ts.last_plan_flag, sizeof(ran), hipMemcpyDeviceToHost));
+            *h_used = ran != 0u ? 1 : 0;
+        }
     }
     return GRACE_OK;
 }
@@ -810,6 +859,15 @@
             h_stats[6] = h.largest_round;
         }
     }
+    return GRACE_OK;
+}
+
+grace_status grace_trace_set_signature_blocks(int blocks)
+{
+    GRACE_REQUIRE(blocks >= 0 && blocks <= SIG_GRID && blocks % 8 == 0,
+                  "trace_set_signature_blocks: 0 (off) or a multiple of 8 up to 1024");
+    GRACE_TRACE_STATE();
+    ts.spec_sig_blocks = blocks;
     return GRACE_OK;
 }
 
diff --git a/grace-devel_amd/csrc/trace_cache.hip b/grace-devel_amd/csrc/trace_cache.hip
--- a/grace-devel_amd/csrc/trace_cache.hip
+++ b/grace-devel_amd/csrc/trace_cache.hip
@@ -1,119 +1,21 @@
-#include "trace_state.hpp"
-
-#include <cstdint>
+#include "trace_signature.hpp"
 
 using namespace grace_hip;
 
 namespace {
 
-constexpr int SIG_BLOCK = 256;
-constexpr int SIG_GRID = 1024;
-constexpr int SIG_GROUPS = 2;
-
-struct SigArgs {
-    const uint32_t* base[4];
-    size_t words[4];
-    size_t chunk0[4];
-    int group[4];
-    int aligned[4];
-    int n_arrays;
-};
-
-__device__ __forceinline__ unsigned long long mix64(unsigned long long v)
-{
-    v ^= v >> 32;
-    v *= 0xD6E8FEB86659FD93ull;
-    v ^= v >> 29;
-    return v;
-}
-
 __global__ __launch_bounds__(SIG_BLOCK) void signature_kernel(const SigArgs a,
                                                               unsigned long long* __restrict__ partial)
 {
-    unsigned long long sx[SIG_GROUPS] = { 0ull, 0ull }, sy[SIG_GROUPS] = { 0ull, 0ull };
-    const size_t t0 = blockIdx.x * size_t(blockDim.x) + threadIdx.x, stride = size_t(gridDim.x) * blockDim.x;
-    for (int k = 0; k < a.n_arrays; ++k) {
-        const size_t n_chunks = (a.words[k] + 3) / 4;
-        const uint32_t* w = a.base[k];
-        unsigned long long ax = 0ull, ay = 0ull;
-        for (size_t c = t0; c < n_chunks; c += stride) {
-            uint4 q;
-            if (a.aligned[k] && 4 * c + 4 <= a.words[k]) {
-                q = reinterpret_cast<const uint4*>(w)[c];
-            } else {
-                q.x = 4 * c + 0 < a.words[k] ? w[4 * c + 0] : 0u;
-                q.y = 4 * c + 1 < a.words[k] ? w[4 * c + 1] : 0u;
-                q.z = 4 * c + 2 < a.words[k] ? w[4 * c + 2] : 0u;
-                q.w = 4 * c + 3 < a.words[k] ? w[4 * c + 3] : 0u;
-            }
-            const unsigned long long i = a.chunk0[k] + c;
-            const unsigned long long lo = (unsigned long long)q.x | ((unsigned long long)q.y << 32);
-            const unsigned long long hi = (unsigned long long)q.z | ((unsigned long long)q.w << 32);
-            const unsigned long long x = mix64(lo ^ (i * 0x9E3779B97F4A7C15ull));
-            const unsigned long long y = mix64((hi + ((x << 31) | (x >> 33))) ^ (i * 0xC2B2AE3D27D4EB4Full));
-            ax += x;
-            ay += y;
-        }
-        sx[a.group[k]] += ax;
-        sy[a.group[k]] += ay;
-    }
-    __shared__ unsigned long long s_red[SIG_BLOCK / 64][2 * SIG_GROUPS];
-    const int lane = threadIdx.x & 63, wave = threadIdx.x >> 6;
-#pragma unroll
-    for (int g = 0; g < SIG_GROUPS; ++g) {
-#pragma unroll
-        for (int off = 32; off > 0; off >>= 1) {
-            sx[g] += __shfl_xor(sx[g], off);
-            sy[g] += __shfl_xor(sy[g], off);
-        }
-        if (lane == 0) { s_red[wave][2 * g] = sx[g]; s_red[wave][2 * g + 1] = sy[g]; }
-    }
-    __syncthreads();
-    if (threadIdx.x < 2 * SIG_GROUPS) {
-        unsigned long long v = 0ull;
-        for (int w = 0; w < SIG_BLOCK / 64; ++w) v += s_red[w][threadIdx.x];
-        partial[size_t(blockIdx.x) * 2 * SIG_GROUPS + threadIdx.x] = v;
-    }
+    __shared__ unsigned long long s_red[SIG_LDS_WORDS];
+    signature_block(a, blockIdx.x, gridDim.x, partial, s_red);
 }
-
-struct CheckArgs {
-    CacheCtl* ctl[SIG_GROUPS];
-    int force[SIG_GROUPS];
-    unsigned long long salt[SIG_GROUPS];
-    uint32_t* rays_ext;
-};
 
 __global__ __launch_bounds__(SIG_BLOCK) void signature_check_kernel(const unsigned long long* __restrict__ partial,
                                                                     const CheckArgs a)
 {
-    __shared__ unsigned long long s_red[SIG_BLOCK / 64][2 * SIG_GROUPS];
-    unsigned long long v[2 * SIG_GROUPS] = { 0ull, 0ull, 0ull, 0ull };
-    for (int b = threadIdx.x; b < SIG_GRID; b += blockDim.x)
-#pragma unroll
-        for (int k = 0; k < 2 * SIG_GROUPS; ++k) v[k] += partial[size_t(b) * 2 * SIG_GROUPS + k];
-    const int lane = threadIdx.x & 63, wave = threadIdx.x >> 6;
-#pragma unroll
-    for (int k = 0; k < 2 * SIG_GROUPS; ++k) {
-#pragma unroll
-        for (int off = 32; off > 0; off >>= 1) v[k] += __shfl_xor(v[k], off);
-        if (lane == 0) s_red[wave][k] = v[k];
-    }
-    __syncthreads();
-    if (threadIdx.x < SIG_GROUPS) {
-        const int g = threadIdx.x;
-        CacheCtl* ctl = a.ctl[g];
-        if (ctl) {
-            unsigned long long x = a.salt[g], y = ~a.salt[g];
-            for (int w = 0; w < SIG_BLOCK / 64; ++w) { x += s_red[w][2 * g]; y += s_red[w][2 * g + 1]; }
-            const bool stale = a.force[g] || ctl->sig[0] != x || ctl->sig[1] != y;
-            ctl->sig[0] = x;
-            ctl->sig[1] = y;
-            ctl->stale = stale ? 1u : 0u;
-            if (g == 1 && stale && a.rays_ext) {
-                for (int k = 0; k < 16; ++k) a.rays_ext[k] = k < 6 ? 0xFFFFFFFFu : 0u;
-            }
-        }
-    }
+    __shared__ unsigned long long s_red[SIG_LDS_WORDS];
+    signature_check(partial, SIG_GRID, a, s_red);
 }
 
 }
@@ -122,10 +24,10 @@
 
 size_t sig_partial_words() { return size_t(SIG_GRID) * 2 * SIG_GROUPS; }
 
-grace_status launch_signatures(const SigRequest& rq, unsigned long long* partial, hipStream_t stream)
+void sig_build(const SigRequest& rq, SigArgs& a, CheckArgs& c)
 {
-    SigArgs a = {};
-    CheckArgs c = {};
+    a = SigArgs();
+    c = CheckArgs();
     size_t next_chunk[SIG_GROUPS] = { 0, 0 };
     auto add = [&](const void* p, size_t bytes, int group) {
         if (!p || bytes == 0) return;
@@ -151,6 +53,13 @@
         c.force[1] = rq.rays_force ? 1 : 0;
         c.rays_ext = rq.rays_ext;
     }
+}
+
+grace_status launch_signatures(const SigRequest& rq, unsigned long long* partial, hipStream_t stream)
+{
+    SigArgs a;
+    CheckArgs c;
+    sig_build(rq, a, c);
     if (!c.ctl[0] && !c.ctl[1]) return GRACE_OK;
     signature_kernel<<<SIG_GRID, SIG_BLOCK, 0, stream>>>(a, partial);
     GRACE_CHECK_LAUNCH();
diff --git a/grace-devel_amd/csrc/trace_coherence.hip b/grace-devel_amd/csrc/trace_coherence.hip
--- a/grace-devel_amd/csrc/trace_coherence.hip
+++ b/grace-devel_amd/csrc/trace_coherence.hip
@@ -179,7 +179,10 @@
     if (lat_flag || split_dev)
         choose_variants(ext12, n, scene_min, lat_flag, split_packets, split_launched, split_dev);
     if (plan_split_dev) *plan_split_dev = planned_split(split_packets);
-    if (gate.ctl) {
+    if (gate.ctl && gate.decided) {
+        PlanCtl& pc = *gate.ctl;
+        if (pc.record != 0u) { pc.unusable = 0u; pc.usable = 1u; }
+    } else if (gate.ctl) {
         PlanCtl& pc = *gate.ctl;
         const bool stale = pc.sig[0] != gate.scene->sig[0] || pc.sig[1] != gate.scene->sig[1]
             || pc.sig[2] != gate.rays->sig[0] || pc.sig[3] != gate.rays->sig[1];
diff --git a/grace-devel_amd/csrc/trace_kernel.hpp b/grace-devel_amd/csrc/trace_kernel.hpp
--- a/grace-devel_amd/csrc/trace_kernel.hpp
+++ b/grace-devel_amd/csrc/trace_kernel.hpp
@@ -2,6 +2,7 @@
 
 #include "trace_diag.hpp"
 #include "trace_packet.hpp"
+#include "trace_signature.hpp"
 #include "trace_state.hpp"
 
 #include <type_traits>
@@ -246,7 +247,6 @@
     static_assert(!LAT || has_lattice(MODE), "no lattice cull for this mode");
     static_assert(!PLANNED || (SPLIT && !LAT && f4_sums(MODE)), "planned: class-split column densities only");
     if constexpr (PLANNED) {
-        if (*plan_const<uint32_t>(a.plan_usable) == 0u) return;
     } else if (has_lattice(MODE)) {
         if (a.plan_usable && *a.plan_usable != 0u) return;
         if (a.lat_dev ? (*a.lat_dev != 0) != LAT : LAT) return;
@@ -264,17 +264,33 @@
     __shared__ __align__(16) float2 s_tile[LDS_TILE ? TRACE_BLOCK / 64 : 1][LDS_TILE ? 3 + WP : 1][LDS_TILE ? 66 : 1];
     __shared__ double s_tile_d[D4 ? TRACE_BLOCK / 64 : 1][D4 ? 64 : 1][D4 ? 6 : 1];
     __shared__ float4 s_tile_f[F4D ? TRACE_BLOCK / 64 : 1][F4D ? 64 : 1][F4D ? 2 : 1];
+    uint32_t block = blockIdx.x;
+    if constexpr (PLANNED) {
+        static_assert(sizeof(s_tile) >= (SIG_LDS_WORDS + 1) * sizeof(unsigned long long), "the signature role reduces in the tile");
+        if (block < uint32_t(a.spec.sig_blocks)) {
+            signature_role(a.spec, reinterpret_cast<unsigned long long*>(&s_tile[0][0][0]));
+            return;
+        }
+        block -= uint32_t(a.spec.sig_blocks);
+        if (*plan_const<uint32_t>(a.plan_usable) == 0u) return;
+        if (a.spec.sig_blocks == 0 && a.spec.flags) {
+            if (*plan_const<uint32_t>(a.spec.flags) != 0u) return;
+            if (block == 0 && threadIdx.x == 0) a.spec.flags[1] = 1u;
+        }
+    }
     const int lane = threadIdx.x & 63;
     static_assert(!SPLIT || class_split(MODE) || MODE == MODE_HITS, "triangle and stats walks do not split");
     constexpr bool RANGE_SPLIT = SPLIT && MODE == MODE_HITS;
     const int split_ordinary = !SPLIT ? 1 : (!RANGE_SPLIT && a.split_dev) ? *a.split_dev : a.split;
     int split_planned = 0;
-    if constexpr (PLANNED)
-        if (a.plan_split_dev) split_planned = *plan_const<int>(a.plan_split_dev);
+    if constexpr (PLANNED) {
+        if (a.spec.split > 0) split_planned = a.spec.split;
+        else if (a.plan_split_dev) split_planned = *plan_const<int>(a.plan_split_dev);
+    }
     const int split = PLANNED && split_planned > 0 ? split_planned : split_ordinary;
     const int n_packets = (a.n_rays + a.width - 1) / a.width;
     const int nb = (n_packets * split + TRACE_BLOCK / 64 - 1) / (TRACE_BLOCK / 64);
-    const int q = nb >> 3, r8 = nb & 7, xcd = blockIdx.x & 7, slot = blockIdx.x >> 3;
+    const int q = nb >> 3, r8 = nb & 7, xcd = block & 7, slot = block >> 3;
     if (slot >= q + (xcd < r8 ? 1 : 0)) return;
     const int vblock = (xcd < r8 ? xcd * (q + 1) : r8 * (q + 1) + (xcd - r8) * q) + slot;
     const int wave_id = __builtin_amdgcn_readfirstlane(vblock * (TRACE_BLOCK / 64)
diff --git a/grace-devel_amd/csrc/trace_planned.hip b/grace-devel_amd/csrc/trace_planned.hip
--- a/grace-devel_amd/csrc/trace_planned.hip
+++ b/grace-devel_amd/csrc/trace_planned.hip
@@ -209,6 +209,7 @@
     GRACE_TRY(plan_free_buffers(ts.plan));
     ts.plan = PacketPlan();
     ts.last_plan_ctl = nullptr;
+    ts.last_plan_flag = nullptr;
     return GRACE_OK;
 }
 
@@ -217,6 +218,7 @@
     PacketPlan& pp = ts.plan;
     GRACE_TRY(plan_free_buffers(pp));
     ts.last_plan_ctl = nullptr;
+    ts.last_plan_flag = nullptr;
     pp.key = key;
     pp.dead = true;
     const int n_packets = (a.n_rays + a.width - 1) / a.width;
diff --git a/grace-devel_amd/csrc/trace_signature.hpp b/grace-devel_amd/csrc/trace_signature.hpp
--- /dev/null
+++ b/grace-devel_amd/csrc/trace_signature.hpp
@@ -0,0 +1,179 @@
+#pragma once
+
+#include "trace_state.hpp"
+
+#include <cstdint>
+
+namespace grace_hip {
+
+constexpr int SIG_LDS_WORDS = (SIG_BLOCK / 64) * 2 * SIG_GROUPS;
+constexpr int SIG_UNROLL = 2;
+
+__device__ __forceinline__ unsigned long long sig_mix64(unsigned long long v)
+{
+    v ^= v >> 32;
+    v *= 0xD6E8FEB86659FD93ull;
+    v ^= v >> 29;
+    return v;
+}
+
+constexpr unsigned long long SIG_K1 = 0x9E3779B97F4A7C15ull, SIG_K2 = 0xC2B2AE3D27D4EB4Full;
+
+__device__ __forceinline__ void sig_add_chunk(const uint4 q, const unsigned long long i1, const unsigned long long i2,
+                                              unsigned long long& ax, unsigned long long& ay)
+{
+    const unsigned long long lo = (unsigned long long)q.x | ((unsigned long long)q.y << 32);
+    const unsigned long long hi = (unsigned long long)q.z | ((unsigned long long)q.w << 32);
+    const unsigned long long x = sig_mix64(lo ^ i1);
+    const unsigned long long y = sig_mix64((hi + ((x << 31) | (x >> 33))) ^ i2);
+    ax += x;
+    ay += y;
+}
+
+template <typename T>
+__device__ __forceinline__ T sig_pick(const T (&v)[4], const int k)
+{
+    return k == 0 ? v[0] : k == 1 ? v[1] : k == 2 ? v[2] : v[3];
+}
+
+__device__ __forceinline__ void signature_block(const SigArgs& a, const int block, const int n_blocks,
+                                       unsigned long long* __restrict__ partial, unsigned long long* s_red)
+{
+    static_assert(SIG_GROUPS == 2, "two groups' sums, selected without indexing");
+    unsigned long long sx[SIG_GROUPS] = { 0ull, 0ull }, sy[SIG_GROUPS] = { 0ull, 0ull };
+    const size_t t0 = size_t(block) * SIG_BLOCK + threadIdx.x, stride = size_t(n_blocks) * SIG_BLOCK;
+    const unsigned long long step1 = stride * SIG_K1, step2 = stride * SIG_K2;
+    for (int k = 0; k < a.n_arrays; ++k) {
+        const size_t words = sig_pick(a.words, k), n_chunks = (words + 3) / 4;
+        const size_t n_whole = sig_pick(a.aligned, k) ? words / 4 : 0;
+        const uint32_t* w = sig_pick(a.base, k);
+        const size_t chunk0 = sig_pick(a.chunk0, k);
+        unsigned long long ax = 0ull, ay = 0ull;
+        size_t c = t0;
+        unsigned long long i1 = (chunk0 + c) * SIG_K1, i2 = (chunk0 + c) * SIG_K2;
+        for (; c + (SIG_UNROLL - 1) * stride < n_whole; c += SIG_UNROLL * stride) {
+            const uint4* p = reinterpret_cast<const uint4*>(w) + c;
+            uint4 q[SIG_UNROLL];
+#pragma unroll
+            for (int u = 0; u < SIG_UNROLL; ++u) q[u] = p[u * stride];
+#pragma unroll
+            for (int u = 0; u < SIG_UNROLL; ++u) {
+                sig_add_chunk(q[u], i1, i2, ax, ay);
+                i1 += step1; i2 += step2;
+            }
+        }
+        for (; c < n_chunks; c += stride, i1 += step1, i2 += step2) {
+            uint4 q;
+            if (c < n_whole) {
+                q = reinterpret_cast<const uint4*>(w)[c];
+            } else {
+                q.x = 4 * c + 0 < words ? w[4 * c + 0] : 0u;
+                q.y = 4 * c + 1 < words ? w[4 * c + 1] : 0u;
+                q.z = 4 * c + 2 < words ? w[4 * c + 2] : 0u;
+                q.w = 4 * c + 3 < words ? w[4 * c + 3] : 0u;
+            }
+            sig_add_chunk(q, i1, i2, ax, ay);
+        }
+        const bool g0 = sig_pick(a.group, k) == 0;
+        sx[0] += g0 ? ax : 0ull; sy[0] += g0 ? ay : 0ull;
+        sx[1] += g0 ? 0ull : ax; sy[1] += g0 ? 0ull : ay;
+    }
+    const int lane = threadIdx.x & 63, wave = threadIdx.x >> 6;
+#pragma unroll
+    for (int g = 0; g < SIG_GROUPS; ++g) {
+#pragma unroll
+        for (int off = 32; off > 0; off >>= 1) {
+            sx[g] += __shfl_xor(sx[g], off);
+            sy[g] += __shfl_xor(sy[g], off);
+        }
+        if (lane == 0) {
+            s_red[wave * 2 * SIG_GROUPS + 2 * g] = sx[g];
+            s_red[wave * 2 * SIG_GROUPS + 2 * g + 1] = sy[g];
+        }
+    }
+    __syncthreads();
+    if (threadIdx.x < 2 * SIG_GROUPS) {
+        unsigned long long v = 0ull;
+        for (int w = 0; w < SIG_BLOCK / 64; ++w) v += s_red[w * 2 * SIG_GROUPS + threadIdx.x];
+        partial[size_t(block) * 2 * SIG_GROUPS + threadIdx.x] = v;
+    }
+}
+
+struct SigVerdict {
+    unsigned long long sig[2 * SIG_GROUPS];
+    bool stale[SIG_GROUPS];
+};
+
+__device__ __forceinline__ SigVerdict signature_check(const unsigned long long* partial, const int n_blocks,
+                                             const CheckArgs& a, unsigned long long* s_red)
+{
+    unsigned long long v[2 * SIG_GROUPS] = { 0ull, 0ull, 0ull, 0ull };
+    for (int b = threadIdx.x; b < n_blocks; b += SIG_BLOCK)
+#pragma unroll
+        for (int k = 0; k < 2 * SIG_GROUPS; ++k)
+            v[k] += __hip_atomic_load(const_cast<unsigned long long*>(partial) + size_t(b) * 2 * SIG_GROUPS + k,
+                                      __ATOMIC_RELAXED, __HIP_MEMORY_SCOPE_AGENT);
+    const int lane = threadIdx.x & 63, wave = threadIdx.x >> 6;
+#pragma unroll
+    for (int k = 0; k < 2 * SIG_GROUPS; ++k) {
+#pragma unroll
+        for (int off = 32; off > 0; off >>= 1) v[k] += __shfl_xor(v[k], off);
+        if (lane == 0) s_red[wave * 2 * SIG_GROUPS + k] = v[k];
+    }
+    __syncthreads();
+    SigVerdict out = {};
+    if (threadIdx.x == 0) {
+#pragma unroll
+        for (int g = 0; g < SIG_GROUPS; ++g) {
+            CacheCtl* ctl = a.ctl[g];
+            if (!ctl) continue;
+            unsigned long long x = a.salt[g], y = ~a.salt[g];
+            for (int w = 0; w < SIG_BLOCK / 64; ++w) {
+                x += s_red[w * 2 * SIG_GROUPS + 2 * g];
+                y += s_red[w * 2 * SIG_GROUPS + 2 * g + 1];
+            }
+            const bool stale = a.force[g] || ctl->sig[0] != x || ctl->sig[1] != y;
+            ctl->sig[0] = x;
+            ctl->sig[1] = y;
+            ctl->stale = stale ? 1u : 0u;
+            if (g == 1 && stale && a.rays_ext) {
+                for (int k = 0; k < 16; ++k) a.rays_ext[k] = k < 6 ? 0xFFFFFFFFu : 0u;
+            }
+            out.sig[2 * g] = x; out.sig[2 * g + 1] = y; out.stale[g] = stale;
+        }
+    }
+    return out;
+}
+
+__device__ __forceinline__ void signature_role(const SpecArgs& s, unsigned long long* s_red)
+{
+    signature_block(s.sig, blockIdx.x, s.sig_blocks, s.partial, s_red);
+    if (threadIdx.x < 64) {
+        __builtin_amdgcn_fence(__ATOMIC_RELEASE, "agent");
+        if (threadIdx.x == 0)
+            s_red[SIG_LDS_WORDS] = atomicAdd(&s.plan_ctl->ticket, 1u) == uint32_t(s.sig_blocks - 1) ? 1ull : 0ull;
+    }
+    __syncthreads();
+    if (s_red[SIG_LDS_WORDS] == 0ull) return;
+    __builtin_amdgcn_fence(__ATOMIC_ACQUIRE, "agent");
+    const SigVerdict v = signature_check(s.partial, s.sig_blocks, s.check, s_red);
+    if (threadIdx.x == 0) {
+        PlanCtl& pc = *s.plan_ctl;
+        bool moved = false;
+#pragma unroll
+        for (int k = 0; k < 2 * SIG_GROUPS; ++k) moved = moved || pc.sig[k] != v.sig[k];
+        pc.record = moved ? 1u : 0u;
+        if (moved) {
+#pragma unroll
+            for (int k = 0; k < 2 * SIG_GROUPS; ++k) pc.sig[k] = v.sig[k];
+            for (int k = 0; k < 6; ++k) pc.stats[k] = 0ull;
+            pc.largest_round = 0u;
+        }
+        const uint32_t ok = !v.stale[0] && !v.stale[1] && !moved && pc.usable != 0u ? 1u : 0u;
+        s.flags[0] = ok;
+        s.flags[1] = ok;
+        pc.ticket = 0u;
+    }
+}
+
+}
diff --git a/grace-devel_amd/csrc/trace_state.hpp b/grace-devel_amd/csrc/trace_state.hpp
--- a/grace-devel_amd/csrc/trace_state.hpp
+++ b/grace-devel_amd/csrc/trace_state.hpp
@@ -26,6 +26,40 @@
 constexpr int MAX_HIT_CHUNKS = 256;
 constexpr int SUM_CLASSES = 8;
 constexpr int GRANULE_SHIFT = 10;
+
+constexpr int SIG_BLOCK = 256;
+constexpr int SIG_GRID = 1024;
+constexpr int SIG_GROUPS = 2;
+static_assert(SIG_BLOCK == TRACE_BLOCK, "the planned kernel's signature role runs in its workgroups");
+
+struct CacheCtl;
+struct PlanCtl;
+
+struct SigArgs {
+    const uint32_t* base[4];
+    size_t words[4];
+    size_t chunk0[4];
+    int group[4];
+    int aligned[4];
+    int n_arrays;
+};
+
+struct CheckArgs {
+    CacheCtl* ctl[SIG_GROUPS];
+    int force[SIG_GROUPS];
+    unsigned long long salt[SIG_GROUPS];
+    uint32_t* rays_ext;
+};
+
+struct SpecArgs {
+    int sig_blocks;
+    int split;
+    SigArgs sig;
+    CheckArgs check;
+    unsigned long long* partial;
+    PlanCtl* plan_ctl;
+    uint32_t* flags;
+};
 
 
 enum { MODE_COUNT = 0, MODE_CUMULATIVE = 1, MODE_HITS = 2, MODE_STATS = 3, MODE_TRI = 4,
@@ -144,6 +178,7 @@
     const int* plan_counts;
     const uint32_t* plan_usable;
     const int* plan_split_dev;
+    SpecArgs spec;
 };
 
 
@@ -198,6 +233,8 @@
     uint32_t largest_round;
     unsigned long long sig[4];
     unsigned long long stats[6];
+    uint32_t ticket;
+    uint32_t pad;
 };
 constexpr uint32_t PLAN_ROUND_END = 4u;
 constexpr int PLAN_FORMAT = 2;
@@ -232,6 +269,7 @@
     const CacheCtl* scene = nullptr;
     const CacheCtl* rays = nullptr;
     PlanCtl* ctl = nullptr;
+    bool decided = false;
 };
 
 __host__ __device__ inline int planned_split(const int n_packets)
@@ -271,6 +309,7 @@
     double custom_host[N_TABLE] = {};
     bool plan_on = true;
     size_t plan_budget = size_t(512) << 20;
+    int spec_sig_blocks = 64;
     Scene scene;
     RayOrder rays;
     HitsCache hits;
@@ -278,6 +317,7 @@
     PacketPlan plan;
     const PlanCtl* last_plan_ctl = nullptr;
     hipStream_t last_plan_stream = nullptr;
+    const uint32_t* last_plan_flag = nullptr;
 };
 
 grace_status trace_state(TraceState** out);
@@ -291,19 +331,28 @@
     return GRACE_OK;
 }
 
-template <typename Launches>
-grace_status timed(TraceState& ts, hipStream_t stream, Launches launches)
+inline grace_status timed_begin(TraceState& ts, hipStream_t stream)
 {
     if (ts.timing) {
         if (!ts.ev0) { GRACE_TRY_HIP(hipEventCreate(&ts.ev0)); GRACE_TRY_HIP(hipEventCreate(&ts.ev1)); }
         GRACE_TRY_HIP(hipEventRecord(ts.ev0, stream));
     }
-    GRACE_TRY(launches());
+    return GRACE_OK;
+}
+inline grace_status timed_end(TraceState& ts, hipStream_t stream)
+{
     if (ts.timing) {
         GRACE_TRY_HIP(hipEventRecord(ts.ev1, stream));
         ts.ev_valid = true;
     }
     return GRACE_OK;
+}
+template <typename Launches>
+grace_status timed(TraceState& ts, hipStream_t stream, Launches launches)
+{
+    GRACE_TRY(timed_begin(ts, stream));
+    GRACE_TRY(launches());
+    return timed_end(ts, stream);
 }
 
 size_t sig_partial_words();
@@ -316,6 +365,7 @@
     CacheCtl* rays_ctl = nullptr; bool rays_force = false;
     uint32_t* rays_ext = nullptr;
 };
+void sig_build(const SigRequest& rq, SigArgs& a, CheckArgs& c);
 grace_status launch_signatures(const SigRequest& rq, unsigned long long* partial, hipStream_t stream);
 
 grace_status scene_release(TraceState& ts);
diff --git a/grace-devel_amd/grace_hip/__init__.py b/grace-devel_amd/grace_hip/__init__.py
--- a/grace-devel_amd/grace_hip/__init__.py
+++ b/grace-devel_amd/grace_hip/__init__.py
@@ -341,6 +341,10 @@
 
 def set_plan_budget(n_bytes):
     _check(_lib.grace_trace_set_plan_budget(C.c_size_t(int(n_bytes))))
+
+
+def set_signature_blocks(n):
+    _check(_lib.grace_trace_set_signature_blocks(C.c_int(int(n))))
 
 
 def plan_bytes():
diff --git a/include/grace_hip.h b/include/grace_hip.h
--- a/include/grace_hip.h
+++ b/include/grace_hip.h
@@ -240,6 +240,7 @@
 grace_status grace_trace_set_plan_budget(size_t bytes);
 grace_status grace_trace_plan_bytes(size_t* h_bytes);
 grace_status grace_trace_last_plan_used(int* h_used);
+grace_status grace_trace_set_signature_blocks(int blocks);
 grace_status grace_trace_plan_stats(unsigned long long* h_stats );
 
 grace_status grace_trace_status(grace_stream stream);
diff --git a/profiles/recipes/perf_fused_validation.py b/profiles/recipes/perf_fused_validation.py
--- /dev/null
+++ b/profiles/recipes/perf_fused_validation.py
@@ -0,0 +1,45 @@
+import sys, os, time, statistics
+ROOT = os.path.dirname(os.path.dirname(os.path.dirname(os.path.abspath(__file__))))
+sys.path.insert(0, os.path.join(ROOT, "grace-devel_amd")); sys.path.insert(0, ROOT)
+import torch
+import grace_hip as gh
+from bench import make_particles
+dev = torch.device("cuda:0")
+n = 10_000_000
+s = make_particles(n, dev)
+lo, hi = gh.min_max_vec4(s); lo[3] = hi[3] = 0.0
+tree = gh.Tree(n, 32, device=dev)
+gh.build_tree(s, tree, lo[:3], hi[:3])
+rays, _ = gh.orthogonal_rays_z(1024, lo, hi, device=dev)
+gh.enable_kernel_timing(True)
+sweep = "--sweep" in sys.argv
+
+
+def measure(call):
+    for _ in range(5): call()
+    torch.cuda.synchronize()
+    t0 = time.perf_counter()
+    for _ in range(30): call()
+    torch.cuda.synchronize()
+    ms = 1e3 * (time.perf_counter() - t0) / 30
+    k = []
+    for _ in range(10):
+        call(); k.append(gh.last_kernel_ms())
+    return ms, statistics.median(k)
+
+
+for d in ((1, 8) if sweep else (1, 2, 4, 8)):
+    sh = rays[: len(rays) // d].contiguous()
+    out = torch.empty(len(sh), dtype=torch.float32, device=dev)
+    call = lambda: gh.trace_cumulative_sph(sh, s, tree, out)
+    if sweep:
+        for rep in range(3):
+            row = []
+            for blocks in (0, 16, 32, 64, 128, 256, 1024):
+                gh.set_signature_blocks(blocks)
+                ms, k = measure(call)
+                row.append("blocks=%d call %.4f kernel %.4f" % (blocks, ms, k))
+            print("1/%d shard, plan used %d: %s" % (d, gh.last_plan_used(), "  ".join(row)), flush=True)
+    else:
+        ms, k = measure(call)
+        print("1/%d shard, plan used %d: call_ms %.4f kernel_ms %.4f" % (d, gh.last_plan_used(), ms, k), flush=True)
```

Result: no change. 555.9, median of 3 (+0.3%).
